# jopohl/urh

Hardware: NVIDIA H100
Metric: MSamples/s IQ demod+digitize (complex64) (higher is better)
Workload: dtype f32

## Files before the change

### urh_b200/csrc/center.cu

```cuda
#include "dense.cuh"
#include "scan.cuh"

#include <math.h>
#include <stdlib.h>

int urh_window_var_bitwise(urh_ctx* ctx, const float* d_x, int64_t n, const int64_t* d_prefix, int64_t t0, int64_t t1, int64_t r0,
                           int64_t r1, float* h_out2);

struct CenStats {
    double sum, sumsq;
    float mn, mx;
    long long cnt;
};

__global__ void __launch_bounds__(URH_WARPS_PER_BLOCK * 32)
k_tile_stats_f32(const float* __restrict__ x, int64_t n, int64_t ntiles, UrhTileStats* __restrict__ ts) {
    const int lane = threadIdx.x & 31;
    const int64_t tile = (int64_t)blockIdx.x * URH_WARPS_PER_BLOCK + (threadIdx.x >> 5);
    if (tile >= ntiles) return;
    const int64_t base = tile * URH_TILE;
    UrhStatAcc acc;
    acc.init();
    acc.all_noise = false;
    if (base + URH_TILE <= n && (((uintptr_t)x) & 15) == 0) {
// ... 344 lines not shown
    const int lane = threadIdx.x & 31;
    if (SMEM)
        for (int b = threadIdx.x; b < nbins; b += 256) s_hist[b] = 0u;
    if (edges_in_smem)
        for (int b = threadIdx.x; b < nbins + 3; b += 256) s_fe[b] = g_fe[b];
    __syncthreads();
    HistBins hb;
    if (FAST) hb.load(s_fe, scale, nbins);
    else hb.load(edges_in_smem ? s_fe : g_fe, scale, nbins);
    HistCache hc;
    hc.init();
    const int64_t gw = (int64_t)blk * 8 + (threadIdx.x >> 5), nw = (int64_t)nblk * 8;
    const bool vec = (((uintptr_t)x) & 15) == 0;
    const unsigned one = blockDim.x >> 8;
    {
        for (int64_t t = t_first + gw; t < t_end; t += nw) {
            if (prefix[t + 1] == prefix[t]) continue;
            const int64_t base = t * URH_TILE;
            if (vec) {
                const float4* p = (const float4*)(x + base) + lane;
                constexpr int ITERS = URH_TILE / 128, DEPTH = 4;
                float4 buf[DEPTH];
#pragma unroll
                for (int j = 0; j < DEPTH; j++) buf[j] = __ldg(p + j * 32);
#pragma unroll 1
                for (int it = 0; it < ITERS; it += DEPTH) {
                    const bool more = it + DEPTH < ITERS;
#pragma unroll
                    for (int j = 0; j < DEPTH; j++) {
                        const float4 v = buf[j];
                        if (more) buf[j] = __ldg(p + (it + DEPTH + j) * 32);
                        hist_put<SMEM, FAST>(hc, hb, s_hist, hist, v.x, one);
                        hist_put<SMEM, FAST>(hc, hb, s_hist, hist, v.y, one);
                        hist_put<SMEM, FAST>(hc, hb, s_hist, hist, v.z, one);
                        hist_put<SMEM, FAST>(hc, hb, s_hist, hist, v.w, one);
                    }
                }
            } else {
                for (int j = lane; j < URH_TILE; j += 32) hist_put<SMEM, FAST>(hc, hb, s_hist, hist, x[base + j], one);
            }
        }
    }
    hist_flush<SMEM>(hc, s_hist, hist);
    if (SMEM) {
        __syncthreads();
        for (int b = threadIdx.x; b < nbins; b += 256)
            if (s_hist[b]) atomicAdd(&hist[b], (unsigned long long)s_hist[b]);
    }
}

template <bool SMEM, bool FAST>
__global__ void __launch_bounds__(256, 4) k_hist_interior(const float* __restrict__ x, int64_t n, const int64_t* __restrict__ win,
                                                      const float* __restrict__ g_fe, float scale, int nbins,
                                                      unsigned long long* __restrict__ hist, int edges_in_smem,
                                                      const int64_t* __restrict__ prefix) {
    const int64_t w0 = win[0];
    hist_interior_body<SMEM, FAST>(x, n, w0 + 1, w0 >= 0 ? win[1] : 0, blockIdx.x, gridDim.x, g_fe, scale, nbins, hist, edges_in_smem, prefix);
}

__device__ __forceinline__ void hist_window_ends_body(const float* __restrict__ x, int64_t n, const int64_t* __restrict__ prefix,
                                                      const int64_t* __restrict__ win, int64_t r0, int64_t r1,
                                                      const float* __restrict__ g_fe, float scale, int nbins,
                                                      unsigned long long* __restrict__ hist, unsigned long long* __restrict__ hist2 = nullptr) {
    __shared__ int s_pre[256];
    const int64_t t = win[blockIdx.x];
    if (t < 0 || (blockIdx.x == 1 && t == win[0])) return;
    HistBins hb;
    hb.load(g_fe, scale, nbins);
    float v[CEN_PER];
    int64_t rank = cen_tile_ranks(x, n, t, prefix[t], v, s_pre);
#pragma unroll
    for (int j = 0; j < CEN_PER; j++) {
        const bool kept = v[j] > -4.0f;
        const int k = hb.bin_of<false>(v[j]);
        if (k >= 0 && rank >= r0 && rank < r1) {
            atomicAdd(&hist[k], 1ull);
            if (hist2) atomicAdd(&hist2[k], 1ull);
        }
        rank += kept ? 1 : 0;
    }
}

__global__ void __launch_bounds__(256) k_hist_window_ends(const float* __restrict__ x, int64_t n, const int64_t* __restrict__ prefix,
                                                         const int64_t* __restrict__ win, int64_t r0, int64_t r1,
                                                         const float* __restrict__ g_fe, float scale, int nbins,
                                                         unsigned long long* __restrict__ hist) {
    hist_window_ends_body(x, n, prefix, win, r0, r1, g_fe, scale, nbins, hist);
}

extern "C" int urh_center_histogram_tiles(urh_ctx* ctx, const float* d_qad, int64_t n, int64_t r0, int64_t r1, double hmin,
                                          double hstep, int64_t nbins, int64_t* h_hist) {
    if (nbins <= 0) return URH_OK;
    if (!tiles_match(ctx, d_qad, n)) URH_FAIL(ctx, URH_ERR_INVALID, "urh_afp_demod_tiles (same qad, same n) must precede urh_center_histogram_tiles");
    if (nbins > (int64_t)1 << 30) URH_FAIL(ctx, URH_ERR_INVALID, "too many histogram bins");
    const int64_t ntiles = urh_div_up(n, URH_TILE);
    const int64_t* prefix = (const int64_t*)ctx->center_prefix;
    unsigned long long* hist;
    float* fe;
    int64_t* d_win;
    URH_CHECK(urh_arena(ctx, (size_t)nbins, &hist));
    URH_CHECK(urh_arena(ctx, (size_t)nbins + 3, &fe));
    URH_CHECK(urh_arena(ctx, 4, &d_win));
    URH_CUDA(ctx, cudaMemsetAsync(hist, 0, (size_t)nbins * sizeof(unsigned long long), ctx->stream));
    URH_CUDA(ctx, cudaMemsetAsync(d_win, 0xff, 4 * sizeof(int64_t), ctx->stream));
    if (r1 > r0) {
        URH_LAUNCH(ctx, k_hist_edges, (unsigned)urh_div_up(nbins + 1, 256), 256, 0, hmin, hstep, nbins, fe);
        URH_LAUNCH(ctx, k_find_window_tiles, (unsigned)urh_div_up(ntiles, 256), 256, 0, prefix, ntiles, r0, r1, d_win);
        const bool in_smem = nbins <= 12000;
        const int edges_smem = (in_smem && nbins <= 6000) ? 1 : 0;
        const size_t dyn = (in_smem ? (size_t)nbins * 4 : 0) + (edges_smem ? (size_t)(nbins + 3) * 4 : 0);
        const float scale = (float)(1.0 / hstep);
        const double edge_abs = fmax(fabs(hmin), fabs(hmin + (double)nbins * hstep));
        const bool fast = edges_smem && hstep > 0.0 && edge_abs / hstep < 1048576.0;
        const unsigned gs = (unsigned)min(urh_div_up(ntiles, 8), (int64_t)ctx->sm_count * 8);
        const int64_t* cw = d_win;
        const float* cfe = fe;
        if (in_smem && fast) URH_LAUNCH(ctx, (k_hist_interior<true, true>), gs, 256, dyn, d_qad, n, cw, cfe, scale, (int)nbins, hist, edges_smem, prefix);
        else if (in_smem) URH_LAUNCH(ctx, (k_hist_interior<true, false>), gs, 256, dyn, d_qad, n, cw, cfe, scale, (int)nbins, hist, edges_smem, prefix);
        else URH_LAUNCH(ctx, (k_hist_interior<false, false>), gs, 256, dyn, d_qad, n, cw, cfe, scale, (int)nbins, hist, edges_smem, prefix);
        URH_LAUNCH(ctx, k_hist_window_ends, 2, 256, 0, d_qad, n, prefix, (const int64_t*)d_win, r0, r1, (const float*)fe, scale, (int)nbins, hist);
    }
    URH_CUDA(ctx, cudaMemcpyAsync(h_hist, hist, (size_t)nbins * sizeof(int64_t), cudaMemcpyDeviceToHost, ctx->stream));
    URH_CUDA(ctx, cudaStreamSynchronize(ctx->stream));
    return URH_OK;
}

extern "C" int urh_center_histogram(urh_ctx* ctx, const float* d_x, int64_t n, int64_t r0, int64_t r1, double hmin,
                                    double hstep, int64_t nbins, int64_t* h_hist) {
    if (nbins <= 0 || n <= 0) return URH_OK;
    if (!tiles_match(ctx, d_x, n)) {
        int64_t total = 0;
        URH_CHECK(tiles_from_array(ctx, d_x, n, &total));
    }
    return urh_center_histogram_tiles(ctx, d_x, n, r0, r1, hmin, hstep, nbins, h_hist);
}

#include "tilescan.cuh"

#define CEN_MAX_BINS 6000

struct __align__(16) CenterPlan {
    long long total, offset;
    long long r0, r1;
    long long lr0, lr1;
    long long win[4];
    CenStats local;
    double hmin, edge1, delta;
    long long nbins;
    double center;
    float centerf;
    float scale;
    int fast;
    int state;
    unsigned int ticket;
    int certified;
    long long straddle;
    long long pad;
};

struct ScanKept {
    const UrhTileStats* ts;
    int64_t* prefix;
    __device__ __forceinline__ int64_t load(int64_t t) const { return ts[t].cnt; }
    __device__ __forceinline__ void post(int64_t t, const int64_t& excl, const int64_t&) const { prefix[t] = excl; }
};
struct CenAddI64 {
    __device__ __forceinline__ int64_t operator()(int64_t a, int64_t b) const { return a + b; }
};

__global__ void k_center_ranks(const int64_t* __restrict__ counts, int rank, int world, int64_t max_size, CenterPlan* __restrict__ plan) {
    long long total = 0, offset = 0;
    for (int q = 0; q < world; q++) {
        if (q < rank) offset += counts[q];
        total += counts[q];
    }
    const long long kept = counts[rank];
    long long r0 = (long long)(0.05 * (double)total), r1 = (long long)(0.95 * (double)total);
    if (max_size >= 0 && r1 - r0 > max_size) r1 = r0 + max_size;
    plan->total = total; plan->offset = offset; plan->r0 = r0; plan->r1 = r1;
    long long a = r0 - offset, b = r1 - offset;
    a = a < 0 ? 0 : (a > kept ? kept : a);
    b = b < 0 ? 0 : (b > kept ? kept : b);
    plan->lr0 = a; plan->lr1 = b;
    plan->ticket = 0u;
    plan->state = 1;
    plan->certified = 0;
    plan->straddle = 0;
}

__device__ __forceinline__ int64_t cen_tile_of_rank(const int64_t* __restrict__ prefix, int64_t ntiles, int64_t r) {
    int64_t lo = 0, hi = ntiles;
    while (hi - lo > 1) {
        const int64_t mid = (lo + hi) >> 1;
        if (prefix[mid] <= r) lo = mid; else hi = mid;
    }
    return lo;
}

__global__ void __launch_bounds__(256) k_center_window(const float* __restrict__ x, int64_t n, const UrhTileStats* __restrict__ ts,
                                                      const int64_t* __restrict__ prefix, int64_t ntiles, CenterPlan* __restrict__ plan,
                                                      CenStats* __restrict__ partial) {
    __shared__ long long s_win[4];
    __shared__ int s_pre[256];
    __shared__ bool s_last;
    const long long r0 = plan->lr0, r1 = plan->lr1;
    if (threadIdx.x == 0) {
        long long w0 = -1, w1 = -1, w2 = -1, w3 = -1;
        if (r1 > r0) {
            w0 = cen_tile_of_rank(prefix, ntiles, r0);
            w1 = cen_tile_of_rank(prefix, ntiles, r1 - 1);
            const bool cov0 = prefix[w0] >= r0 && prefix[w0 + 1] <= r1;
            const bool cov1 = prefix[w1] >= r0 && prefix[w1 + 1] <= r1;
            w2 = cov0 ? -1 : w0;
            w3 = (cov1 || w1 == w0) ? -1 : w1;
        }
        s_win[0] = w0; s_win[1] = w1; s_win[2] = w2; s_win[3] = w3;
        if (blockIdx.x == 0) { plan->win[0] = w0; plan->win[1] = w1; plan->win[2] = w2; plan->win[3] = w3; }
    }
    __syncthreads();
    double sum = 0.0, sq = 0.0;
    float mn = INFINITY, mx = -INFINITY;
    long long cnt = 0;
    if (s_win[0] >= 0) {
        for (int64_t t = s_win[0] + (int64_t)blockIdx.x * 256 + threadIdx.x; t <= s_win[1]; t += (int64_t)gridDim.x * 256) {
            const int64_t a = prefix[t], b = prefix[t + 1];
            if (b > a && a >= r0 && b <= r1) {
                const UrhTileStats v = ts[t];
                sum += v.sum; sq += v.sumsq; mn = fminf(mn, v.mn); mx = fmaxf(mx, v.mx); cnt += v.cnt;
            }
        }
    }
    cen_block_fold(sum, sq, mn, mx, cnt, partial + blockIdx.x);
    if (blockIdx.x < 2) {
        const int64_t t = s_win[2 + blockIdx.x];
        sum = 0.0; sq = 0.0; mn = INFINITY; mx = -INFINITY; cnt = 0;
        if (t >= 0) {
            float v[CEN_PER];
            int64_t rank = cen_tile_ranks(x, n, t, prefix[t], v, s_pre);
#pragma unroll
            for (int j = 0; j < CEN_PER; j++) {
                if (v[j] > -4.0f) {
                    if (rank >= r0 && rank < r1) {
                        sum += (double)v[j];
                        sq += (double)v[j] * (double)v[j];
                        mn = fminf(mn, v[j]);
                        mx = fmaxf(mx, v[j]);
                        cnt++;
                    }
                    rank++;
                }
            }
        }
        cen_block_fold(sum, sq, mn, mx, cnt, partial + gridDim.x + blockIdx.x);
    }
    __threadfence();
    __syncthreads();
    if (threadIdx.x == 0) s_last = atomicAdd(&plan->ticket, 1u) == gridDim.x - 1;
    __syncthreads();
    if (!s_last) return;
    __threadfence();
    sum = 0.0; sq = 0.0; mn = INFINITY; mx = -INFINITY; cnt = 0;
    for (int64_t t = threadIdx.x; t < (int64_t)gridDim.x + 2; t += 256) {
        CenStats p;
        {
            const int4* src = (const int4*)(partial + t);
            int4 w0 = __ldcg(src), w1 = __ldcg(src + 1);
            memcpy(&p, &w0, 16);
            memcpy((char*)&p + 16, &w1, 16);
        }
        sum += p.sum; sq += p.sumsq; mn = fminf(mn, p.mn); mx = fmaxf(mx, p.mx); cnt += p.cnt;
    }
    cen_block_fold(sum, sq, mn, mx, cnt, &plan->local);
}

__global__ void __launch_bounds__(256) k_center_plan(const CenStats* __restrict__ parts, int world, CenterPlan* __restrict__ plan,
                                                    float* __restrict__ fe, unsigned long long* __restrict__ hist,
                                                    unsigned long long* __restrict__ xhist) {
    __shared__ int s_state;
    __shared__ long long s_nbins;
    __shared__ double s_hmin, s_edge1, s_delta;
    if (threadIdx.x == 0) {
        double cnt = 0.0, sum = 0.0, sq = 0.0;
        float mn = INFINITY, mx = -INFINITY;
        for (int q = 0; q < world; q++) {
            cnt += (double)parts[q].cnt;
            mn = fminf(mn, parts[q].mn);
            mx = fmaxf(mx, parts[q].mx);
            sum = __dadd_rn(sum, parts[q].sum);
            sq = __dadd_rn(sq, parts[q].sumsq);
        }
        int state = 0;
        long long nbins = 0;
        double hmin = 0.0, edge1 = 0.0, delta = 0.0;
        if (plan->r1 > plan->r0 && cnt > 0.0) {
            const double mean = __ddiv_rn(sum, cnt);
            double ss = __dsub_rn(sq, __dmul_rn(__dmul_rn(cnt, mean), mean));
            if (ss < 0.0) ss = 0.0;
            const double var = __ddiv_rn(ss, cnt);
            const double hstep = (double)__double2float_rn(var);
            hmin = (double)mn;
            const double stop = __dadd_rn((double)mx, hstep);
            if (hstep != 0.0) {
                const double val = __ddiv_rn(__dsub_rn(stop, hmin), hstep);
                if (val == val && fabs(val) < 9.0e18) {
                    const long long len = (long long)ceil(val);
                    if (len >= 2) {
                        nbins = len - 1;
                        edge1 = __dadd_rn(hmin, hstep);
                        delta = __dsub_rn(edge1, hmin);
                        state = (nbins <= CEN_MAX_BINS && delta > 0.0) ? 1 : 2;
                    }
                }
            }
        }
        plan->hmin = hmin; plan->edge1 = edge1; plan->delta = delta; plan->nbins = nbins;
        plan->state = state;
        plan->center = 0.0; plan->centerf = 0.0f;
        if (state == 1) {
            plan->scale = (float)(1.0 / delta);
            const double edge_abs = fmax(fabs(hmin), fabs(hmin + (double)nbins * delta));
            plan->fast = (edge_abs / delta < 1048576.0) ? 1 : 0;
        }
        s_state = state; s_nbins = nbins; s_hmin = hmin; s_edge1 = edge1; s_delta = delta;
    }
    __syncthreads();
    if (s_state != 1) return;
    const long long nbins = s_nbins;
    for (long long k = threadIdx.x; k <= nbins; k += 256) {
        const double e = (k == 0) ? s_hmin : (k == 1 ? s_edge1 : __dadd_rn(s_hmin, __dmul_rn((double)k, s_delta)));
        fe[k] = __double2float_ru(e);
        if (k == nbins) {
            fe[nbins + 1] = __double2float_rd(e);
            fe[nbins + 2] = fmaxf(__double2float_ru(s_hmin), nextafterf(-4.0f, 0.0f));
        }
        if (k < nbins) {
            hist[k] = 0ull;
            if (xhist) xhist[k] = 0ull;
        }
    }
}

template <bool FAST>
__global__ void __launch_bounds__(256, 3) k_hist_interior_dev(const float* __restrict__ x, int64_t n, const CenterPlan* __restrict__ plan,
                                                          const float* __restrict__ g_fe, unsigned long long* __restrict__ hist,
                                                          const int64_t* __restrict__ prefix) {
    if (plan->state != 1 || plan->certified || (plan->fast != 0) != FAST) return;
    hist_interior_body<true, FAST>(x, n, plan->win[0] + 1, plan->win[1], blockIdx.x, gridDim.x, g_fe, plan->scale, (int)plan->nbins, hist, 1,
                                   prefix);
}

__device__ __forceinline__ void cen_full_slabs(int64_t win0, int64_t win1, int64_t slab_tiles, int64_t* sf, int64_t* se) {
    *sf = (win0 + slab_tiles) / slab_tiles;
    *se = win1 / slab_tiles;
}

__global__ void __launch_bounds__(256) k_hist_window_ends_dev(const float* __restrict__ x, int64_t n, const int64_t* __restrict__ prefix,
                                                             const CenterPlan* __restrict__ plan, const float* __restrict__ g_fe,
                                                             unsigned long long* __restrict__ hist, unsigned long long* __restrict__ xhist,
                                                             int64_t slab_tiles) {
    if (plan->state != 1) return;
    if (blockIdx.x < 2) {
        hist_window_ends_body(x, n, prefix, (const int64_t*)plan->win, plan->lr0, plan->lr1, g_fe, plan->scale, (int)plan->nbins, hist, xhist);
        return;
    }
    const int64_t w0 = plan->win[0], w1 = plan->win[1];
    int64_t sf, se;
    cen_full_slabs(w0, w1, slab_tiles, &sf, &se);
    int64_t a_end = w1, b_begin = w1;
    if (sf < se) { a_end = sf * slab_tiles; b_begin = se * slab_tiles; }
    const int blk = blockIdx.x - 2, nblk = gridDim.x - 2, nbins = (int)plan->nbins;
    const float scale = plan->scale;
    if (plan->fast) {
        hist_interior_body<true, true>(x, n, w0 + 1, a_end, blk, nblk, g_fe, scale, nbins, xhist, 1, prefix);
        hist_interior_body<true, true>(x, n, b_begin, w1, blk, nblk, g_fe, scale, nbins, xhist, 1, prefix);
    } else {
        hist_interior_body<true, false>(x, n, w0 + 1, a_end, blk, nblk, g_fe, scale, nbins, xhist, 1, prefix);
        hist_interior_body<true, false>(x, n, b_begin, w1, blk, nblk, g_fe, scale, nbins, xhist, 1, prefix);
    }
}

__device__ __forceinline__ double cen_left_edge(const CenterPlan* plan, int k) {
    return (k == 0) ? plan->hmin : (k == 1 ? plan->edge1 : __dadd_rn(plan->hmin, __dmul_rn((double)k, plan->delta)));
}

#define CERT_THREADS 512
__global__ void __launch_bounds__(CERT_THREADS) k_center_certify(const UrhFine fine, CenterPlan* __restrict__ plan, const float* __restrict__ fe,
                                                                 const unsigned long long* __restrict__ xhist, unsigned long long* __restrict__ lo,
                                                                 unsigned long long* __restrict__ hi) {
    __shared__ unsigned long long s_ge[URH_FINE_NB + 1];
    __shared__ unsigned long long s_part[CERT_THREADS];
    __shared__ unsigned char s_flag[CEN_MAX_BINS];
    __shared__ unsigned long long s_key[3];
    __shared__ unsigned int s_certain;
    if (plan->state != 1) return;
    const int tid = threadIdx.x;
    constexpr int PER = URH_FINE_NB / CERT_THREADS;
    int64_t sf, se;
    cen_full_slabs(plan->win[0], plan->win[1], fine.slab_tiles, &sf, &se);
    unsigned long long b[PER], tot = 0;
#pragma unroll
    for (int j = 0; j < PER; j++) {
        unsigned long long v = 0;
        for (int64_t sl = sf; sl < se; sl++) v += fine.gh[sl * URH_FINE_NB + tid * PER + j];
        b[j] = v;
        tot += v;
    }
    s_part[tid] = tot;
    if (tid < 3) s_key[tid] = 0ull;
    if (tid == 0) s_certain = 0u;
    __syncthreads();
    for (int off = 1; off < CERT_THREADS; off <<= 1) {
        const unsigned long long add = (tid + off < CERT_THREADS) ? s_part[tid + off] : 0ull;
        __syncthreads();
        s_part[tid] += add;
        __syncthreads();
    }
    unsigned long long run = (tid + 1 < CERT_THREADS) ? s_part[tid + 1] : 0ull;
#pragma unroll
    for (int j = PER - 1; j >= 0; j--) {
        run += b[j];
        s_ge[tid * PER + j] = run;
    }
    if (tid == 0) s_ge[URH_FINE_NB] = 0ull;
    __syncthreads();
    const int nbins = (int)plan->nbins;
    const float f_hi = fe[nbins + 1], f_min = fe[nbins + 2], top = nextafterf(f_hi, INFINITY);
    auto ge = [&](float t, unsigned long long& glo, unsigned long long& ghi) {
        const int bt = urh_fine_bucket(t, fine.scale, fine.off);
        const bool straddles = urh_fine_bucket(nextafterf(t, -INFINITY), fine.scale, fine.off) == bt;
        ghi = s_ge[bt];
        glo = straddles ? s_ge[bt + 1] : s_ge[bt];
    };
    for (int k = tid; k < nbins; k += CERT_THREADS) {
        const float a = fmaxf(fe[k], f_min), e = (k == nbins - 1) ? top : fminf(fe[k + 1], top);
        unsigned long long l = 0, u = 0;
        if (a < e) {
            unsigned long long alo, ahi, elo, ehi;
            ge(a, alo, ahi);
            ge(e, elo, ehi);
            l = alo > ehi ? alo - ehi : 0ull;
            u = ahi - elo;
        }
        lo[k] = xhist[k] + l;
        hi[k] = xhist[k] + u;
    }
    __syncthreads();
    int window = (int)(0.05 * (double)nbins) + 1;
    if (window < 2) window = 2;
    for (int k = tid; k < nbins; k += CERT_THREADS) {
        const unsigned long long l = lo[k], u = hi[k];
        bool certain = l > 0ull, possible = u > 0ull;
        for (int d = -(window - 1); d < window && (certain || possible); d++) {
            const int j = k + d;
            if (d == 0 || j < 0 || j >= nbins) continue;
            certain = certain && l > hi[j];
            possible = possible && u > lo[j];
        }
        s_flag[k] = certain ? 1 : (possible ? 2 : 0);
        if (certain) atomicAdd(&s_certain, 1u);
    }
    __syncthreads();
    for (int pass = 0; pass < 3; pass++) {
        const long long p0 = pass > 0 ? (long long)(8191 - (s_key[0] & 8191)) : -1, p1 = pass > 1 ? (long long)(8191 - (s_key[1] & 8191)) : -1;
        for (int k = tid; k < nbins; k += CERT_THREADS) {
            if (k == p0 || k == p1) continue;
            if (pass < 2 && s_flag[k] == 1) atomicMax(&s_key[pass], (lo[k] << 13) | (unsigned long long)(8191 - k));
            if (pass == 2 && s_flag[k] != 0) atomicMax(&s_key[2], hi[k]);
        }
        __syncthreads();
    }
    if (tid != 0 || s_certain < 2u) return;
    const int k1 = 8191 - (int)(s_key[0] & 8191), k2 = 8191 - (int)(s_key[1] & 8191);
    plan->straddle = (long long)((hi[k1] - lo[k1]) + (hi[k2] - lo[k2]));
    if (!(lo[k2] > s_key[2])) return;
    const double c = __ddiv_rn(__dadd_rn(cen_left_edge(plan, k1), cen_left_edge(plan, k2)), 2.0);
    plan->center = c;
    plan->centerf = __double2float_rn(c);
    plan->certified = 1;
}

__global__ void __launch_bounds__(256) k_center_pick(const unsigned long long* __restrict__ y, CenterPlan* __restrict__ plan) {
    __shared__ unsigned long long s_best[256];
    __shared__ int s_idx[256];
    __shared__ int s_cnt[256];
    if (plan->state != 1 || plan->certified) return;
    const int nbins = (int)plan->nbins;
    int window = (int)(0.05 * (double)nbins) + 1;
    if (window < 2) window = 2;
    unsigned long long top_val[2] = {0ull, 0ull};
    int top_idx[2] = {-1, -1};
    int found = 0;
    bool undecided = false;
    for (int pass = 0; pass < 2 && !undecided; pass++) {
        unsigned long long best = 0ull;
        int bi = -1, ties = 0;
        for (int i = threadIdx.x; i < nbins; i += 256) {
            if (pass == 1 && i == top_idx[0]) continue;
            const unsigned long long v = y[i];
            if (v == 0ull || v < best) continue;
            bool peak = true;
            for (int d = 1; d < window && peak; d++) {
                const unsigned long long a = (i + d < nbins) ? y[i + d] : 0ull;
                const unsigned long long b = (i - d >= 0) ? y[i - d] : 0ull;
                peak = v > a && v > b;
            }
            if (!peak) continue;
            if (v > best) { best = v; bi = i; ties = 1; }
            else ties++;
        }
        s_best[threadIdx.x] = best; s_idx[threadIdx.x] = bi; s_cnt[threadIdx.x] = ties;
        __syncthreads();
        if (threadIdx.x == 0) {
            unsigned long long b = 0ull;
            int idx = -1, t = 0;
            for (int j = 0; j < 256; j++) {
                if (s_idx[j] < 0) continue;
                if (s_best[j] > b) { b = s_best[j]; idx = s_idx[j]; t = s_cnt[j]; }
                else if (s_best[j] == b) t += s_cnt[j];
            }
            s_best[0] = b; s_idx[0] = idx; s_cnt[0] = t;
        }
        __syncthreads();
        const unsigned long long b = s_best[0];
        const int idx = s_idx[0], t = s_cnt[0];
        __syncthreads();
        if (idx < 0) break;
        if (pass == 0) {
            top_val[0] = b; top_idx[0] = idx; found = 1;
            if (t == 2) {
                int other = -1;
                for (int i = threadIdx.x; i < nbins; i += 256) {
                    if (i == idx || y[i] != b) continue;
                    bool peak = true;
                    for (int d = 1; d < window && peak; d++) {
                        const unsigned long long a = (i + d < nbins) ? y[i + d] : 0ull;
                        const unsigned long long c = (i - d >= 0) ? y[i - d] : 0ull;
                        peak = b > a && b > c;
                    }
                    if (peak) other = i;
                }
                s_idx[threadIdx.x] = other;
                __syncthreads();
                if (threadIdx.x == 0) {
                    int o = -1;
                    for (int j = 0; j < 256; j++) if (s_idx[j] >= 0) o = s_idx[j];
                    s_idx[0] = o;
                }
                __syncthreads();
                top_idx[1] = s_idx[0]; top_val[1] = b; found = 2;
                __syncthreads();
                break;
            }
            if (t > 2) undecided = true;
        } else {
            if (t > 1) undecided = true;
            else { top_val[1] = b; top_idx[1] = idx; found = 2; }
        }
    }
    if (threadIdx.x != 0) return;
    if (undecided) { plan->state = 2; return; }
    if (found == 0) { plan->state = 0; return; }
    double c;
    if (found == 1) c = cen_left_edge(plan, top_idx[0]);
    else c = __ddiv_rn(__dadd_rn(cen_left_edge(plan, top_idx[0]), cen_left_edge(plan, top_idx[1])), 2.0);
    plan->center = c;
    plan->centerf = __double2float_rn(c);
    plan->state = 1;
    (void)top_val;
}

int urh_coll_allgather(urh_ctx* ctx, const void* d_send, void* d_recv, size_t bytes_per_rank);
bool urh_p2p_usable(urh_ctx* ctx, size_t bytes_per_rank);
extern "C" int urh_p2p_allreduce_u64_dev(urh_ctx* ctx, const void* d_in, void* d_out, const int64_t* d_count, int max_words);
extern "C" int urh_nccl_allreduce_i64(urh_ctx* ctx, int64_t* d_buf, int64_t count, int op);

int urh_center_chain(urh_ctx* ctx, const float* d_qad, int64_t n, const UrhTileStats* ts, int64_t max_size, int rank, int world,
                     const UrhFine* fine, CenterPlan** d_plan_out) {
    const int64_t ntiles = urh_div_up(n, URH_TILE);
    int64_t* prefix;
    CenterPlan* plan;
    CenStats* partial;
    float* fe;
    unsigned long long* hist;
    int64_t* d_counts;
    CenStats* d_parts;
    unsigned long long *xhist = nullptr, *cert_lo = nullptr, *cert_hi = nullptr;
    const int nb = ctx->sm_count * 2;
    URH_CHECK(urh_arena(ctx, (size_t)ntiles + 1, &prefix));
    URH_CHECK(urh_arena(ctx, 1, &plan));
    URH_CHECK(urh_arena(ctx, (size_t)nb + 2, &partial));
    URH_CHECK(urh_arena(ctx, (size_t)CEN_MAX_BINS + 3, &fe));
    URH_CHECK(urh_arena(ctx, (size_t)CEN_MAX_BINS, &hist));
    URH_CHECK(urh_arena(ctx, (size_t)world, &d_counts));
    URH_CHECK(urh_arena(ctx, (size_t)world, &d_parts));
    if (fine) {
        URH_CHECK(urh_arena(ctx, (size_t)CEN_MAX_BINS, &xhist));
        URH_CHECK(urh_arena(ctx, (size_t)CEN_MAX_BINS, &cert_lo));
        URH_CHECK(urh_arena(ctx, (size_t)CEN_MAX_BINS, &cert_hi));
    }
    ScanKept fk;
    fk.ts = ts; fk.prefix = prefix;
    URH_CHECK((urhts::scan<int64_t, CenAddI64, ScanKept>(ctx, ntiles, (int64_t)0, CenAddI64(), fk, prefix + ntiles)));
    const int64_t* counts = prefix + ntiles;
    if (world > 1) {
        URH_TL_MARK(ctx, "x1 kept counts: enter");
        URH_CHECK(urh_coll_allgather(ctx, prefix + ntiles, d_counts, sizeof(int64_t)));
        URH_TL_MARK(ctx, "x1 kept counts: done");
        counts = d_counts;
    }
    URH_LAUNCH(ctx, k_center_ranks, 1, 1, 0, counts, rank, world, max_size, plan);
    URH_LAUNCH(ctx, k_center_window, nb, 256, 0, d_qad, n, ts, (const int64_t*)prefix, ntiles, plan, partial);
    const CenStats* parts = &plan->local;
    if (world > 1) {
        URH_TL_MARK(ctx, "x2 window partials: enter");
        URH_CHECK(urh_coll_allgather(ctx, &plan->local, d_parts, sizeof(CenStats)));
        URH_TL_MARK(ctx, "x2 window partials: done");
        parts = d_parts;
    }
    URH_LAUNCH(ctx, k_center_plan, 1, 256, 0, parts, world, plan, fe, hist, xhist);
    const size_t dyn = (size_t)CEN_MAX_BINS * 4 + (size_t)(CEN_MAX_BINS + 3) * 4;
    const unsigned gs = (unsigned)min(urh_div_up(ntiles, 8), (int64_t)ctx->sm_count * 8);
    URH_LAUNCH(ctx, k_hist_window_ends_dev, fine ? 2 + ctx->sm_count * 4 : 2, 256, fine ? dyn : 0, d_qad, n, (const int64_t*)prefix,
               (const CenterPlan*)plan, (const float*)fe, hist, xhist, fine ? fine->slab_tiles : (int64_t)1);
    if (fine) URH_LAUNCH(ctx, k_center_certify, 1, CERT_THREADS, 0, *fine, plan, (const float*)fe, (const unsigned long long*)xhist, cert_lo, cert_hi);
    URH_LAUNCH(ctx, (k_hist_interior_dev<true>), gs, 256, dyn, d_qad, n, (const CenterPlan*)plan, (const float*)fe, hist, (const int64_t*)prefix);
    URH_LAUNCH(ctx, (k_hist_interior_dev<false>), gs, 256, dyn, d_qad, n, (const CenterPlan*)plan, (const float*)fe, hist, (const int64_t*)prefix);
    const unsigned long long* hist_all = hist;
    if (world > 1) URH_TL_MARK(ctx, "x3 histogram sum: enter");
    if (world > 1) {
        if (urh_p2p_usable(ctx, 8)) {
            unsigned long long* hist_sum;
            URH_CHECK(urh_arena(ctx, (size_t)CEN_MAX_BINS, &hist_sum));
            URH_CHECK(urh_p2p_allreduce_u64_dev(ctx, hist, hist_sum, (const int64_t*)&plan->nbins, CEN_MAX_BINS));
            hist_all = hist_sum;
        } else {
            URH_CHECK(urh_nccl_allreduce_i64(ctx, (int64_t*)hist, CEN_MAX_BINS, 0));
        }
    }
    if (world > 1) URH_TL_MARK(ctx, "x3 histogram sum: done");
    URH_LAUNCH(ctx, k_center_pick, 1, 256, 0, hist_all, plan);
    ctx->center_prefix = prefix;
    ctx->center_ts = ts;
    ctx->center_n = n;
    ctx->center_x = d_qad;
    *d_plan_out = plan;
    return URH_OK;
}

int urh_center_plan_certify_stats(urh_ctx* ctx, const CenterPlan* plan, int64_t* h_dst3) {
    h_dst3[0] = h_dst3[1] = h_dst3[2] = 0;
    URH_CUDA(ctx, cudaMemcpyAsync(h_dst3, &plan->certified, sizeof(int), cudaMemcpyDeviceToHost, ctx->stream));
    URH_CUDA(ctx, cudaMemcpyAsync(h_dst3 + 2, &plan->straddle, sizeof(long long), cudaMemcpyDeviceToHost, ctx->stream));
    return URH_OK;
}

extern "C" int urh_center_certify_stats(urh_ctx* ctx, int64_t* h_out3) {
    for (int i = 0; i < 3; i++) h_out3[i] = ctx->center_cert[i];
    return URH_OK;
}

int urh_center_plan_result(urh_ctx* ctx, const CenterPlan* plan, const float** d_centerf, const double** d_center, const int** d_state) {
    if (d_centerf) *d_centerf = &plan->centerf;
    if (d_center) *d_center = &plan->center;
    if (d_state) *d_state = &plan->state;
    return URH_OK;
}
```

### urh_b200/csrc/common.cuh

```cuda
#pragma once
#include <cuda_runtime.h>
#include <stdint.h>
#include <stdio.h>
#include <stdlib.h>
#include <string.h>
#include <vector>

#include "../../include/urh_b200.h"

#define URH_FULL_MASK 0xffffffffu

struct urh_block {
    void* ptr;
    size_t bytes;
};

struct urh_ctx {
    int device;
    int sm_count;
    cudaStream_t stream;
    cudaStream_t copy_stream[2];
    cudaEvent_t ev_start, ev_stop;
    cudaEvent_t ev_copy[2], ev_comp[2];
    cudaEvent_t ev_k0, ev_k1;
    int profiling;
    int dense_timed;
    cudaEvent_t tl_ev[32];
    const char* tl_name[32];
    int tl_count, tl_ready;
    char err[512];
    int64_t launches;
    std::vector<urh_block> arena;
    size_t arena_block;
    size_t arena_used;
    size_t arena_need;
    int64_t* pulses;
    size_t pulses_cap_rows;
    int64_t pulses_k;
    int64_t* h_mail;
    void* h_stage[2];
    size_t h_stage_bytes;
    int fft_plan;
    int fft_nfft;
    int64_t fft_batch;
    bool fft_valid;
    void* img_tw;
    int img_tw_n;
    void* shard_tiles;
    void* shard_staging;
    int shard_cap, shard_tol;
    int64_t shard_n;
    void* shard_state;
    int64_t costas_stats[3];
    int64_t costas_redone;
    int64_t costas_stitch[4];
    int mod_plan[2];
    int mod_plan_valid[2];
    int64_t mod_plan_n[2];
    int bits_valid;
    int64_t bits_nmsg, bits_total, bits_npos;
    void *bits_ptr, *bits_msg_off, *bits_pauses, *bits_pos;
    const void* center_ts;
    const void* center_x;
    int64_t center_n;
    void* center_prefix;
    int64_t center_cert[3];
    int64_t spec_stats[3];
    void* nccl_comm;
    void* nccl_stage;
    void* nccl_hstage;
    int nccl_rank, nccl_world;
    void* p2p_local;
    void* p2p_peer[8];
    void* p2p_hout;
    int p2p_rank, p2p_world;
    unsigned long long p2p_seq;
    void* ts_mem;
    int64_t ts_cap_blocks;
    unsigned long long ts_issued;
    uint32_t ts_epoch;
    void* step_dev;
    void* shard_fin;
    int64_t stream_free_low, stream_chunks;
    size_t arena_live;
    size_t arena_peak;
};

#define URH_CUDA(ctx, call)                                                                         \
    do {                                                                                            \
        cudaError_t e__ = (call);                                                                   \
        if (e__ != cudaSuccess) {                                                                   \
            snprintf((ctx)->err, sizeof((ctx)->err), "%s:%d: %s -> %s", __FILE__, __LINE__, #call,  \
                     cudaGetErrorString(e__));                                                      \
            return (e__ == cudaErrorMemoryAllocation) ? URH_ERR_NOMEM : URH_ERR_CUDA;               \
        }                                                                                           \
    } while (0)

#define URH_CHECK(call)                 \
    do {                                \
        int rc__ = (call);              \
        if (rc__ != URH_OK) return rc__; \
    } while (0)

#define URH_FAIL(ctx, code, ...)                                  \
    do {                                                          \
        snprintf((ctx)->err, sizeof((ctx)->err), __VA_ARGS__);    \
        return (code);                                            \
    } while (0)

#define URH_LAUNCH(ctx, kernel, grid, block, smem, ...)                                   \
    do {                                                                                  \
        kernel<<<(grid), (block), (smem), (ctx)->stream>>>(__VA_ARGS__);                  \
        (ctx)->launches++;                                                                \
        URH_CUDA(ctx, cudaGetLastError());                                                \
    } while (0)

#define URH_TL_MARK(ctx, label) do { if ((ctx)->profiling >= 2 && (ctx)->tl_ready && (ctx)->tl_count < 32) { \
        (ctx)->tl_name[(ctx)->tl_count] = (label); cudaEventRecord((ctx)->tl_ev[(ctx)->tl_count++], (ctx)->stream); } } while (0)
#define URH_TL_RESET(ctx) do { (ctx)->tl_count = 0; } while (0)
#define URH_PROF_BEGIN(ctx) do { if ((ctx)->profiling) cudaEventRecord((ctx)->ev_k0, (ctx)->stream); } while (0)
#define URH_PROF_END(ctx) do { if ((ctx)->profiling) { cudaEventRecord((ctx)->ev_k1, (ctx)->stream); (ctx)->dense_timed = 1; } } while (0)

void urh_arena_reset(urh_ctx* ctx);
int urh_arena_alloc(urh_ctx* ctx, size_t bytes, void** out);
template <typename T>
static inline int urh_arena(urh_ctx* ctx, size_t count, T** out) {
    void* p = nullptr;
    int rc = urh_arena_alloc(ctx, count * sizeof(T), &p);
    *out = (T*)p;
    return rc;
}
struct UrhArenaMark {
    size_t block, used, live;
};
static inline UrhArenaMark urh_arena_mark(const urh_ctx* ctx) { return UrhArenaMark{ctx->arena_block, ctx->arena_used, ctx->arena_live}; }
static inline void urh_arena_release(urh_ctx* ctx, const UrhArenaMark& m) {
    ctx->arena_block = m.block;
    ctx->arena_used = m.used;
    ctx->arena_live = m.live;
}
int urh_ensure_pulses(urh_ctx* ctx, size_t rows);
int urh_ensure_pulses_keep(urh_ctx* ctx, size_t rows, size_t keep);
void urh_stream_sample_free(urh_ctx* ctx);
void urh_release_mod_plans(urh_ctx* ctx);
int urh_ensure_stage(urh_ctx* ctx, size_t bytes);

struct UrhCostasStream {
    float* state;
    int64_t* acc;
    int segs;
};
int urh_costas_stream_begin(urh_ctx* ctx, UrhCostasStream* S);
int urh_costas_stream_chunk(urh_ctx* ctx, UrhCostasStream* S, int64_t c, const void* d_iq, int dtype, int64_t n, float noise_sqrd,
                            int loop_order, float bandwidth, float* d_out);
int urh_costas_stream_end(urh_ctx* ctx, const UrhCostasStream* S);
int64_t urh_costas_arena_bytes(int64_t n, int loop_order);

int urh_read_i64(urh_ctx* ctx, const int64_t* d_src, int count, int64_t* h_out);

__host__ __device__ static inline int64_t urh_div_up(int64_t a, int64_t b) { return (a + b - 1) / b; }

static inline int urh_iq_bytes(int dtype) {
    switch (dtype) {
        case URH_DT_I8:
        case URH_DT_U8: return 2;
        case URH_DT_I16:
        case URH_DT_U16: return 4;
        case URH_DT_F32: return 8;
        default: return 0;
    }
}

static inline float urh_noise_value(int mod_type) {
    switch (mod_type) {
        case URH_MOD_ASK: return 0.0f;
        case URH_MOD_FSK:
        case URH_MOD_PSK:
        case URH_MOD_OQPSK: return -4.0f;
        case URH_MOD_QAM: return 0.0f * -4.0f;
        default: return 0.0f;
    }
}
```

### urh_b200/csrc/context.cu

```cuda
#include "common.cuh"
#include "tilescan.cuh"

extern "C" int urh_device_count(void) {
    int n = 0;
    if (cudaGetDeviceCount(&n) != cudaSuccess) return 0;
    return n;
}

extern "C" int urh_ctx_create(int device, urh_ctx** out) {
    if (!out) return URH_ERR_INVALID;
    *out = nullptr;
    int n = 0;
    if (cudaGetDeviceCount(&n) != cudaSuccess || n <= 0) return URH_ERR_NO_DEVICE;
    if (device < 0 || device >= n) return URH_ERR_INVALID;
    urh_ctx* ctx = new urh_ctx();
    ctx->device = device;
    ctx->err[0] = 0;
    ctx->launches = 0;
    ctx->arena_block = 0;
    ctx->arena_used = 0;
    ctx->arena_need = 0;
    ctx->pulses = nullptr;
    ctx->pulses_cap_rows = 0;
    ctx->pulses_k = 0;
    ctx->h_mail = nullptr;
    ctx->h_stage[0] = ctx->h_stage[1] = nullptr;
    ctx->h_stage_bytes = 0;
    ctx->fft_valid = false;
    ctx->shard_tiles = nullptr;
    ctx->shard_staging = nullptr;
    ctx->shard_state = nullptr;
    ctx->bits_valid = 0;
    ctx->mod_plan_valid[0] = ctx->mod_plan_valid[1] = 0;
    ctx->center_prefix = nullptr;
    ctx->center_ts = nullptr;
    ctx->center_x = nullptr;
    ctx->center_n = 0;
    ctx->nccl_comm = nullptr;
    ctx->nccl_stage = nullptr;
    ctx->nccl_hstage = nullptr;
    ctx->p2p_local = nullptr;
    ctx->p2p_hout = nullptr;
    ctx->p2p_world = 0;
    ctx->p2p_rank = 0;
    ctx->p2p_seq = 0;
    for (int i = 0; i < 8; i++) ctx->p2p_peer[i] = nullptr;
    ctx->nccl_rank = 0;
    ctx->nccl_world = 1;
    ctx->stream_free_low = -1;
    ctx->stream_chunks = 0;
    if (cudaSetDevice(device) != cudaSuccess) {
        delete ctx;
        return URH_ERR_CUDA;
    }
    cudaDeviceProp prop;
    if (cudaGetDeviceProperties(&prop, device) != cudaSuccess) {
        delete ctx;
        return URH_ERR_CUDA;
    }
    ctx->sm_count = prop.multiProcessorCount;
    {
        cudaMemPool_t pool;
        if (cudaDeviceGetDefaultMemPool(&pool, device) == cudaSuccess) {
            unsigned long long keep = ~0ull;
            cudaMemPoolSetAttribute(pool, cudaMemPoolAttrReleaseThreshold, &keep);
        }
    }
    bool ok = cudaStreamCreateWithFlags(&ctx->stream, cudaStreamNonBlocking) == cudaSuccess;
    ok = ok && cudaStreamCreateWithFlags(&ctx->copy_stream[0], cudaStreamNonBlocking) == cudaSuccess;
    ok = ok && cudaStreamCreateWithFlags(&ctx->copy_stream[1], cudaStreamNonBlocking) == cudaSuccess;
    ok = ok && cudaEventCreate(&ctx->ev_start) == cudaSuccess && cudaEventCreate(&ctx->ev_stop) == cudaSuccess;
    for (int i = 0; i < 2 && ok; i++) {
        ok = ok && cudaEventCreateWithFlags(&ctx->ev_copy[i], cudaEventDisableTiming) == cudaSuccess;
        ok = ok && cudaEventCreateWithFlags(&ctx->ev_comp[i], cudaEventDisableTiming) == cudaSuccess;
    }
    ok = ok && cudaEventCreate(&ctx->ev_k0) == cudaSuccess && cudaEventCreate(&ctx->ev_k1) == cudaSuccess;
    ctx->profiling = 0;
    ctx->dense_timed = 0;
    ctx->tl_count = 0;
    ctx->tl_ready = 0;
    ok = ok && cudaHostAlloc((void**)&ctx->h_mail, 64 * sizeof(int64_t), cudaHostAllocDefault) == cudaSuccess;
    if (!ok) {
        delete ctx;
        return URH_ERR_CUDA;
    }
    *out = ctx;
    return URH_OK;
}

extern "C" void urh_ctx_destroy(urh_ctx* ctx) {
    if (!ctx) return;
    cudaSetDevice(ctx->device);
    cudaStreamSynchronize(ctx->stream);
    urh_release_mod_plans(ctx);
    for (auto& b : ctx->arena) cudaFree(b.ptr);
    if (ctx->pulses) cudaFree(ctx->pulses);
    if (ctx->shard_state) free(ctx->shard_state);
    if (ctx->h_mail) cudaFreeHost(ctx->h_mail);
    if (ctx->ts_mem) cudaFree(ctx->ts_mem);
    if (ctx->step_dev) cudaFree(ctx->step_dev);
    if (ctx->img_tw) cudaFree(ctx->img_tw);
    if (ctx->shard_fin) free(ctx->shard_fin);
    for (int i = 0; i < 2; i++)
        if (ctx->h_stage[i]) cudaFreeHost(ctx->h_stage[i]);
    cudaEventDestroy(ctx->ev_start);
    cudaEventDestroy(ctx->ev_stop);
    for (int i = 0; i < 2; i++) {
        cudaEventDestroy(ctx->ev_copy[i]);
        cudaEventDestroy(ctx->ev_comp[i]);
        cudaStreamDestroy(ctx->copy_stream[i]);
    }
    cudaStreamDestroy(ctx->stream);
    delete ctx;
}

extern "C" const char* urh_last_error(urh_ctx* ctx) { return ctx ? ctx->err : "null context"; }

extern "C" int urh_sync(urh_ctx* ctx) {
    URH_CUDA(ctx, cudaStreamSynchronize(ctx->stream));
    return URH_OK;
}

extern "C" int urh_device_info(urh_ctx* ctx, int* sm_count, int* cc_major, int* cc_minor, size_t* total_mem,
                               char* name, int name_cap) {
    cudaDeviceProp prop;
    URH_CUDA(ctx, cudaGetDeviceProperties(&prop, ctx->device));
    if (sm_count) *sm_count = prop.multiProcessorCount;
    if (cc_major) *cc_major = prop.major;
    if (cc_minor) *cc_minor = prop.minor;
    if (total_mem) *total_mem = prop.totalGlobalMem;
    if (name && name_cap > 0) {
        strncpy(name, prop.name, name_cap - 1);
        name[name_cap - 1] = 0;
    }
    return URH_OK;
}

extern "C" int urh_malloc(urh_ctx* ctx, size_t bytes, void** d_ptr) {
    URH_CUDA(ctx, cudaSetDevice(ctx->device));
    if (bytes == 0) bytes = 16;
    URH_CUDA(ctx, cudaMallocAsync(d_ptr, bytes, ctx->stream));
    return URH_OK;
}

extern "C" int urh_free(urh_ctx* ctx, void* d_ptr) {
    if (!d_ptr) return URH_OK;
    URH_CUDA(ctx, cudaFreeAsync(d_ptr, ctx->stream));
    return URH_OK;
}

extern "C" int urh_memset(urh_ctx* ctx, void* d_ptr, int value, size_t bytes) {
    URH_CUDA(ctx, cudaMemsetAsync(d_ptr, value, bytes, ctx->stream));
    return URH_OK;
}

extern "C" int urh_memcpy_h2d(urh_ctx* ctx, void* d_dst, const void* h_src, size_t bytes) {
    if (bytes == 0) return URH_OK;
    URH_CUDA(ctx, cudaMemcpyAsync(d_dst, h_src, bytes, cudaMemcpyHostToDevice, ctx->stream));
    return URH_OK;
}

extern "C" int urh_memcpy_d2h(urh_ctx* ctx, void* h_dst, const void* d_src, size_t bytes) {
    if (bytes) URH_CUDA(ctx, cudaMemcpyAsync(h_dst, d_src, bytes, cudaMemcpyDeviceToHost, ctx->stream));
    URH_CUDA(ctx, cudaStreamSynchronize(ctx->stream));
    return URH_OK;
}

extern "C" int urh_memcpy_d2d(urh_ctx* ctx, void* d_dst, const void* d_src, size_t bytes) {
    if (bytes == 0) return URH_OK;
    URH_CUDA(ctx, cudaMemcpyAsync(d_dst, d_src, bytes, cudaMemcpyDeviceToDevice, ctx->stream));
    return URH_OK;
}

extern "C" int urh_host_alloc(urh_ctx* ctx, size_t bytes, void** h_ptr) {
    if (bytes == 0) bytes = 16;
    URH_CUDA(ctx, cudaHostAlloc(h_ptr, bytes, cudaHostAllocDefault));
    return URH_OK;
}

extern "C" int urh_host_free(urh_ctx* ctx, void* h_ptr) {
    if (h_ptr) URH_CUDA(ctx, cudaFreeHost(h_ptr));
    return URH_OK;
}

extern "C" int urh_timer_start(urh_ctx* ctx) {
    URH_CUDA(ctx, cudaEventRecord(ctx->ev_start, ctx->stream));
    return URH_OK;
}

extern "C" int urh_timer_stop(urh_ctx* ctx, float* ms) {
    URH_CUDA(ctx, cudaEventRecord(ctx->ev_stop, ctx->stream));
    URH_CUDA(ctx, cudaEventSynchronize(ctx->ev_stop));
    float t = 0.f;
    URH_CUDA(ctx, cudaEventElapsedTime(&t, ctx->ev_start, ctx->ev_stop));
    if (ms) *ms = t;
    return URH_OK;
}

extern "C" int urh_set_profiling(urh_ctx* ctx, int enabled) {
    ctx->profiling = enabled < 0 ? 0 : (enabled > 2 ? 2 : enabled);
    ctx->dense_timed = 0;
    if (ctx->profiling >= 2 && !ctx->tl_ready) {
        for (int i = 0; i < 32; i++) URH_CUDA(ctx, cudaEventCreate(&ctx->tl_ev[i]));
        ctx->tl_ready = 1;
    }
    ctx->tl_count = 0;
    return URH_OK;
}

extern "C" int urh_timeline_fetch(urh_ctx* ctx, float* h_ms, char* h_names, int names_cap, int* count) {
    if (!count) return URH_ERR_INVALID;
    *count = 0;
    if (ctx->profiling < 2 || ctx->tl_count == 0) return URH_OK;
    URH_CUDA(ctx, cudaEventSynchronize(ctx->tl_ev[ctx->tl_count - 1]));
    int pos = 0;
    for (int i = 0; i < ctx->tl_count; i++) {
        float t = 0.f;
        URH_CUDA(ctx, cudaEventElapsedTime(&t, ctx->tl_ev[0], ctx->tl_ev[i]));
        if (h_ms) h_ms[i] = t;
        if (h_names) pos += snprintf(h_names + pos, pos < names_cap ? (size_t)(names_cap - pos) : 0, "%s\n", ctx->tl_name[i]);
    }
    *count = ctx->tl_count;
    return URH_OK;
}

extern "C" int urh_last_dense_ms(urh_ctx* ctx, float* ms) {
    if (!ctx->dense_timed) URH_FAIL(ctx, URH_ERR_INVALID, "no dense kernel timed (enable urh_set_profiling first)");
    URH_CUDA(ctx, cudaEventSynchronize(ctx->ev_k1));
    URH_CUDA(ctx, cudaEventElapsedTime(ms, ctx->ev_k0, ctx->ev_k1));
    return URH_OK;
}

extern "C" int64_t urh_launch_count(urh_ctx* ctx) { return ctx ? ctx->launches : 0; }

void urh_arena_reset(urh_ctx* ctx) {
    if (ctx->arena.size() > 1) {
        cudaStreamSynchronize(ctx->stream);
        size_t total = 0;
        for (auto& b : ctx->arena) {
            total += b.bytes;
            cudaFree(b.ptr);
        }
        ctx->arena.clear();
        void* p = nullptr;
        if (cudaMalloc(&p, total) == cudaSuccess) ctx->arena.push_back({p, total});
        else cudaGetLastError();
    }
    ctx->arena_block = 0;
    ctx->arena_used = 0;
    ctx->arena_need = 0;
    ctx->arena_live = 0;
    ctx->arena_peak = 0;
    ctx->center_prefix = nullptr;
    ctx->bits_valid = 0;
}

static void arena_note_peak(urh_ctx* ctx) {
    if (ctx->arena_live > ctx->arena_peak) ctx->arena_peak = ctx->arena_live;
}

int urh_arena_alloc(urh_ctx* ctx, size_t bytes, void** out) {
    bytes = (bytes + 255) & ~(size_t)255;
    if (bytes == 0) bytes = 256;
    ctx->arena_need += bytes;
// ... 126 lines not shown
```

### urh_b200/csrc/digitize.cu

```cuda
#include "dense.cuh"
#include "scan.cuh"
#include "sparse.cuh"
#ifndef URH_FAST_MIN_BLOCKS
#define URH_FAST_MIN_BLOCKS 4
#endif
#include "fsk_fast.cuh"
#include "dense_f32.cuh"
#include "stream_ring.cuh"

#include <math.h>
#include <stdlib.h>


template <int DT, int MOD, bool DIGITIZE>
__device__ __forceinline__ void dense_iq_tile(const void* __restrict__ iq, int64_t n, const UrhDemodParams& dp, float* __restrict__ qad_out,
                                              int vec_in, int vec_out, const UrhClassify& cls, int tol, UrhTileSummary* __restrict__ tiles,
                                              uint32_t* __restrict__ staging, int stage_cap, int16_t* __restrict__ init_cls, int cls_of_zero,
                                              int64_t tile, int has_halo, UrhTileStats* __restrict__ tile_stats, const UrhFine& fine,
                                              unsigned int* s_fine, unsigned int* g_fine) {
    const int lane = threadIdx.x & 31;
    const int64_t tile_start = tile * URH_TILE;
    const int tile_len = (int)((n - tile_start) < URH_TILE ? (n - tile_start) : URH_TILE);
    const int iters = (tile_len + 63) >> 6;

    UrhRunTracker rt;
    if (DIGITIZE) rt.init(tol, staging + tile * (int64_t)stage_cap);
    UrhStatAcc acc;
    acc.init();

    float cA = 0.0f, cB = 0.0f;
    if (MOD == URH_MOD_FSK && (tile_start > 0 || has_halo) && lane == 0) {
        typedef typename UrhElem<DT>::type E;
        const E* pp = (const E*)iq + 2 * (tile_start - 1);
        const UrhFskTerms t = urh_fsk_terms((float)pp[0], (float)pp[1]);
        cA = t.A; cB = t.B;
    }

    UrhPair cur = urh_load_pair<DT>(iq, tile_start + 2 * lane, n, vec_in != 0);
    for (int it = 0; it < iters; it++) {
        const int64_t pos0 = tile_start + (int64_t)it * 64 + 2 * lane;
        UrhPair nxt;
        if (it + 1 < iters) nxt = urh_load_pair<DT>(iq, pos0 + 64, n, vec_in != 0);

        const float m0 = __fadd_rn(__fmul_rn(cur.r0, cur.r0), __fmul_rn(cur.i0, cur.i0));
        const float m1 = __fadd_rn(__fmul_rn(cur.r1, cur.r1), __fmul_rn(cur.i1, cur.i1));
        float s0 = dp.noise_value, s1 = dp.noise_value;
        if (MOD == URH_MOD_FSK) {
            const UrhFskTerms t0 = urh_fsk_terms(cur.r0, cur.i0);
            const UrhFskTerms t1 = urh_fsk_terms(cur.r1, cur.i1);
            float pA = __shfl_up_sync(URH_FULL_MASK, t1.A, 1);
            float pB = __shfl_up_sync(URH_FULL_MASK, t1.B, 1);
            if (lane == 0) { pA = cA; pB = cB; }
            cA = __shfl_sync(URH_FULL_MASK, t1.A, 31);
            cB = __shfl_sync(URH_FULL_MASK, t1.B, 31);
            if (!(m0 <= dp.noise_sqrd)) s0 = urh_fsk_angle(pA, pB, t0.C, t0.D);
            if (!(m1 <= dp.noise_sqrd)) s1 = urh_fsk_angle(t0.A, t0.B, t1.C, t1.D);
        } else if (MOD == URH_MOD_ASK) {
            if (!(m0 <= dp.noise_sqrd)) s0 = __fdiv_rn(__fsqrt_rn(m0), dp.max_mag);
            if (!(m1 <= dp.noise_sqrd)) s1 = __fdiv_rn(__fsqrt_rn(m1), dp.max_mag);
        }
        if (pos0 == 0 && !has_halo) s0 = dp.noise_value;

        const bool v0 = pos0 < n, v1 = pos0 + 1 < n;
        if (tile_stats) {
            if (v0) { acc.add(s0); acc.all_noise = acc.all_noise && (s0 == dp.noise_value); }
            if (v1) { acc.add(s1); acc.all_noise = acc.all_noise && (s1 == dp.noise_value); }
            if (s_fine) {
                if (v0) urh_fine_add(s0, fine, s_fine, g_fine);
                if (v1) urh_fine_add(s1, fine, s_fine, g_fine);
            }
        }
        if (qad_out) {
            if (v1 && vec_out) urh_stg_f2(qad_out + pos0, s0, s1);
            else {
                if (v0) qad_out[pos0] = s0;
                if (v1) qad_out[pos0 + 1] = s1;
            }
        }
        if (DIGITIZE) {
            const int c0 = urh_classify(s0, cls), c1 = urh_classify(s1, cls);
            if (pos0 == 0) *init_cls = (int16_t)((s0 == cls.noise_value) ? -1 : cls_of_zero);
            rt.feed(it, c0, c1, v0, v1, lane);
        }
        cur = nxt;
    }
    if (tile_stats) acc.store(tile_stats + tile, lane);
    if (DIGITIZE) rt.finish(tile_len, tiles + tile, lane);
}

template <int DT, int MOD, bool DIGITIZE>
__global__ void __launch_bounds__(URH_WARPS_PER_BLOCK * 32)
k_dense_iq(const void* __restrict__ iq, int64_t n, UrhDemodParams dp, float* __restrict__ qad_out, int vec_in,
           int vec_out, const __grid_constant__ UrhClassify cls, int tol, UrhTileSummary* __restrict__ tiles,
           uint32_t* __restrict__ staging, int stage_cap, int16_t* __restrict__ init_cls, int cls_of_zero,
           int64_t tile_begin, int64_t tile_count, int has_halo, UrhTileStats* __restrict__ tile_stats, const UrhFine fine) {
    extern __shared__ unsigned int s_fine[];
    const int64_t tile_rel = (int64_t)blockIdx.x * URH_WARPS_PER_BLOCK + (threadIdx.x >> 5);
    const int64_t block_tile0 = tile_begin + (int64_t)blockIdx.x * URH_WARPS_PER_BLOCK;
    if (fine.gh) urh_fine_zero(s_fine);
    if (tile_rel < tile_count && (tile_begin + tile_rel) * URH_TILE < n)
        dense_iq_tile<DT, MOD, DIGITIZE>(iq, n, dp, qad_out, vec_in, vec_out, cls, tol, tiles, staging, stage_cap, init_cls, cls_of_zero,
                                    tile_begin + tile_rel, has_halo, tile_stats, fine,
                                    fine.gh ? s_fine : nullptr, fine.gh ? urh_fine_row(fine, tile_begin + tile_rel, block_tile0) : nullptr);
    if (fine.gh) urh_fine_flush(fine, s_fine, block_tile0);
}

template <int DT, bool DIGITIZE, bool WRITE, bool STATS>
__global__ void __launch_bounds__(URH_WARPS_PER_BLOCK * 32, URH_FAST_MIN_BLOCKS)
k_fsk_fast(const void* __restrict__ iq, int64_t n, UrhDemodParams dp, float* __restrict__ qad_out, float thr0,
           float cls_noise, int tol, UrhTileSummary* __restrict__ tiles, uint32_t* __restrict__ staging, int stage_cap,
           int64_t tile_begin, int64_t tile_count, UrhTileStats* __restrict__ tile_stats, const UrhFine fine) {
    extern __shared__ unsigned int s_fine[];
    const bool fine_on = STATS && fine.gh;
    const int lane = threadIdx.x & 31;
    const int64_t tile_rel = (int64_t)blockIdx.x * URH_WARPS_PER_BLOCK + (threadIdx.x >> 5);
    const int64_t block_tile0 = tile_begin + (int64_t)blockIdx.x * URH_WARPS_PER_BLOCK;
    if (fine_on) urh_fine_zero(s_fine);
    if (tile_rel < tile_count) {
        const int64_t tile = tile_begin + tile_rel;
        UrhRunTracker rt;
        if (DIGITIZE) rt.init(tol, staging + tile * (int64_t)stage_cap);
        UrhOne one;
        one.p = dp.one;
        one.m = dp.mone;
        urh_fsk_full_tile<DT, DIGITIZE, WRITE, STATS>(iq, n, tile * URH_TILE, dp, qad_out, thr0, cls_noise, rt, lane, one,
                                                      STATS ? tile_stats + tile : nullptr, 0u, DIGITIZE ? tiles + tile : nullptr, fine,
                                                      fine_on ? s_fine : nullptr, fine_on ? urh_fine_row(fine, tile, block_tile0) : nullptr);
    }
    if (fine_on) urh_fine_flush(fine, s_fine, block_tile0);
}

#define URH_FSK_FIFO 3
template <int DT, bool DIGITIZE, bool WRITE, bool STATS>
__global__ void __launch_bounds__(URH_WARPS_PER_BLOCK * 32, (DT == URH_DT_F32) ? 5 : 4)
k_fsk_fifo(const void* __restrict__ iq, int64_t n, UrhDemodParams dp, float* __restrict__ qad_out, float thr0,
           float cls_noise, int tol, UrhTileSummary* __restrict__ tiles, uint32_t* __restrict__ staging, int stage_cap,
           int64_t tile_begin, int64_t tile_count, UrhTileStats* __restrict__ tile_stats, const UrhFine fine,
           const float* __restrict__ d_thr0 = nullptr, float* __restrict__ margin = nullptr) {
    __shared__ __align__(16) unsigned char s_fifo[URH_WARPS_PER_BLOCK][URH_FSK_FIFO + 1][64 * 2 * sizeof(typename UrhElem<DT>::type)];
    extern __shared__ unsigned int s_fine[];
    const bool fine_on = STATS && fine.gh;
    if (DIGITIZE && STATS) thr0 = *d_thr0;
    const int lane = threadIdx.x & 31;
    const int64_t tile_rel = (int64_t)blockIdx.x * URH_WARPS_PER_BLOCK + (threadIdx.x >> 5);
    const int64_t block_tile0 = tile_begin + (int64_t)blockIdx.x * URH_WARPS_PER_BLOCK;
    if (fine_on) urh_fine_zero(s_fine);
    if (tile_rel < tile_count) {
        const int64_t tile = tile_begin + tile_rel;
        UrhRunTracker rt;
        if (DIGITIZE) rt.init(tol, staging + tile * (int64_t)stage_cap);
        UrhOne one;
        one.p = dp.one;
        one.m = dp.mone;
        const uint32_t fifo = (uint32_t)__cvta_generic_to_shared(&s_fifo[threadIdx.x >> 5][0][0]);
        urh_fsk_full_tile<DT, DIGITIZE, WRITE, STATS, URH_FSK_FIFO>(iq, n, tile * URH_TILE, dp, qad_out, thr0, cls_noise, rt, lane, one,
                                                                    STATS ? tile_stats + tile : nullptr, fifo,
                                                                    DIGITIZE ? tiles + tile : nullptr, fine, fine_on ? s_fine : nullptr,
                                                                    fine_on ? urh_fine_row(fine, tile, block_tile0) : nullptr,
                                                                    (DIGITIZE && STATS) ? margin + tile : nullptr);
    }
    if (fine_on) urh_fine_flush(fine, s_fine, block_tile0);
}

#define URH_GUESS_SAMPLES 16384
#define URH_GUESS_BINS 128
#define URH_GUESS_THREADS 1024
__global__ void __launch_bounds__(URH_GUESS_THREADS) k_speculate_guess(const float2* __restrict__ iq, int64_t n, float noise_sqrd, int forced,
                                                                      float forced_tg, float* __restrict__ d_tg, unsigned int* __restrict__ redone) {
    constexpr int PER = URH_GUESS_SAMPLES / URH_GUESS_THREADS;
    __shared__ unsigned int s_hist[URH_GUESS_BINS];
    __shared__ float s_mn[32], s_mx[32];
    if (forced) {
        if (threadIdx.x == 0) { *d_tg = forced_tg; *redone = 0u; }
        return;
    }
    for (int b = threadIdx.x; b < URH_GUESS_BINS; b += blockDim.x) s_hist[b] = 0u;
    float v[PER];
    float mn = INFINITY, mx = -INFINITY;
#pragma unroll
    for (int k = 0; k < PER; k++) {
        const int64_t i = 1 + (int64_t)(k * URH_GUESS_THREADS + threadIdx.x) * (n - 1) / URH_GUESS_SAMPLES;
        const float2 p = iq[i - 1], c = iq[i];
        v[k] = NAN;
        if (!(c.x * c.x + c.y * c.y <= noise_sqrd)) {
            v[k] = atan2f(p.x * c.y - p.y * c.x, p.x * c.x + p.y * c.y);
            mn = fminf(mn, v[k]);
            mx = fmaxf(mx, v[k]);
        }
    }
    for (int off = 16; off > 0; off >>= 1) {
        mn = fminf(mn, __shfl_xor_sync(URH_FULL_MASK, mn, off));
        mx = fmaxf(mx, __shfl_xor_sync(URH_FULL_MASK, mx, off));
    }
    if ((threadIdx.x & 31) == 0) { s_mn[threadIdx.x >> 5] = mn; s_mx[threadIdx.x >> 5] = mx; }
    __syncthreads();
    mn = INFINITY; mx = -INFINITY;
    for (int w = 0; w < URH_GUESS_THREADS / 32; w++) { mn = fminf(mn, s_mn[w]); mx = fmaxf(mx, s_mx[w]); }
    const float width = (mx - mn) / URH_GUESS_BINS;
    if (width > 0.0f) {
#pragma unroll
        for (int k = 0; k < PER; k++)
            if (!isnan(v[k])) atomicAdd(&s_hist[min((int)((v[k] - mn) / width), URH_GUESS_BINS - 1)], 1u);
    }
    __syncthreads();
    if (threadIdx.x != 0) return;
    *redone = 0u;
    if (!(mn <= mx)) { *d_tg = 0.0f; return; }
    if (!(width > 0.0f)) { *d_tg = mn; return; }
    constexpr int WINDOW = (int)(0.05 * URH_GUESS_BINS) + 1;
    int top[2] = {-1, -1};
    for (int b = 0; b < URH_GUESS_BINS; b++) {
        const unsigned int y = s_hist[b];
        bool peak = y > 0u;
        for (int d = 1; d < WINDOW && peak; d++)
            peak = y > (b + d < URH_GUESS_BINS ? s_hist[b + d] : 0u) && y > (b - d >= 0 ? s_hist[b - d] : 0u);
        if (!peak) continue;
        if (top[0] < 0 || y > s_hist[top[0]]) { top[1] = top[0]; top[0] = b; }
        else if (top[1] < 0 || y > s_hist[top[1]]) top[1] = b;
    }
    if (top[0] < 0) *d_tg = 0.5f * (mn + mx);
    else if (top[1] < 0) *d_tg = mn + ((float)top[0] + 0.5f) * width;
    else *d_tg = mn + (0.5f * (float)(top[0] + top[1]) + 0.5f) * width;
}


extern "C" int urh_get_center_thresholds(float center, float spacing, int modulation_order, float* h_out) {
    const int n = modulation_order / 2;
    for (int i = 0; i < n; i++) {
        volatile float t = (float)(n - (i + 1)) * spacing;
        h_out[i] = center - t;
    }
    for (int i = n; i < modulation_order - 1; i++) {
        volatile float t = (float)(i + 1 - n) * spacing;
        h_out[i] = center + t;
    }
    return URH_OK;
}

static int fill_classify(urh_ctx* ctx, UrhClassify* C, int mod_type, float center, uint8_t bits_per_symbol,
                         float spacing) {
    if (bits_per_symbol > 8) URH_FAIL(ctx, URH_ERR_INVALID, "bits_per_symbol %d > 8 not supported", (int)bits_per_symbol);
    memset(C, 0, sizeof(*C));
    C->noise_value = urh_noise_value(mod_type);
    C->order = 1 << bits_per_symbol;
    if (C->order > 1) urh_get_center_thresholds(center, spacing, C->order, C->thr);
    return URH_OK;
}

static int host_classify(float s, const UrhClassify& C) {
    int c = C.order - 1;
    for (int k = 0; k < C.order - 1; k++)
        if (s <= C.thr[k]) { c = k; break; }
    return c;
}

static float max_magnitude_for(int dtype) {
    switch (dtype) {
        case URH_DT_I8: return (float)sqrt(127.0 * 127.0 + 128.0 * 128.0);
        case URH_DT_U8: return (float)sqrt(255.0 * 255.0);
        case URH_DT_I16: return (float)sqrt(32768.0 * 32768.0 + 32767.0 * 32767.0);
        case URH_DT_U16: return (float)sqrt(65535.0 * 65535.0);
        default: return (float)sqrt(2.0);
    }
}

static bool iq_vec_aligned(const void* p, int dtype) { return ((uintptr_t)p % (2 * (size_t)urh_iq_bytes(dtype))) == 0; }

template <int DT, int MOD, bool DIG>
static int launch_dense_iq_t(urh_ctx* ctx, const void* d_iq, int64_t n, const UrhDemodParams& dp, float* d_qad,
                             const UrhClassify& cls, int tol, UrhTileSummary* tiles, uint32_t* staging,
                             int stage_cap, int16_t* init_cls, int cls_of_zero, int has_halo = 0,
                             UrhTileStats* tile_stats = nullptr, int64_t tile_lo = 0, int64_t tile_hi = -1,
                             const UrhFine& fine = UrhFine{}, UrhSpec* spec = nullptr) {
    const int64_t ntiles = urh_div_up(n, URH_TILE);
    const size_t fine_smem = fine.gh ? (size_t)URH_FINE_NB * sizeof(unsigned int) : 0;
    if (tile_hi < 0 || tile_hi > ntiles) tile_hi = ntiles;
    const int vec_in = iq_vec_aligned(d_iq, DT) ? 1 : 0;
    const int vec_out = (d_qad && ((uintptr_t)d_qad % 8) == 0) ? 1 : 0;
    const int threads = URH_WARPS_PER_BLOCK * 32;
    auto generic = [&](int64_t begin, int64_t end) -> int {
        begin = begin < tile_lo ? tile_lo : begin;
        end = end > tile_hi ? tile_hi : end;
        const int64_t count = end - begin;
        if (count <= 0) return URH_OK;
        URH_LAUNCH(ctx, (k_dense_iq<DT, MOD, DIG>), (unsigned)urh_div_up(count, URH_WARPS_PER_BLOCK), threads, fine_smem, d_iq, n, dp,
                   d_qad, vec_in, vec_out, cls, tol, tiles, staging, stage_cap, init_cls, cls_of_zero, begin, count, has_halo,
                   tile_stats, fine);
        return URH_OK;
    };
    const int64_t nfull = n / URH_TILE;
    const bool fast = MOD == URH_MOD_FSK && vec_in && (!d_qad || vec_out) && (!DIG || cls.order == 2) && nfull > 1;
    URH_PROF_BEGIN(ctx);
    if (fast) {
        const int64_t fb = tile_lo > 1 ? tile_lo : 1, fe = tile_hi < nfull ? tile_hi : nfull;
        if (fe > fb) {
            const unsigned grid = (unsigned)urh_div_up(fe - fb, URH_WARPS_PER_BLOCK);
            static const bool fifo = getenv("URH_B200_FSK_NO_FIFO") == nullptr;
            const bool ff = fifo;
            bool speculated = false;
            if constexpr (DT == URH_DT_F32 && MOD == URH_MOD_FSK && !DIG) {
                if (spec && ff && tile_stats && d_qad) {
                    URH_LAUNCH(ctx, (k_fsk_fifo<DT, true, true, true>), grid, threads, fine_smem, d_iq, n, dp, d_qad, 0.0f, dp.noise_value,
                               tol, tiles, staging, stage_cap, fb, fe - fb, tile_stats, fine, (const float*)spec->tg, spec->margin);
                    spec->lo = fb;
                    spec->hi = fe;
                    speculated = true;
                }
            }
            if (speculated) {
            } else if (tile_stats && d_qad && !DIG) {
                if (ff) URH_LAUNCH(ctx, (k_fsk_fifo<DT, false, true, true>), grid, threads, fine_smem, d_iq, n, dp, d_qad, cls.thr[0], cls.noise_value,
                                   tol, tiles, staging, stage_cap, fb, fe - fb, tile_stats, fine);
                else URH_LAUNCH(ctx, (k_fsk_fast<DT, false, true, true>), grid, threads, fine_smem, d_iq, n, dp, d_qad, cls.thr[0], cls.noise_value,
                                tol, tiles, staging, stage_cap, fb, fe - fb, tile_stats, fine);
            } else if (d_qad) {
                if (ff) URH_LAUNCH(ctx, (k_fsk_fifo<DT, DIG, true, false>), grid, threads, 0, d_iq, n, dp, d_qad, cls.thr[0], cls.noise_value, tol,
                                   tiles, staging, stage_cap, fb, fe - fb, nullptr, UrhFine{});
                else URH_LAUNCH(ctx, (k_fsk_fast<DT, DIG, true, false>), grid, threads, 0, d_iq, n, dp, d_qad, cls.thr[0], cls.noise_value, tol,
                                tiles, staging, stage_cap, fb, fe - fb, nullptr, UrhFine{});
            } else {
                if (ff) URH_LAUNCH(ctx, (k_fsk_fifo<DT, DIG, false, false>), grid, threads, 0, d_iq, n, dp, d_qad, cls.thr[0], cls.noise_value, tol,
                                   tiles, staging, stage_cap, fb, fe - fb, nullptr, UrhFine{});
                else URH_LAUNCH(ctx, (k_fsk_fast<DT, DIG, false, false>), grid, threads, 0, d_iq, n, dp, d_qad, cls.thr[0], cls.noise_value, tol,
                                tiles, staging, stage_cap, fb, fe - fb, nullptr, UrhFine{});
            }
        }
        URH_CHECK(generic(0, 1));
        URH_CHECK(generic(nfull, ntiles));
    } else {
        URH_CHECK(generic(0, ntiles));
    }
    URH_PROF_END(ctx);
    return URH_OK;
}

template <int MOD, bool DIG>
static int launch_dense_iq_m(urh_ctx* ctx, int dtype, const void* d_iq, int64_t n, const UrhDemodParams& dp,
                             float* d_qad, const UrhClassify& cls, int tol, UrhTileSummary* tiles,
                             uint32_t* staging, int stage_cap, int16_t* init_cls, int cls_of_zero, int has_halo = 0,
                             UrhTileStats* tile_stats = nullptr, int64_t tile_lo = 0, int64_t tile_hi = -1,
                             const UrhFine& fine = UrhFine{}, UrhSpec* spec = nullptr) {
    switch (dtype) {
        case URH_DT_I8: return launch_dense_iq_t<URH_DT_I8, MOD, DIG>(ctx, d_iq, n, dp, d_qad, cls, tol, tiles, staging, stage_cap, init_cls, cls_of_zero, has_halo, tile_stats, tile_lo, tile_hi, fine);
        case URH_DT_U8: return launch_dense_iq_t<URH_DT_U8, MOD, DIG>(ctx, d_iq, n, dp, d_qad, cls, tol, tiles, staging, stage_cap, init_cls, cls_of_zero, has_halo, tile_stats, tile_lo, tile_hi, fine);
        case URH_DT_I16: return launch_dense_iq_t<URH_DT_I16, MOD, DIG>(ctx, d_iq, n, dp, d_qad, cls, tol, tiles, staging, stage_cap, init_cls, cls_of_zero, has_halo, tile_stats, tile_lo, tile_hi, fine);
        case URH_DT_U16: return launch_dense_iq_t<URH_DT_U16, MOD, DIG>(ctx, d_iq, n, dp, d_qad, cls, tol, tiles, staging, stage_cap, init_cls, cls_of_zero, has_halo, tile_stats, tile_lo, tile_hi, fine);
        case URH_DT_F32: return launch_dense_iq_t<URH_DT_F32, MOD, DIG>(ctx, d_iq, n, dp, d_qad, cls, tol, tiles, staging, stage_cap, init_cls, cls_of_zero, has_halo, tile_stats, tile_lo, tile_hi, fine, spec);
        default: URH_FAIL(ctx, URH_ERR_DTYPE, "Unsupported dtype");
    }
}

int urh_costas_demod(urh_ctx* ctx, const void* d_iq, int dtype, int64_t n, float noise_sqrd, int loop_order,
                     float bandwidth, float* d_out);

static UrhDemodParams make_demod_params(float noise_mag, int mod_type, int dtype) {
    UrhDemodParams dp;
    volatile float nm = noise_mag;
    volatile float sq = nm * nm;
    dp.noise_sqrd = sq;
    dp.noise_value = urh_noise_value(mod_type);
    dp.max_mag = max_magnitude_for(dtype);
    dp.one = 1.0f;
    dp.mone = -1.0f;
    return dp;
}

extern "C" int urh_afp_demod(urh_ctx* ctx, const void* d_iq, int dtype, int64_t n, float noise_mag, int mod_type,
                             int mod_order, float costas_loop_bandwidth, float* d_out) {
    if (n < 0) URH_FAIL(ctx, URH_ERR_INVALID, "negative length");
    if (urh_iq_bytes(dtype) == 0) URH_FAIL(ctx, URH_ERR_DTYPE, "Unsupported dtype");
    if (n == 0) return URH_OK;
    if (n <= 2 || (mod_type != URH_MOD_ASK && mod_type != URH_MOD_FSK && mod_type != URH_MOD_PSK)) {
        URH_CUDA(ctx, cudaMemsetAsync(d_out, 0, (size_t)n * sizeof(float), ctx->stream));
        if (n > 2) {
            const float nv = urh_noise_value(mod_type);
            URH_CUDA(ctx, cudaMemcpyAsync(d_out, &nv, sizeof(float), cudaMemcpyHostToDevice, ctx->stream));
            URH_CUDA(ctx, cudaStreamSynchronize(ctx->stream));
        }
        return URH_OK;
    }
    const UrhDemodParams dp = make_demod_params(noise_mag, mod_type, dtype);
    if (mod_type == URH_MOD_PSK) return urh_costas_demod(ctx, d_iq, dtype, n, dp.noise_sqrd, mod_order, costas_loop_bandwidth, d_out);
    UrhClassify cls;
    memset(&cls, 0, sizeof(cls));
    if (mod_type == URH_MOD_ASK)
        return launch_dense_iq_m<URH_MOD_ASK, false>(ctx, dtype, d_iq, n, dp, d_out, cls, 0, nullptr, nullptr, 0, nullptr, 0);
    return launch_dense_iq_m<URH_MOD_FSK, false>(ctx, dtype, d_iq, n, dp, d_out, cls, 0, nullptr, nullptr, 0, nullptr, 0);
}

int urh_center_tiles_begin(urh_ctx* ctx, const float* d_x, const UrhTileStats* ts, int64_t n, int64_t* h_total);

extern "C" int urh_afp_demod_tiles(urh_ctx* ctx, const void* d_iq, int dtype, int64_t n, float noise_mag, int mod_type,
                                   float* d_qad_out, int halo, int64_t* h_kept) {
    if (n <= 2 || (mod_type != URH_MOD_ASK && mod_type != URH_MOD_FSK) || !d_qad_out)
        URH_FAIL(ctx, URH_ERR_INVALID, "urh_afp_demod_tiles: ASK/FSK, n > 2 and a qad buffer are required");
    if (urh_iq_bytes(dtype) == 0) URH_FAIL(ctx, URH_ERR_DTYPE, "Unsupported dtype");
    urh_arena_reset(ctx);
    const UrhDemodParams dp = make_demod_params(noise_mag, mod_type, dtype);
    UrhClassify cls;
    memset(&cls, 0, sizeof(cls));
    const int64_t ntiles = urh_div_up(n, URH_TILE);
    UrhTileStats* ts;
    URH_CHECK(urh_arena(ctx, (size_t)ntiles, &ts));
    if (mod_type == URH_MOD_ASK)
        URH_CHECK((launch_dense_iq_m<URH_MOD_ASK, false>(ctx, dtype, d_iq, n, dp, d_qad_out, cls, 0, nullptr, nullptr, 0, nullptr, 0, halo, ts)));
    else
        URH_CHECK((launch_dense_iq_m<URH_MOD_FSK, false>(ctx, dtype, d_iq, n, dp, d_qad_out, cls, 0, nullptr, nullptr, 0, nullptr, 0, halo, ts)));
    return urh_center_tiles_begin(ctx, d_qad_out, ts, n, h_kept);
}

int urh_finish_local(urh_ctx* ctx, int64_t n, int tol, bool is_ask, uint32_t sps, const UrhTileSummary* tiles, const uint32_t* staging,
                     int stage_cap, const int16_t* d_init, int64_t* k);
int urh_finish_shard(urh_ctx* ctx, int64_t n, int tol, bool is_ask, uint32_t sps, const UrhTileSummary* tiles, const uint32_t* staging,
                     int stage_cap, const int16_t* d_init, int64_t global_offset, int64_t n_total, int64_t* k);

static int digitize_finish(urh_ctx* ctx, int64_t n, int tol, bool is_ask, uint32_t sps, UrhTileSummary* tiles,
                           uint32_t* staging, int stage_cap, int16_t* d_init, int64_t* k) {
    if (getenv("URH_B200_OLD_FINISH")) {
        UrhCandidates cand;
        URH_CHECK(urh_collect_candidates(ctx, n, tol, tiles, staging, stage_cap, &cand));
        return urh_pulses_from_candidates(ctx, n, tol, is_ask, sps, cand, d_init, k);
    }
    return urh_finish_local(ctx, n, tol, is_ask, sps, tiles, staging, stage_cap, d_init, k);
}

static int stage_cap_for(int tol) { return URH_TILE / (tol + 1) + 2; }

extern "C" int urh_grab_pulse_lens(urh_ctx* ctx, const float* d_qad, int64_t n, float center, uint16_t tolerance,
                                   int mod_type, uint32_t samples_per_symbol, uint8_t bits_per_symbol,
                                   float center_spacing, int64_t* k) {
    if (!k) return URH_ERR_INVALID;
    *k = 0;
    ctx->pulses_k = 0;
    if (n < 0) URH_FAIL(ctx, URH_ERR_INVALID, "negative length");
    if (n == 0) return URH_OK;
    urh_arena_reset(ctx);
    UrhClassify cls;
    URH_CHECK(fill_classify(ctx, &cls, mod_type, center, bits_per_symbol, center_spacing));
    const int tol = tolerance;
    const int64_t ntiles = urh_div_up(n, URH_TILE);
    const int cap = stage_cap_for(tol);
    UrhTileSummary* tiles;
    uint32_t* staging;
    int16_t* d_init;
    URH_CHECK(urh_arena(ctx, (size_t)ntiles, &tiles));
    URH_CHECK(urh_arena(ctx, (size_t)ntiles * cap, &staging));
    URH_CHECK(urh_arena(ctx, 8, &d_init));
    const unsigned grid = (unsigned)urh_div_up(ntiles, URH_WARPS_PER_BLOCK);
    const int vec_in = (((uintptr_t)d_qad % 8) == 0) ? 1 : 0;
    URH_PROF_BEGIN(ctx);
    if (cls.order == 2)
        URH_LAUNCH(ctx, (k_dense_f32<SrcQad2, float>), grid, URH_WARPS_PER_BLOCK * 32, 0, d_qad, n, vec_in, cls, tol, tiles,
                   staging, cap, d_init, host_classify(0.0f, cls));
    else
        URH_LAUNCH(ctx, (k_dense_f32<SrcQad, float>), grid, URH_WARPS_PER_BLOCK * 32, 0, d_qad, n, vec_in, cls, tol, tiles,
                   staging, cap, d_init, host_classify(0.0f, cls));
    URH_PROF_END(ctx);
    return digitize_finish(ctx, n, tol, mod_type == URH_MOD_ASK, samples_per_symbol, tiles, staging, cap, d_init, k);
}

extern "C" int urh_demod_digitize(urh_ctx* ctx, const void* d_iq, int dtype, int64_t n, float noise_mag,
                                  int mod_type, float center, uint16_t tolerance, uint32_t samples_per_symbol,
                                  uint8_t bits_per_symbol, float center_spacing, float* d_qad_out, int64_t* k) {
    if (!k) return URH_ERR_INVALID;
    *k = 0;
    ctx->pulses_k = 0;
    if (n < 0) URH_FAIL(ctx, URH_ERR_INVALID, "negative length");
    if (urh_iq_bytes(dtype) == 0) URH_FAIL(ctx, URH_ERR_DTYPE, "Unsupported dtype");
    if (n == 0) return URH_OK;
    if (n <= 2 || (mod_type != URH_MOD_ASK && mod_type != URH_MOD_FSK)) {
        float* q = d_qad_out;
        if (!q) URH_CUDA(ctx, cudaMalloc((void**)&q, (size_t)n * sizeof(float)));
        int rc = urh_afp_demod(ctx, d_iq, dtype, n, noise_mag, mod_type, 1 << bits_per_symbol, 0.1f, q);
        if (rc == URH_OK)
            rc = urh_grab_pulse_lens(ctx, q, n, center, tolerance, mod_type, samples_per_symbol, bits_per_symbol,
                                     center_spacing, k);
        if (!d_qad_out) {
            cudaStreamSynchronize(ctx->stream);
            cudaFree(q);
        }
        return rc;
    }
    urh_arena_reset(ctx);
    UrhClassify cls;
    URH_CHECK(fill_classify(ctx, &cls, mod_type, center, bits_per_symbol, center_spacing));
    const UrhDemodParams dp = make_demod_params(noise_mag, mod_type, dtype);
    const int tol = tolerance;
    const int64_t ntiles = urh_div_up(n, URH_TILE);
    const int cap = stage_cap_for(tol);
    UrhTileSummary* tiles;
    uint32_t* staging;
    int16_t* d_init;
    URH_CHECK(urh_arena(ctx, (size_t)ntiles, &tiles));
    URH_CHECK(urh_arena(ctx, (size_t)ntiles * cap, &staging));
    URH_CHECK(urh_arena(ctx, 8, &d_init));
    const int c0 = host_classify(0.0f, cls);
    if (mod_type == URH_MOD_ASK)
        URH_CHECK((launch_dense_iq_m<URH_MOD_ASK, true>(ctx, dtype, d_iq, n, dp, d_qad_out, cls, tol, tiles, staging, cap, d_init, c0)));
    else
        URH_CHECK((launch_dense_iq_m<URH_MOD_FSK, true>(ctx, dtype, d_iq, n, dp, d_qad_out, cls, tol, tiles, staging, cap, d_init, c0)));
    return digitize_finish(ctx, n, tol, mod_type == URH_MOD_ASK, samples_per_symbol, tiles, staging, cap, d_init, k);
}

extern "C" int urh_shard_dense(urh_ctx* ctx, const void* d_iq, int dtype, int64_t n, int has_halo, float noise_mag, int mod_type,
                               float center, uint16_t tolerance, uint8_t bits_per_symbol, float center_spacing,
                               float* d_qad_out, int64_t* h_summary) {
    if (n <= 0) URH_FAIL(ctx, URH_ERR_INVALID, "empty shard");
    if (mod_type != URH_MOD_ASK && mod_type != URH_MOD_FSK) URH_FAIL(ctx, URH_ERR_INVALID, "sharded path: ASK / FSK only (PSK is a serial recurrence)");
    if (urh_iq_bytes(dtype) == 0) URH_FAIL(ctx, URH_ERR_DTYPE, "Unsupported dtype");
    urh_arena_reset(ctx);
    UrhClassify cls;
    URH_CHECK(fill_classify(ctx, &cls, mod_type, center, bits_per_symbol, center_spacing));
    const UrhDemodParams dp = make_demod_params(noise_mag, mod_type, dtype);
    const int tol = tolerance;
    const int64_t ntiles = urh_div_up(n, URH_TILE);
    const int cap = stage_cap_for(tol);
    UrhTileSummary* tiles;
    uint32_t* staging;
    int16_t* d_init;
    URH_CHECK(urh_arena(ctx, (size_t)ntiles, &tiles));
    URH_CHECK(urh_arena(ctx, (size_t)ntiles * cap, &staging));
    URH_CHECK(urh_arena(ctx, 8, &d_init));
    URH_CUDA(ctx, cudaMemsetAsync(d_init, 0, 16, ctx->stream));
    const int c0 = host_classify(0.0f, cls);
    if (mod_type == URH_MOD_ASK)
        URH_CHECK((launch_dense_iq_m<URH_MOD_ASK, true>(ctx, dtype, d_iq, n, dp, d_qad_out, cls, tol, tiles, staging, cap, d_init, c0, has_halo)));
    else
        URH_CHECK((launch_dense_iq_m<URH_MOD_FSK, true>(ctx, dtype, d_iq, n, dp, d_qad_out, cls, tol, tiles, staging, cap, d_init, c0, has_halo)));
    ctx->shard_tiles = tiles;
    ctx->shard_staging = staging;
    ctx->shard_cap = cap;
    ctx->shard_n = n;
    ctx->shard_tol = tol;
    URH_CHECK(urh_shard_run_total(ctx, n, tiles, h_summary));
    int16_t init16 = 0;
    URH_CUDA(ctx, cudaMemcpyAsync(&init16, d_init, sizeof(int16_t), cudaMemcpyDeviceToHost, ctx->stream));
    URH_CUDA(ctx, cudaStreamSynchronize(ctx->stream));
    h_summary[3] = init16;
    return URH_OK;
}

extern "C" int urh_shard_dense_qad(urh_ctx* ctx, const float* d_qad, int64_t n, int mod_type, float center, uint16_t tolerance,
                                   uint8_t bits_per_symbol, float center_spacing, int64_t* h_summary) {
    if (n <= 0) URH_FAIL(ctx, URH_ERR_INVALID, "empty shard");
    urh_arena_reset(ctx);
    UrhClassify cls;
    URH_CHECK(fill_classify(ctx, &cls, mod_type, center, bits_per_symbol, center_spacing));
    const int tol = tolerance;
    const int64_t ntiles = urh_div_up(n, URH_TILE);
    const int cap = stage_cap_for(tol);
    UrhTileSummary* tiles;
    uint32_t* staging;
    int16_t* d_init;
    URH_CHECK(urh_arena(ctx, (size_t)ntiles, &tiles));
    URH_CHECK(urh_arena(ctx, (size_t)ntiles * cap, &staging));
    URH_CHECK(urh_arena(ctx, 8, &d_init));
    URH_CUDA(ctx, cudaMemsetAsync(d_init, 0, 16, ctx->stream));
    const int vec_in = (((uintptr_t)d_qad % 8) == 0) ? 1 : 0;
    URH_PROF_BEGIN(ctx);
    const unsigned grid = (unsigned)urh_div_up(ntiles, URH_WARPS_PER_BLOCK);
    if (cls.order == 2)
        URH_LAUNCH(ctx, (k_dense_f32<SrcQad2, float>), grid, URH_WARPS_PER_BLOCK * 32, 0, d_qad, n, vec_in, cls, tol, tiles, staging, cap,
                   d_init, host_classify(0.0f, cls));
    else
        URH_LAUNCH(ctx, (k_dense_f32<SrcQad, float>), grid, URH_WARPS_PER_BLOCK * 32, 0, d_qad, n, vec_in, cls, tol, tiles, staging, cap,
                   d_init, host_classify(0.0f, cls));
    URH_PROF_END(ctx);
// ... 83 lines not shown
    } else {
        z.src_slot = (kind == URH_STREAM_ENTRY_GRAB_PULSE_LENS && (entry & URH_STREAM_QAD_ON_DEVICE)) ? 0
                     : URH_STREAM_PAD + z.cs * (iq ? urh_iq_bytes(dtype) : 4);
        const bool qad_ring = kind == URH_STREAM_ENTRY_AFP_DEMOD ||
                              (kind == URH_STREAM_ENTRY_DEMOD_DIGITIZE && ((entry & URH_STREAM_QAD_OUT) || psk));
        z.qad_slot = qad_ring ? z.cs * 4 : 0;
        z.ring_bytes = ring * (r256(z.src_slot) + r256(z.qad_slot));
        if (kind == URH_STREAM_ENTRY_DEMOD_CENTER_DIGITIZE) z.ring_bytes += r256(n * 4);
    }
    z.arena = 0;
    z.scan_items = ct > z.rows_chunk ? ct : z.rows_chunk;
    if (digitize) z.arena += r256(ct * (int64_t)sizeof(UrhTileSummary)) + r256(ct * cap * 4) + r256(16) + r256(sizeof(UrhChain)) +
                             finish_arena_bytes(ct, z.rows_chunk, true);
    if (psk && !resident) z.arena += urh_costas_arena_bytes(z.cs, psk) + r256(16) + r256(6 * 8);
    if (kind == URH_STREAM_ENTRY_DEMOD_CENTER_DIGITIZE) {
        z.arena += r256(ntiles * (int64_t)sizeof(UrhTileStats)) + r256((int64_t)URH_FINE_SLABS * URH_FINE_NB * 4) + r256((ntiles + 1) * 8) +
                   ((int64_t)2 << 20);
        if (ntiles > z.scan_items) z.scan_items = ntiles;
    }
    return z;
}

extern "C" int urh_stream_footprint(int64_t n, int dtype, int tolerance, int64_t chunk_samples, int ring, int entry, int64_t rows,
                                    int64_t* bytes) {
    if (!bytes || n < 0 || tolerance < 0 || tolerance > 0xffff || (entry & 0xf) > URH_STREAM_ENTRY_DEMOD_CENTER_DIGITIZE) return URH_ERR_INVALID;
    if (!(entry & URH_STREAM_RESIDENT) && (ring < 2 || ring > URH_STREAM_MAX_RING)) return URH_ERR_INVALID;
    if ((entry & 0xf) != URH_STREAM_ENTRY_GRAB_PULSE_LENS && urh_iq_bytes(dtype) == 0) return URH_ERR_DTYPE;
    if ((entry & URH_STREAM_PSK) && (entry & 0xf) != URH_STREAM_ENTRY_AFP_DEMOD && (entry & 0xf) != URH_STREAM_ENTRY_DEMOD_DIGITIZE)
        return URH_ERR_INVALID;
    const StreamSizes z = stream_sizes(n, dtype, tolerance, chunk_samples, ring, entry);
    const bool digitize = (entry & 0xf) != URH_STREAM_ENTRY_AFP_DEMOD;
    const int64_t r = rows == -2 ? n / 64 + 1024 : (rows < 0 ? rows_bound(n, tolerance) : rows);
    if (entry & URH_STREAM_RESIDENT) {
        const int64_t ntiles = urh_div_up(n, URH_TILE);
        int64_t b = z.ring_bytes + ((int64_t)64 << 20);
        if (digitize)
            b += r256(ntiles * (int64_t)sizeof(UrhTileSummary)) + r256(ntiles * (int64_t)stage_cap_for(tolerance) * 4) +
                 finish_arena_bytes(ntiles, r + r / 4, true) + 16 * (r + r / 4);
        if ((entry & 0xf) == URH_STREAM_ENTRY_DEMOD_CENTER_DIGITIZE)
            b += r256(ntiles * (int64_t)sizeof(UrhTileStats)) + r256((int64_t)URH_FINE_SLABS * URH_FINE_NB * 4) + r256((ntiles + 1) * 8);
        if (psk_order_of(entry)) b += urh_costas_arena_bytes(n, psk_order_of(entry));
        *bytes = b;
        return URH_OK;
    }
    int64_t b = z.ring_bytes;
    b += 2 * z.arena + ((int64_t)64 << 20);
    const int64_t nb = 2 * (z.scan_items / 256 + 1);
    b += 256 + (nb > 8192 ? nb : 8192) * (4 + 2 * 32);
    if (digitize) b += 3 * 16 * (r + z.rows_chunk);
    *bytes = b;
    return URH_OK;
}

extern "C" int urh_stream_stats(urh_ctx* ctx, int64_t* h_out3) {
    h_out3[0] = ctx->stream_free_low;
    h_out3[1] = ctx->stream_chunks;
    h_out3[2] = (int64_t)ctx->arena_peak;
    return URH_OK;
}

struct StreamDigitizer {
    UrhTileSummary* tiles;
    uint32_t* staging;
    int16_t* d_init;
    UrhChain* chain;
    int cap, tol;
    bool is_ask;
    uint32_t sps;
    int64_t n, rows, rows_all;
    UrhArenaMark mark;
    int init(urh_ctx* ctx, int64_t n_total, int64_t cs, int tolerance, bool ask, uint32_t samples_per_symbol) {
        n = n_total; tol = tolerance; is_ask = ask; sps = samples_per_symbol; rows = 0;
        cap = stage_cap_for(tol);
        rows_all = rows_bound(n, tol);
        const int64_t ct = cs / URH_TILE;
        URH_CHECK(urh_arena(ctx, (size_t)ct, &tiles));
        URH_CHECK(urh_arena(ctx, (size_t)ct * cap, &staging));
        URH_CHECK(urh_arena(ctx, 8, &d_init));
        URH_CHECK(urh_arena(ctx, 1, &chain));
        URH_CUDA(ctx, cudaMemsetAsync(d_init, 0, 16, ctx->stream));
        mark = urh_arena_mark(ctx);
        return URH_OK;
    }
    int finish(urh_ctx* ctx, int64_t s0, int64_t s1) {
        const int64_t rc = rows_bound(s1 - s0, tol);
        const int64_t need = rows + rc;
        if (need > (int64_t)ctx->pulses_cap_rows) {
            int64_t grow = 2 * (int64_t)ctx->pulses_cap_rows;
            if (grow > rows_all + rc) grow = rows_all + rc;
            URH_CHECK(urh_ensure_pulses_keep(ctx, (size_t)(grow > need ? grow : need), (size_t)rows));
        }
        urh_arena_release(ctx, mark);
        int64_t kc = 0;
        URH_CHECK(urh_finish_chunk(ctx, s1 - s0, tol, is_ask, sps, tiles, staging, cap, d_init, chain, s0, n, rows, rc, &kc));
        urh_stream_sample_free(ctx);
        rows += kc;
        return URH_OK;
    }
};

static int stream_check(urh_ctx* ctx, int64_t n, int ring, int mod_type, int dtype, bool iq);
static int psk_stream_check(urh_ctx* ctx, int64_t n, int ring, int dtype) {
    URH_CHECK(stream_check(ctx, n, ring, URH_MOD_PSK, dtype, false));
    if (n <= 2) URH_FAIL(ctx, URH_ERR_INVALID, "streamed PSK demodulation: n > 2");
    if (urh_iq_bytes(dtype) == 0) URH_FAIL(ctx, URH_ERR_DTYPE, "Unsupported dtype");
    return URH_OK;
}

static int stream_check(urh_ctx* ctx, int64_t n, int ring, int mod_type, int dtype, bool iq) {
    if (n <= 0) URH_FAIL(ctx, URH_ERR_INVALID, "streamed call: empty capture");
    if (ring < 2 || ring > URH_STREAM_MAX_RING) URH_FAIL(ctx, URH_ERR_INVALID, "streamed call: ring of %d slots (2..%d)", ring, URH_STREAM_MAX_RING);
    if (iq && (n <= 2 || (mod_type != URH_MOD_ASK && mod_type != URH_MOD_FSK)))
        URH_FAIL(ctx, URH_ERR_INVALID, "streamed demodulation: ASK/FSK and n > 2 (PSK is a serial recurrence)");
    if (iq && urh_iq_bytes(dtype) == 0) URH_FAIL(ctx, URH_ERR_DTYPE, "Unsupported dtype");
    return URH_OK;
}

template <bool DIG>
static int stream_dense_iq(urh_ctx* ctx, int dtype, int mod_type, const char* d_src, int64_t src_slot, int64_t n, const UrhDemodParams& dp,
                           float* qad_global, const UrhClassify& cls, int tol, StreamDigitizer* dz, int64_t s0, int64_t s1, int s,
                           UrhTileStats* ts = nullptr, const UrhFine& fine = UrhFine{}) {
    const int b = urh_iq_bytes(dtype);
    const void* iq = d_src + s * src_slot + URH_STREAM_PAD - s0 * b;
    const int64_t t0 = s0 / URH_TILE, t1 = urh_div_up(s1, URH_TILE);
    UrhTileSummary* tiles = dz ? dz->tiles - t0 : nullptr;
    uint32_t* staging = dz ? dz->staging - t0 * dz->cap : nullptr;
    const int cap = dz ? dz->cap : 0;
    int16_t* init = dz ? dz->d_init : nullptr;
    const int c0 = DIG ? host_classify(0.0f, cls) : 0;
    if (mod_type == URH_MOD_ASK)
        return launch_dense_iq_m<URH_MOD_ASK, DIG>(ctx, dtype, iq, n, dp, qad_global, cls, tol, tiles, staging, cap, init, c0, 0, ts, t0, t1, fine);
    return launch_dense_iq_m<URH_MOD_FSK, DIG>(ctx, dtype, iq, n, dp, qad_global, cls, tol, tiles, staging, cap, init, c0, 0, ts, t0, t1, fine);
}

static int stream_dense_qad(urh_ctx* ctx, const float* x, int64_t s0, int64_t s1, const UrhClassify& cls, StreamDigitizer& dz,
                            const float* d_thr0 = nullptr, const UrhTileStats* ts = nullptr) {
    const int64_t nc = s1 - s0;
    const unsigned grid = (unsigned)urh_div_up(urh_div_up(nc, URH_TILE), URH_WARPS_PER_BLOCK);
    const int vec_in = (((uintptr_t)x % 8) == 0) ? 1 : 0;
    int16_t* init = s0 == 0 ? dz.d_init : nullptr;
    const int c0 = d_thr0 ? 0 : host_classify(0.0f, cls);
    const UrhTileStats* tsc = ts ? ts + s0 / URH_TILE : nullptr;
    if (cls.order == 2)
        URH_LAUNCH(ctx, (k_dense_f32<SrcQad2, float>), grid, URH_WARPS_PER_BLOCK * 32, 0, x, nc, vec_in, cls, dz.tol, dz.tiles, dz.staging,
                   dz.cap, init, c0, d_thr0, tsc);
    else
        URH_LAUNCH(ctx, (k_dense_f32<SrcQad, float>), grid, URH_WARPS_PER_BLOCK * 32, 0, x, nc, vec_in, cls, dz.tol, dz.tiles, dz.staging,
                   dz.cap, init, c0, d_thr0, tsc);
    return URH_OK;
}

struct CenterPlan;
int urh_center_chain(urh_ctx* ctx, const float* d_qad, int64_t n, const UrhTileStats* ts, int64_t max_size, int rank, int world,
                     const UrhFine* fine, CenterPlan** d_plan_out);
int urh_center_plan_result(urh_ctx* ctx, const CenterPlan* plan, const float** d_centerf, const double** d_center, const int** d_state);
int urh_center_plan_certify_stats(urh_ctx* ctx, const CenterPlan* plan, int64_t* h_dst3);

extern "C" int urh_shard_digitize(urh_ctx* ctx, const void* d_iq, int dtype, const float* d_qad_in, int64_t n, int has_halo,
                                  float noise_mag, int mod_type, float center, uint16_t tolerance, uint32_t samples_per_symbol,
                                  uint8_t bits_per_symbol, float center_spacing, float* d_qad_out, int64_t global_offset,
                                  int64_t n_total, int64_t* k) {
    if (!k) return URH_ERR_INVALID;
    *k = 0;
    ctx->pulses_k = 0;
    if (n <= 0) URH_FAIL(ctx, URH_ERR_INVALID, "empty shard");
    if (mod_type != URH_MOD_ASK && mod_type != URH_MOD_FSK) URH_FAIL(ctx, URH_ERR_INVALID, "sharded path: ASK / FSK only");
    if (!d_qad_in && urh_iq_bytes(dtype) == 0) URH_FAIL(ctx, URH_ERR_DTYPE, "Unsupported dtype");
    if (!ctx->nccl_comm) URH_FAIL(ctx, URH_ERR_INVALID, "NCCL communicator not initialised (urh_nccl_init)");
    urh_arena_reset(ctx);
    UrhClassify cls;
    URH_CHECK(fill_classify(ctx, &cls, mod_type, center, bits_per_symbol, center_spacing));
    const int tol = tolerance;
    const int64_t ntiles = urh_div_up(n, URH_TILE);
    const int cap = stage_cap_for(tol);
    UrhTileSummary* tiles;
    uint32_t* staging;
    int16_t* d_init;
    URH_CHECK(urh_arena(ctx, (size_t)ntiles, &tiles));
    URH_CHECK(urh_arena(ctx, (size_t)ntiles * cap, &staging));
    URH_CHECK(urh_arena(ctx, 8, &d_init));
    URH_CUDA(ctx, cudaMemsetAsync(d_init, 0, 16, ctx->stream));
    const int c0 = host_classify(0.0f, cls);
    if (d_qad_in) {
        const int vec_in = (((uintptr_t)d_qad_in % 8) == 0) ? 1 : 0;
        const unsigned grid = (unsigned)urh_div_up(ntiles, URH_WARPS_PER_BLOCK);
        URH_PROF_BEGIN(ctx);
        if (cls.order == 2)
            URH_LAUNCH(ctx, (k_dense_f32<SrcQad2, float>), grid, URH_WARPS_PER_BLOCK * 32, 0, d_qad_in, n, vec_in, cls, tol, tiles, staging, cap,
                       d_init, c0, (const float*)nullptr);
        else
            URH_LAUNCH(ctx, (k_dense_f32<SrcQad, float>), grid, URH_WARPS_PER_BLOCK * 32, 0, d_qad_in, n, vec_in, cls, tol, tiles, staging, cap,
                       d_init, c0, (const float*)nullptr);
        URH_PROF_END(ctx);
    } else {
        const UrhDemodParams dp = make_demod_params(noise_mag, mod_type, dtype);
        if (mod_type == URH_MOD_ASK)
            URH_CHECK((launch_dense_iq_m<URH_MOD_ASK, true>(ctx, dtype, d_iq, n, dp, d_qad_out, cls, tol, tiles, staging, cap, d_init, c0, has_halo)));
        else
            URH_CHECK((launch_dense_iq_m<URH_MOD_FSK, true>(ctx, dtype, d_iq, n, dp, d_qad_out, cls, tol, tiles, staging, cap, d_init, c0, has_halo)));
    }
    return urh_finish_shard(ctx, n, tol, mod_type == URH_MOD_ASK, samples_per_symbol, tiles, staging, cap, d_init, global_offset, n_total, k);
}

struct StreamCenter {
    int ring;
    int64_t chunk_samples;
    const void* h_iq;
    float* h_qad;
    int64_t* kept;
};
static int demod_center_digitize_impl(urh_ctx* ctx, const void* d_iq, int dtype, int64_t n, int has_halo, float noise_mag, int mod_type,
                                      uint16_t tolerance, uint32_t samples_per_symbol, int64_t max_size, float* d_qad_out, bool sharded,
                                      int64_t global_offset, int64_t n_total, double* center, int* center_state, int64_t* k,
                                      const void* h_iq = nullptr, int64_t chunk_samples = 0, const StreamCenter* sc = nullptr) {
    if (!k || !center || !center_state) return URH_ERR_INVALID;
    *k = 0;
    *center = 0.0;
    *center_state = 0;
    ctx->pulses_k = 0;
    if (n <= 2 || (mod_type != URH_MOD_ASK && mod_type != URH_MOD_FSK) || !d_qad_out)
        URH_FAIL(ctx, URH_ERR_INVALID, "demod_center_digitize: ASK/FSK, n > 2 and a qad buffer are required");
    if (urh_iq_bytes(dtype) == 0) URH_FAIL(ctx, URH_ERR_DTYPE, "Unsupported dtype");
    if (sharded && !ctx->nccl_comm) URH_FAIL(ctx, URH_ERR_INVALID, "NCCL communicator not initialised (urh_nccl_init)");
    urh_arena_reset(ctx);
    URH_TL_RESET(ctx);
    URH_TL_MARK(ctx, "step start");
    const UrhDemodParams dp = make_demod_params(noise_mag, mod_type, dtype);
    UrhClassify cls;
    memset(&cls, 0, sizeof(cls));
    const int64_t ntiles = urh_div_up(n, URH_TILE);
    UrhTileStats* ts;
    URH_CHECK(urh_arena(ctx, (size_t)ntiles, &ts));
    const bool no_certify = getenv("URH_B200_CENTER_NO_CERTIFY") != nullptr;
    UrhFine fine = {};
    if (!sharded && !no_certify) {
        fine.slab_tiles = urh_div_up(ntiles, URH_FINE_SLABS);
        if (fine.slab_tiles < URH_WARPS_PER_BLOCK) fine.slab_tiles = URH_WARPS_PER_BLOCK;
        const int64_t nslabs = urh_div_up(ntiles, fine.slab_tiles);
        URH_CHECK(urh_arena(ctx, (size_t)(nslabs * URH_FINE_NB), &fine.gh));
        URH_CUDA(ctx, cudaMemsetAsync(fine.gh, 0, (size_t)(nslabs * URH_FINE_NB) * sizeof(unsigned int), ctx->stream));
        fine.scale = (mod_type == URH_MOD_FSK) ? 512.0f : 4096.0f;
        fine.off = (mod_type == URH_MOD_FSK) ? 2048.0f : 0.0f;
    }
    const int64_t chunk_tiles = (h_iq && chunk_samples > 0) ? (chunk_samples >= URH_TILE ? chunk_samples / URH_TILE : 1) : ntiles;
    const size_t sample_bytes = (size_t)urh_iq_bytes(dtype);
    StreamRing ring;
    int64_t scs = 0;
    if (sc) {
        const StreamSizes z = stream_sizes(n, dtype, tolerance, sc->chunk_samples, sc->ring, URH_STREAM_ENTRY_DEMOD_CENTER_DIGITIZE);
        scs = z.cs;
        URH_CHECK(ring.init(ctx, sc->ring, sc->ring * r256(z.src_slot)));
        const int64_t slot = r256(z.src_slot);
        URH_CHECK(stream_run(ctx, n, scs, ring, (const char*)sc->h_iq, urh_iq_bytes(dtype), true, ring.mem, slot, sc->h_qad, d_qad_out,
                             [&](int64_t, int64_t s0, int64_t s1, int s) {
                                 return stream_dense_iq<false>(ctx, dtype, mod_type, ring.mem, slot, n, dp, d_qad_out, cls, 0, nullptr, s0, s1, s,
                                                               ts, fine);
                             }, true));
    }
    cls.noise_value = urh_noise_value(mod_type);
    cls.order = 2;
    const int tol = tolerance;
    const int cap = stage_cap_for(tol);
    UrhTileSummary* tiles = nullptr;
    uint32_t* staging = nullptr;
    int16_t* d_init = nullptr;
    if (!sc) {
        URH_CHECK(urh_arena(ctx, (size_t)ntiles, &tiles));
        URH_CHECK(urh_arena(ctx, (size_t)ntiles * cap, &staging));
        URH_CHECK(urh_arena(ctx, 8, &d_init));
    }
    const bool speculate = !sharded && !h_iq && !sc && mod_type == URH_MOD_FSK && dtype == URH_DT_F32 &&
                           getenv("URH_B200_NO_SPECULATE") == nullptr;
    UrhSpec spec = {};
    if (speculate) {
        float* tg;
        URH_CHECK(urh_arena(ctx, 1, &tg));
        URH_CHECK(urh_arena(ctx, 1, &spec.redone));
        URH_CHECK(urh_arena(ctx, (size_t)ntiles, &spec.margin));
        spec.tg = tg;
        const char* forced = getenv("URH_B200_SPECULATE_GUESS");
        URH_LAUNCH(ctx, k_speculate_guess, 1, URH_GUESS_THREADS, 0, (const float2*)d_iq, n, dp.noise_sqrd, forced ? 1 : 0,
                   forced ? strtof(forced, nullptr) : 0.0f, tg, spec.redone);
    }
    int chunk_no = 0;
    for (int64_t t0 = 0; t0 < (sc ? 0 : ntiles); t0 += chunk_tiles, chunk_no++) {
        const int64_t t1 = (t0 + chunk_tiles < ntiles) ? t0 + chunk_tiles : ntiles;
        if (h_iq) {
            const int64_t s0 = t0 * URH_TILE, s1 = (t1 * URH_TILE < n) ? t1 * URH_TILE : n;
            cudaEvent_t ev = ctx->ev_copy[chunk_no & 1];
            URH_CUDA(ctx, cudaMemcpyAsync((char*)d_iq + (size_t)s0 * sample_bytes, (const char*)h_iq + (size_t)s0 * sample_bytes,
                                          (size_t)(s1 - s0) * sample_bytes, cudaMemcpyHostToDevice, ctx->copy_stream[0]));
            URH_CUDA(ctx, cudaEventRecord(ev, ctx->copy_stream[0]));
            URH_CUDA(ctx, cudaStreamWaitEvent(ctx->stream, ev, 0));
        }
        if (mod_type == URH_MOD_ASK)
            URH_CHECK((launch_dense_iq_m<URH_MOD_ASK, false>(ctx, dtype, d_iq, n, dp, d_qad_out, cls, 0, nullptr, nullptr, 0, nullptr, 0, has_halo, ts, t0, t1, fine)));
        else
            URH_CHECK((launch_dense_iq_m<URH_MOD_FSK, false>(ctx, dtype, d_iq, n, dp, d_qad_out, cls, tol, tiles, staging, cap, nullptr, 0, has_halo,
                                                             ts, t0, t1, fine, speculate ? &spec : nullptr)));
    }
    CenterPlan* plan = nullptr;
    URH_CHECK(urh_center_chain(ctx, d_qad_out, n, ts, max_size, sharded ? ctx->nccl_rank : 0, sharded ? ctx->nccl_world : 1,
                               fine.gh ? &fine : nullptr, &plan));
    const float* d_centerf;
    const double* d_center;
    const int* d_state;
    urh_center_plan_result(ctx, plan, &d_centerf, &d_center, &d_state);
    int64_t rows = 0;
    if (sc) {
        URH_CUDA(ctx, cudaMemcpyAsync(ctx->h_mail + 40, d_center, sizeof(double), cudaMemcpyDeviceToHost, ctx->stream));
        URH_CUDA(ctx, cudaMemcpyAsync(ctx->h_mail + 41, d_state, sizeof(int), cudaMemcpyDeviceToHost, ctx->stream));
        URH_CHECK(urh_center_plan_certify_stats(ctx, plan, ctx->h_mail + 42));
        URH_CUDA(ctx, cudaMemcpyAsync(ctx->h_mail + 45, (const int64_t*)ctx->center_prefix + ntiles, sizeof(int64_t), cudaMemcpyDeviceToHost,
                                      ctx->stream));
        URH_CUDA(ctx, cudaStreamSynchronize(ctx->stream));
        int st0 = 0;
        memcpy(&st0, ctx->h_mail + 41, sizeof(int));
        if (st0 == 1) {
            StreamDigitizer dz;
            URH_CHECK(dz.init(ctx, n, scs, tol, mod_type == URH_MOD_ASK, samples_per_symbol));
            for (int64_t s0 = 0; s0 < n; s0 += scs) {
                const int64_t s1 = s0 + scs < n ? s0 + scs : n;
                URH_CHECK(stream_dense_qad(ctx, d_qad_out + s0, s0, s1, cls, dz, d_centerf, ts));
                URH_CHECK(dz.finish(ctx, s0, s1));
            }
            rows = dz.rows;
        }
        *sc->kept = ctx->h_mail[45];
    } else {
        URH_CUDA(ctx, cudaMemsetAsync(d_init, 0, 16, ctx->stream));
        const int vec_in = (((uintptr_t)d_qad_out % 8) == 0) ? 1 : 0;
        int64_t grid = urh_div_up(ntiles, URH_WARPS_PER_BLOCK);
        if (speculate) {
            int per_sm = 0;
            URH_CUDA(ctx, cudaOccupancyMaxActiveBlocksPerMultiprocessor(&per_sm, k_dense_f32<SrcQad2, float>, URH_WARPS_PER_BLOCK * 32, 0));
            const int64_t resident = (int64_t)ctx->sm_count * (per_sm > 0 ? per_sm : 1);
            if (grid > resident) grid = resident;
        }
        URH_LAUNCH(ctx, (k_dense_f32<SrcQad2, float>), (unsigned)grid, URH_WARPS_PER_BLOCK * 32, 0,
                   (const float*)d_qad_out, n, vec_in, cls, tol, tiles, staging, cap, d_init, 0, d_centerf, (const UrhTileStats*)ts, spec);
        URH_CUDA(ctx, cudaMemcpyAsync(ctx->h_mail + 40, d_center, sizeof(double), cudaMemcpyDeviceToHost, ctx->stream));
        URH_CUDA(ctx, cudaMemcpyAsync(ctx->h_mail + 41, d_state, sizeof(int), cudaMemcpyDeviceToHost, ctx->stream));
        URH_CHECK(urh_center_plan_certify_stats(ctx, plan, ctx->h_mail + 42));
        ctx->h_mail[46] = 0;
        if (speculate) URH_CUDA(ctx, cudaMemcpyAsync(ctx->h_mail + 46, spec.redone, sizeof(unsigned int), cudaMemcpyDeviceToHost, ctx->stream));
        if (sharded)
            URH_CHECK(urh_finish_shard(ctx, n, tol, mod_type == URH_MOD_ASK, samples_per_symbol, tiles, staging, cap, d_init, global_offset, n_total, &rows));
        else
            URH_CHECK(urh_finish_local(ctx, n, tol, mod_type == URH_MOD_ASK, samples_per_symbol, tiles, staging, cap, d_init, &rows));
    }
    memcpy(center, ctx->h_mail + 40, sizeof(double));
    int st = 0;
    memcpy(&st, ctx->h_mail + 41, sizeof(int));
    *center_state = st;
    ctx->center_cert[0] = ctx->h_mail[42];
    ctx->center_cert[1] = fine.gh ? URH_FINE_NB : 0;
    ctx->center_cert[2] = ctx->h_mail[44];
    const int64_t redone = (spec.hi > spec.lo) ? ctx->h_mail[46] : 0;
    ctx->spec_stats[0] = spec.hi - spec.lo;
    ctx->spec_stats[1] = spec.hi - spec.lo - redone;
    ctx->spec_stats[2] = redone;
    if (st != 1) {
        ctx->pulses_k = 0;
        rows = 0;
    }
    *k = rows;
    return URH_OK;
}

extern "C" int urh_speculate_stats(urh_ctx* ctx, int64_t* h_out3) {
    for (int i = 0; i < 3; i++) h_out3[i] = ctx->spec_stats[i];
    return URH_OK;
}

extern "C" int urh_demod_center_digitize(urh_ctx* ctx, const void* d_iq, int dtype, int64_t n, float noise_mag, int mod_type,
                                         uint16_t tolerance, uint32_t samples_per_symbol, int64_t max_size, float* d_qad_out,
                                         double* center, int* center_state, int64_t* k) {
    return demod_center_digitize_impl(ctx, d_iq, dtype, n, 0, noise_mag, mod_type, tolerance, samples_per_symbol, max_size, d_qad_out, false,
                                      0, n, center, center_state, k);
}

extern "C" int urh_demod_center_digitize_host(urh_ctx* ctx, const void* h_iq, int dtype, int64_t n, float noise_mag, int mod_type,
                                              uint16_t tolerance, uint32_t samples_per_symbol, int64_t max_size, int64_t chunk_samples,
                                              void* d_iq_scratch, float* d_qad_out, double* center, int* center_state, int64_t* k) {
    if (!h_iq || !d_iq_scratch) return URH_ERR_INVALID;
    URH_CUDA(ctx, cudaEventRecord(ctx->ev_comp[0], ctx->stream));
    URH_CUDA(ctx, cudaStreamWaitEvent(ctx->copy_stream[0], ctx->ev_comp[0], 0));
    return demod_center_digitize_impl(ctx, d_iq_scratch, dtype, n, 0, noise_mag, mod_type, tolerance, samples_per_symbol, max_size, d_qad_out,
                                      false, 0, n, center, center_state, k, h_iq, chunk_samples > 0 ? chunk_samples : ((int64_t)1 << 24));
}

extern "C" int urh_shard_demod_center_digitize_host(urh_ctx* ctx, const void* h_iq, int dtype, int64_t n, int has_halo, float noise_mag,
                                                    int mod_type, uint16_t tolerance, uint32_t samples_per_symbol, int64_t max_size,
                                                    int64_t chunk_samples, void* d_iq_scratch, float* d_qad_out, int64_t global_offset,
                                                    int64_t n_total, double* center, int* center_state, int64_t* k) {
    if (!h_iq || !d_iq_scratch) return URH_ERR_INVALID;
    URH_CUDA(ctx, cudaEventRecord(ctx->ev_comp[0], ctx->stream));
    URH_CUDA(ctx, cudaStreamWaitEvent(ctx->copy_stream[0], ctx->ev_comp[0], 0));
    return demod_center_digitize_impl(ctx, d_iq_scratch, dtype, n, has_halo, noise_mag, mod_type, tolerance, samples_per_symbol, max_size,
                                      d_qad_out, true, global_offset, n_total, center, center_state, k, h_iq,
                                      chunk_samples > 0 ? chunk_samples : ((int64_t)1 << 24));
}

extern "C" int urh_shard_demod_center_digitize(urh_ctx* ctx, const void* d_iq, int dtype, int64_t n, int has_halo, float noise_mag,
                                               int mod_type, uint16_t tolerance, uint32_t samples_per_symbol, int64_t max_size,
                                               float* d_qad_out, int64_t global_offset, int64_t n_total, double* center,
                                               int* center_state, int64_t* k) {
    return demod_center_digitize_impl(ctx, d_iq, dtype, n, has_halo, noise_mag, mod_type, tolerance, samples_per_symbol, max_size, d_qad_out,
                                      true, global_offset, n_total, center, center_state, k);
}

extern "C" int urh_afp_demod_stream(urh_ctx* ctx, const void* h_iq, int dtype, int64_t n, float noise_mag, int mod_type, int64_t chunk_samples,
                                    int ring, float* h_qad) {
    if (!h_iq || !h_qad) return URH_ERR_INVALID;
    URH_CHECK(stream_check(ctx, n, ring, mod_type, dtype, true));
    urh_arena_reset(ctx);
    const StreamSizes z = stream_sizes(n, dtype, 0, chunk_samples, ring, URH_STREAM_ENTRY_AFP_DEMOD);
    StreamRing R;
    URH_CHECK(R.init(ctx, ring, z.ring_bytes));
    char* d_src = R.mem;
    float* d_qad = (float*)(R.mem + ring * r256(z.src_slot));
    const UrhDemodParams dp = make_demod_params(noise_mag, mod_type, dtype);
    UrhClassify cls;
    memset(&cls, 0, sizeof(cls));
    return stream_run(ctx, n, z.cs, R, (const char*)h_iq, urh_iq_bytes(dtype), true, d_src, r256(z.src_slot), h_qad, d_qad,
                      [&](int64_t, int64_t s0, int64_t s1, int s) {
                          return stream_dense_iq<false>(ctx, dtype, mod_type, d_src, r256(z.src_slot), n, dp, d_qad + s * z.cs - s0, cls, 0,
                                                        nullptr, s0, s1, s);
                      });
}

extern "C" int urh_grab_pulse_lens_stream(urh_ctx* ctx, const float* qad, int qad_on_device, int64_t n, float center, uint16_t tolerance,
                                          int mod_type, uint32_t samples_per_symbol, uint8_t bits_per_symbol, float center_spacing,
                                          int64_t chunk_samples, int ring, int64_t* k) {
    if (!k || !qad) return URH_ERR_INVALID;
    *k = 0;
    ctx->pulses_k = 0;
    URH_CHECK(stream_check(ctx, n, ring, mod_type, 0, false));
    urh_arena_reset(ctx);
    UrhClassify cls;
    URH_CHECK(fill_classify(ctx, &cls, mod_type, center, bits_per_symbol, center_spacing));
    const StreamSizes z = stream_sizes(n, 0, tolerance, chunk_samples, ring,
                                       URH_STREAM_ENTRY_GRAB_PULSE_LENS | (qad_on_device ? URH_STREAM_QAD_ON_DEVICE : 0));
    StreamRing R;
    URH_CHECK(R.init(ctx, ring, z.ring_bytes));
    StreamDigitizer dz;
    URH_CHECK(dz.init(ctx, n, z.cs, tolerance, mod_type == URH_MOD_ASK, samples_per_symbol));
    char* d_src = R.mem;
    URH_CHECK(stream_run(ctx, n, z.cs, R, qad_on_device ? nullptr : (const char*)qad, 4, false, d_src, r256(z.src_slot), nullptr, nullptr,
                         [&](int64_t, int64_t s0, int64_t s1, int s) {
                             const float* x = qad_on_device ? qad + s0 : (const float*)(d_src + s * r256(z.src_slot) + URH_STREAM_PAD);
                             URH_CHECK(stream_dense_qad(ctx, x, s0, s1, cls, dz));
                             return dz.finish(ctx, s0, s1);
                         }));
    *k = dz.rows;
    return URH_OK;
}

extern "C" int urh_demod_digitize_stream(urh_ctx* ctx, const void* h_iq, int dtype, int64_t n, float noise_mag, int mod_type, float center,
                                         uint16_t tolerance, uint32_t samples_per_symbol, uint8_t bits_per_symbol, float center_spacing,
                                         int64_t chunk_samples, int ring, float* h_qad_out, int64_t* k) {
    if (!k || !h_iq) return URH_ERR_INVALID;
    *k = 0;
    ctx->pulses_k = 0;
    URH_CHECK(stream_check(ctx, n, ring, mod_type, dtype, true));
    urh_arena_reset(ctx);
    UrhClassify cls;
    URH_CHECK(fill_classify(ctx, &cls, mod_type, center, bits_per_symbol, center_spacing));
    const UrhDemodParams dp = make_demod_params(noise_mag, mod_type, dtype);
    const StreamSizes z = stream_sizes(n, dtype, tolerance, chunk_samples, ring,
                                       URH_STREAM_ENTRY_DEMOD_DIGITIZE | (h_qad_out ? URH_STREAM_QAD_OUT : 0));
    StreamRing R;
    URH_CHECK(R.init(ctx, ring, z.ring_bytes));
    StreamDigitizer dz;
    URH_CHECK(dz.init(ctx, n, z.cs, tolerance, mod_type == URH_MOD_ASK, samples_per_symbol));
    char* d_src = R.mem;
    float* d_qad = h_qad_out ? (float*)(R.mem + ring * r256(z.src_slot)) : nullptr;
    URH_CHECK(stream_run(ctx, n, z.cs, R, (const char*)h_iq, urh_iq_bytes(dtype), true, d_src, r256(z.src_slot), h_qad_out, d_qad,
                         [&](int64_t, int64_t s0, int64_t s1, int s) {
                             URH_CHECK(stream_dense_iq<true>(ctx, dtype, mod_type, d_src, r256(z.src_slot), n, dp,
                                                             d_qad ? d_qad + s * z.cs - s0 : nullptr, cls, tolerance, &dz, s0, s1, s));
                             return dz.finish(ctx, s0, s1);
                         }));
    *k = dz.rows;
    return URH_OK;
}

extern "C" int urh_demod_center_digitize_stream(urh_ctx* ctx, const void* h_iq, int dtype, int64_t n, float noise_mag, int mod_type,
                                                uint16_t tolerance, uint32_t samples_per_symbol, int64_t max_size, int64_t chunk_samples,
                                                int ring, float* d_qad_out, float* h_qad_out, double* center, int* center_state,
                                                int64_t* kept, int64_t* k) {
    if (!h_iq || !d_qad_out || !kept) return URH_ERR_INVALID;
    URH_CHECK(stream_check(ctx, n, ring, mod_type, dtype, true));
    StreamCenter sc;
    sc.ring = ring; sc.chunk_samples = chunk_samples; sc.h_iq = h_iq; sc.h_qad = h_qad_out; sc.kept = kept;
    return demod_center_digitize_impl(ctx, nullptr, dtype, n, 0, noise_mag, mod_type, tolerance, samples_per_symbol, max_size, d_qad_out,
                                      false, 0, n, center, center_state, k, nullptr, 0, &sc);
}

extern "C" int urh_afp_demod_psk_stream(urh_ctx* ctx, const void* h_iq, int dtype, int64_t n, float noise_mag, int mod_order,
                                        float costas_loop_bandwidth, int64_t chunk_samples, int ring, float* h_qad) {
    if (!h_iq || !h_qad) return URH_ERR_INVALID;
    URH_CHECK(psk_stream_check(ctx, n, ring, dtype));
    urh_arena_reset(ctx);
    const StreamSizes z = stream_sizes(n, dtype, 0, chunk_samples, ring, URH_STREAM_ENTRY_AFP_DEMOD | psk_entry_flags(mod_order));
    StreamRing R;
    URH_CHECK(R.init(ctx, ring, z.ring_bytes));
    const int64_t slot = r256(z.src_slot);
    char* d_src = R.mem;
    float* d_qad = (float*)(R.mem + ring * slot);
    const UrhDemodParams dp = make_demod_params(noise_mag, URH_MOD_PSK, dtype);
// ... 187 lines not shown
```

### urh_b200/csrc/finish.cu

```cuda
#include "sparse.cuh"
#include "tilescan.cuh"

#include <limits.h>

#define CLS_NONE INT_MIN

struct __align__(16) CandAgg {
    int64_t cnt;
    int32_t last_cls;
    int32_t pad;
};
struct CandOp {
    __device__ __forceinline__ CandAgg operator()(const CandAgg& a, const CandAgg& b) const {
        CandAgg r;
        r.cnt = a.cnt + b.cnt;
        r.last_cls = (b.last_cls != CLS_NONE) ? b.last_cls : a.last_cls;
        r.pad = 0;
        return r;
    }
};
struct __align__(16) FireAgg {
    int64_t fired;
    int64_t last_pos;
};
// ... 27 lines not shown
    int32_t first_cls;
    int32_t first_rel;
    int32_t fired;
    int32_t last_rel;
};
struct ScanCandidates {
    const UrhTileSummary* tiles;
    const uint32_t* staging;
    int stage_cap;
    const RunCarry* carry;
    const RunCarry* xcarry;
    int tol;
    int32_t* head_rel;
    int32_t* prev_cls;
    TileFire* fire;
    __device__ __forceinline__ CandAgg load(int64_t t) const {
        const UrhTileSummary s = tiles[t];
        RunCarry c = carry[t];
        if (xcarry) c = RunCarryOp()(*xcarry, c);
        int64_t start_len = 0;
        if (!(c.flags & 2) && c.cls == s.first_cls) start_len = c.len;
        int32_t rel = -1;
        if (start_len <= tol && (int64_t)tol < start_len + s.head_len) rel = (int32_t)(tol - start_len);
        head_rel[t] = rel;
        TileFire f;
        f.first_cls = CLS_NONE; f.first_rel = -1; f.fired = 0; f.last_rel = -1;
        int prev = CLS_NONE;
        if (rel >= 0) {
            prev = s.first_cls;
            f.first_cls = prev;
            f.first_rel = rel;
        }
        const uint32_t* st = staging + t * (int64_t)stage_cap;
        for (int j = 0; j < s.ncand; j += 4) {
            uint32_t w[4];
#pragma unroll
            for (int u = 0; u < 4; u++) w[u] = (j + u < s.ncand) ? st[j + u] : 0u;
#pragma unroll
            for (int u = 0; u < 4; u++) {
                if (j + u < s.ncand) {
                    const int cl = (int)(w[u] & 0xffffu) - 1;
                    const int p = (int)(w[u] >> 16);
                    if (prev == CLS_NONE) {
                        f.first_cls = cl;
                        f.first_rel = p;
                    } else if (cl != prev) {
                        f.fired++;
                        f.last_rel = p;
                    }
                    prev = cl;
                }
            }
        }
        fire[t] = f;
        CandAgg r;
        r.cnt = (int64_t)s.ncand + (rel >= 0 ? 1 : 0);
        r.last_cls = prev;
        r.pad = 0;
        return r;
    }
    __device__ __forceinline__ void post(int64_t t, const CandAgg& excl, const CandAgg&) const { prev_cls[t] = excl.last_cls; }
};

struct ScanFirings {
    const TileFire* fire;
    const int32_t* prev_cls;
    const int16_t* d_prev0;
    int64_t global_offset;
    int64_t* row_off;
    int64_t* prev_fired;
    __device__ __forceinline__ FireAgg load(int64_t t) const {
        const TileFire f = fire[t];
        int prev = prev_cls[t];
        if (prev == CLS_NONE) prev = *d_prev0;
        FireAgg r;
        r.fired = f.fired;
        int32_t last = f.last_rel;
        if (f.first_cls != CLS_NONE && f.first_cls != prev) {
            r.fired++;
            if (last < 0) last = f.first_rel;
        }
        r.last_pos = (last >= 0) ? t * URH_TILE + global_offset + last : -1;
        return r;
    }
    __device__ __forceinline__ void post(int64_t t, const FireAgg& excl, const FireAgg&) const {
        row_off[t] = excl.fired;
        prev_fired[t] = excl.last_pos;
    }
};

constexpr int FIN_TILES = 32;
constexpr int FIN_BATCH = 8;

struct FinRows {
    int64_t* out;
    int64_t cap_rows;
    int tol;
    int is_ask;
    int64_t sps;
};

struct FinWalk {
    int prev;
    int64_t pp;
    int64_t idx;
};

__device__ __forceinline__ void fin_row(const FinRows& R, int64_t idx, int64_t p, int64_t pp, int prev) {
    const int64_t rec = (pp >= 0) ? (p - pp) : (p + 1 - R.tol);
    int64_t st = prev;
    if (R.is_ask && st == -1 && rec < R.sps) st = 0;
    if (idx < R.cap_rows) *((longlong2*)R.out + idx) = make_longlong2(st, rec);
}

__device__ __forceinline__ void fin_chunk(FinWalk& W, uint32_t w, int cnt, int lane, int64_t base, const FinRows& R) {
    const int c = (int)(w & 0xffffu) - 1;
    const int rel = (int)(w >> 16);
    int pc = __shfl_up_sync(URH_FULL_MASK, c, 1);
    if (lane == 0) pc = W.prev;
    const bool fire = lane < cnt && c != pc;
    const unsigned fm = __ballot_sync(URH_FULL_MASK, fire);
    const unsigned lower = fm & ((1u << lane) - 1u);
    const int before = __shfl_sync(URH_FULL_MASK, rel, lower ? 31 - __clz(lower) : 0);
    if (fire) fin_row(R, W.idx + __popc(lower), base + rel, lower ? base + before : W.pp, pc);
    if (fm) W.pp = base + __shfl_sync(URH_FULL_MASK, rel, 31 - __clz(fm));
    W.idx += __popc(fm);
    if (cnt > 0) W.prev = __shfl_sync(URH_FULL_MASK, c, cnt - 1);
}

__global__ void __launch_bounds__(256) k_finish_rows(const UrhTileSummary* __restrict__ tiles, const uint32_t* __restrict__ staging,
                                                    int stage_cap, const int32_t* __restrict__ head_rel, const int32_t* __restrict__ prev_cls,
                                                    const int16_t* __restrict__ d_prev0, const int64_t* __restrict__ row_off,
                                                    const int64_t* __restrict__ prev_fired, const int64_t* __restrict__ d_xprev_fired,
                                                    int64_t ntiles, int64_t global_offset, int64_t n_total, int tol, int is_ask, int64_t sps,
                                                    int emit_tail, int64_t row_base, int64_t* __restrict__ out, int64_t cap_rows,
                                                    int64_t* __restrict__ d_out) {
    const int64_t t0 = ((int64_t)blockIdx.x * blockDim.x + threadIdx.x) / 32 * FIN_TILES;
    if (t0 >= ntiles) return;
    const int lane = threadIdx.x & 31;
    FinRows R;
    R.out = out; R.cap_rows = cap_rows; R.tol = tol; R.is_ask = is_ask; R.sps = sps;
    const int64_t tl = t0 + lane;
    int l_first = 0, l_ncand = 0, l_rel = -1, l_prev = 0;
    int64_t l_idx = 0, l_pp = -1;
    if (tl < ntiles) {
        const UrhTileSummary s = tiles[tl];
        l_first = s.first_cls;
        l_ncand = s.ncand;
        l_rel = head_rel[tl];
        l_prev = prev_cls[tl];
        if (l_prev == CLS_NONE) l_prev = *d_prev0;
        l_idx = row_off[tl];
        l_pp = prev_fired[tl];
        if (l_pp < 0) l_pp = *d_xprev_fired;
    }
    for (int j0 = 0; j0 < FIN_TILES && t0 + j0 < ntiles; j0 += FIN_BATCH) {
        uint32_t w0[FIN_BATCH];
#pragma unroll
        for (int u = 0; u < FIN_BATCH; u++) {
            const int nc = __shfl_sync(URH_FULL_MASK, l_ncand, j0 + u);
            w0[u] = (lane < nc) ? __ldg(staging + (t0 + j0 + u) * (int64_t)stage_cap + lane) : 0u;
        }
#pragma unroll
        for (int u = 0; u < FIN_BATCH; u++) {
            const int j = j0 + u;
            const int64_t t = t0 + j;
            if (t >= ntiles) break;
            const int64_t base = t * URH_TILE + global_offset;
            const int ncand = __shfl_sync(URH_FULL_MASK, l_ncand, j);
            const int rel = __shfl_sync(URH_FULL_MASK, l_rel, j);
            FinWalk W;
            W.prev = __shfl_sync(URH_FULL_MASK, l_prev, j);
            W.pp = __shfl_sync(URH_FULL_MASK, l_pp, j);
            W.idx = __shfl_sync(URH_FULL_MASK, l_idx, j);
            if (rel >= 0) {
                const int c = __shfl_sync(URH_FULL_MASK, l_first, j);
                if (c != W.prev) {
                    if (lane == 0) fin_row(R, W.idx, base + rel, W.pp, W.prev);
                    W.idx++;
                    W.pp = base + rel;
                }
                W.prev = c;
            }
            const uint32_t* st = staging + t * (int64_t)stage_cap;
            for (int k = 0; k < ncand; k += 32) {
                const uint32_t w = (k == 0) ? w0[u] : ((k + lane < ncand) ? __ldg(st + k + lane) : 0u);
                fin_chunk(W, w, min(32, ncand - k), lane, base, R);
            }
            if (t == ntiles - 1 && lane == 0) {
                int64_t idx = W.idx;
                const int64_t fired = idx;
                if (emit_tail && (is_ask || row_base + fired < n_total)) {
                    if (idx < cap_rows) *((longlong2*)out + idx) = make_longlong2(W.prev, (W.pp >= 0) ? (n_total - 1 - W.pp) : (n_total - tol));
                    idx++;
                }
                d_out[0] = idx;
                d_out[1] = fired;
            }
        }
    }
}

struct ScanMergeRows {
    const int64_t* raw;
    int64_t rows;
    int64_t n_total;
    int has_tail;
    int64_t* out;
    int64_t* d_k;
    const int64_t* prev_last;
    int64_t row_base;
    __device__ __forceinline__ int64_t load(int64_t r) const {
        if (r == 0) return (prev_last && raw[0] == *prev_last) ? 0 : 1;
        return raw[2 * r] != raw[2 * r - 2] ? 1 : 0;
    }
    __device__ __forceinline__ void post(int64_t r, const int64_t& excl, const int64_t& head) const {
        const bool is_tail = has_tail && r == rows - 1;
        if (is_tail && row_base + excl >= n_total) {
            *d_k = excl;
            return;
        }
        const int64_t o = excl + head - 1;
        if (head) out[2 * o] = raw[2 * r];
        atomicAdd((unsigned long long*)&out[2 * o + 1], (unsigned long long)raw[2 * r + 1]);
        if (r == rows - 1) *d_k = o + 1;
    }
};
struct AddI64 {
    __device__ __forceinline__ int64_t operator()(int64_t a, int64_t b) const { return a + b; }
};

__global__ void k_pack_stage1(const int16_t* __restrict__ d_init, const RunCarry* __restrict__ total, int64_t* __restrict__ msg) {
    memcpy(msg, total, sizeof(RunCarry));
    msg[2] = *d_init;
    msg[3] = 0;
}
__global__ void k_fold_carry(const int64_t* __restrict__ all, int rank, RunCarry* __restrict__ xcarry) {
    RunCarry acc;
    acc.len = 0; acc.cls = 0; acc.flags = 2 | 1;
    for (int q = 0; q < rank; q++) {
        RunCarry c;
        memcpy(&c, all + 4 * q, sizeof(c));
        acc = RunCarryOp()(acc, c);
    }
    if (rank == 0) acc.flags = 2;
    else acc.flags &= ~1;
    *xcarry = acc;
}
__global__ void k_fold_prev_cls(const int64_t* __restrict__ all, int rank, const int64_t* __restrict__ stage1, int16_t* __restrict__ prev0) {
    int v = (int)stage1[2];
    for (int q = 0; q < rank; q++) {
        CandAgg c;
        memcpy(&c, all + 2 * q, sizeof(c));
        if (c.last_cls != CLS_NONE) v = c.last_cls;
    }
    *prev0 = (int16_t)v;
}
__global__ void k_fold_prev_fired(const int64_t* __restrict__ all, int rank, int64_t* __restrict__ xprev) {
    int64_t v = -1;
    for (int q = 0; q < rank; q++) {
        FireAgg c;
        memcpy(&c, all + 2 * q, sizeof(c));
        if (c.last_pos >= 0) v = c.last_pos;
    }
    *xprev = v;
}

__global__ void k_chain_start(const int16_t* __restrict__ d_init, UrhChain* __restrict__ chain) {
    chain->run.len = 0; chain->run.cls = 0; chain->run.flags = 2 | 1;
    chain->prev_fired = -1;
    chain->last_state = INT64_MIN;
    chain->prev_cls = *d_init;
}
__global__ void k_chain_advance(UrhChain* __restrict__ chain, const RunCarry* __restrict__ tot_run, const CandAgg* __restrict__ tot_cand,
                                const FireAgg* __restrict__ tot_fire) {
    chain->run = RunCarryOp()(chain->run, *tot_run);
    if (tot_cand->last_cls != CLS_NONE) chain->prev_cls = (int16_t)tot_cand->last_cls;
    if (tot_fire->last_pos >= 0) chain->prev_fired = tot_fire->last_pos;
}
__global__ void k_chain_last_row(UrhChain* __restrict__ chain, const int64_t* __restrict__ table, int64_t rows) {
    if (rows > 0) chain->last_state = table[2 * (rows - 1)];
}

int urh_coll_allgather(urh_ctx* ctx, const void* d_send, void* d_recv, size_t bytes_per_rank);
extern "C" int urh_p2p_check(urh_ctx* ctx);

struct FinishShard {
    int rank, world;
    int64_t global_offset;
    int64_t n_total;
    int emit_tail;
    UrhChain* chain;
    int64_t row_base, rows_cap;
};

static int finish_tiles(urh_ctx* ctx, int64_t n, int tol, bool is_ask, uint32_t sps, const UrhTileSummary* tiles, const uint32_t* staging,
                        int stage_cap, const int16_t* d_init, const FinishShard& sh, int64_t* k) {
    const int64_t ntiles = urh_div_up(n, URH_TILE);
    const bool sharded = sh.world > 1;
    UrhChain* chain = sh.chain;
    RunCarry* carry;
    int32_t *head_rel, *prev_cls;
    int64_t *row_off, *prev_fired, *d_small;
    URH_CHECK(urh_arena(ctx, (size_t)ntiles, &carry));
    URH_CHECK(urh_arena(ctx, (size_t)ntiles, &head_rel));
    URH_CHECK(urh_arena(ctx, (size_t)ntiles, &prev_cls));
    URH_CHECK(urh_arena(ctx, (size_t)ntiles, &row_off));
    URH_CHECK(urh_arena(ctx, (size_t)ntiles, &prev_fired));
    TileFire* fire;
    URH_CHECK(urh_arena(ctx, (size_t)ntiles, &fire));
    URH_CHECK(urh_arena(ctx, (size_t)(32 + 8 * (sharded ? sh.world : 0)), &d_small));
    URH_CUDA(ctx, cudaMemsetAsync(d_small, 0xff, 4 * sizeof(int64_t), ctx->stream));
    RunCarry* d_tot_run = (RunCarry*)(d_small + 4);
    CandAgg* d_tot_cand = (CandAgg*)(d_small + 6);
    FireAgg* d_tot_fire = (FireAgg*)(d_small + 8);
    RunCarry* d_xcarry = (RunCarry*)(d_small + 10);
    int16_t* d_prev0 = (int16_t*)(d_small + 12);
    int64_t* d_xprev = d_small + 13;
    int64_t* d_msg1 = d_small + 16;
    int64_t* d_all1 = d_small + 32;
    int64_t* d_all2 = d_all1 + 4 * (sharded ? sh.world : 0);
    int64_t* d_all3 = d_all2 + 2 * (sharded ? sh.world : 0);

    if (chain && sh.global_offset == 0) URH_LAUNCH(ctx, k_chain_start, 1, 1, 0, d_init, chain);
    RunCarry rc_ident;
    rc_ident.len = 0; rc_ident.cls = 0; rc_ident.flags = 2 | 1;
    ScanRunCarry fa;
    fa.tiles = tiles; fa.n = n; fa.carry = carry;
    URH_CHECK((urhts::scan<RunCarry, RunCarryOp, ScanRunCarry>(ctx, ntiles, rc_ident, RunCarryOp(), fa, d_tot_run)));
    if (sharded) {
        URH_LAUNCH(ctx, k_pack_stage1, 1, 1, 0, d_init, (const RunCarry*)d_tot_run, d_msg1);
        URH_TL_MARK(ctx, "x4 run carry: enter");
        URH_CHECK(urh_coll_allgather(ctx, d_msg1, d_all1, 4 * sizeof(int64_t)));
        URH_TL_MARK(ctx, "x4 run carry: done");
        URH_LAUNCH(ctx, k_fold_carry, 1, 1, 0, (const int64_t*)d_all1, sh.rank, d_xcarry);
    }
    ScanCandidates fb;
    fb.tiles = tiles; fb.staging = staging; fb.stage_cap = stage_cap; fb.carry = carry;
    fb.xcarry = sharded ? d_xcarry : (chain ? &chain->run : nullptr);
    fb.tol = tol; fb.head_rel = head_rel; fb.prev_cls = prev_cls; fb.fire = fire;
    CandAgg ca_ident;
    ca_ident.cnt = 0; ca_ident.last_cls = CLS_NONE; ca_ident.pad = 0;
    URH_CHECK((urhts::scan<CandAgg, CandOp, ScanCandidates, 4>(ctx, ntiles, ca_ident, CandOp(), fb, d_tot_cand)));
    const int16_t* prev0 = chain ? &chain->prev_cls : d_init;
    if (sharded) {
        URH_TL_MARK(ctx, "x5 candidates: enter");
        URH_CHECK(urh_coll_allgather(ctx, d_tot_cand, d_all2, sizeof(CandAgg)));
        URH_TL_MARK(ctx, "x5 candidates: done");
        URH_LAUNCH(ctx, k_fold_prev_cls, 1, 1, 0, (const int64_t*)d_all2, sh.rank, (const int64_t*)d_all1, d_prev0);
        prev0 = d_prev0;
    }
    ScanFirings fc;
    fc.fire = fire; fc.prev_cls = prev_cls; fc.d_prev0 = prev0; fc.global_offset = sh.global_offset; fc.row_off = row_off;
    fc.prev_fired = prev_fired;
    FireAgg fi_ident;
    fi_ident.fired = 0; fi_ident.last_pos = -1;
    URH_CHECK((urhts::scan<FireAgg, FireOp, ScanFirings>(ctx, ntiles, fi_ident, FireOp(), fc, d_tot_fire)));
    const int64_t* xprev = chain ? &chain->prev_fired : d_small + 2;
    if (sharded) {
        URH_TL_MARK(ctx, "x6 firings: enter");
        URH_CHECK(urh_coll_allgather(ctx, d_tot_fire, d_all3, sizeof(FireAgg)));
        URH_TL_MARK(ctx, "x6 firings: done");
        URH_LAUNCH(ctx, k_fold_prev_fired, 1, 1, 0, (const int64_t*)d_all3, sh.rank, d_xprev);
        xprev = d_xprev;
    }

    int64_t cap_rows = (int64_t)ctx->pulses_cap_rows;
    const int64_t guess = n / 64 + 1024;
    if (!chain && cap_rows < guess) {
        URH_CHECK(urh_ensure_pulses(ctx, (size_t)guess));
        cap_rows = (int64_t)ctx->pulses_cap_rows;
    }
    const int64_t row_base = chain ? sh.row_base : 0;
    int64_t* raw = ctx->pulses + 2 * row_base;
    int64_t raw_cap = chain ? sh.rows_cap : cap_rows;
    if (is_ask) URH_CHECK(urh_arena(ctx, (size_t)raw_cap * 2, &raw));
    int64_t got[2] = {0, 0};
    for (int attempt = 0; attempt < 2; attempt++) {
        URH_LAUNCH(ctx, k_finish_rows, (unsigned)urh_div_up(ntiles, 8 * FIN_TILES), 256, 0, tiles, staging, stage_cap, (const int32_t*)head_rel,
                   (const int32_t*)prev_cls, prev0, (const int64_t*)row_off, (const int64_t*)prev_fired, xprev, ntiles, sh.global_offset,
                   sh.n_total, tol, is_ask ? 1 : 0, (int64_t)sps, sh.emit_tail, row_base, raw, raw_cap, d_small);
        if (sharded && attempt == 0) URH_TL_MARK(ctx, "rows written");
        URH_CHECK(urh_read_i64(ctx, d_small, 2, got));
        if (sharded) URH_CHECK(urh_p2p_check(ctx));
        if (got[0] <= raw_cap) break;
        if (attempt == 1 || chain) URH_FAIL(ctx, URH_ERR_CUDA, "finish_tiles: row buffer overflow after regrowth");
        if (is_ask) {
            URH_CHECK(urh_arena(ctx, (size_t)got[0] * 2, &raw));
            raw_cap = got[0];
        } else {
            URH_CHECK(urh_ensure_pulses(ctx, (size_t)got[0]));
            raw = ctx->pulses;
            raw_cap = (int64_t)ctx->pulses_cap_rows;
        }
    }
    if (chain) URH_LAUNCH(ctx, k_chain_advance, 1, 1, 0, chain, (const RunCarry*)d_tot_run, (const CandAgg*)d_tot_cand, (const FireAgg*)d_tot_fire);
    int64_t K = got[0];
    if (is_ask && K > 0) {
        if (!chain) URH_CHECK(urh_ensure_pulses(ctx, (size_t)K));
        int64_t* out = ctx->pulses + 2 * row_base;
        URH_CUDA(ctx, cudaMemsetAsync(out, 0, (size_t)K * 2 * sizeof(int64_t), ctx->stream));
        ScanMergeRows fm;
        fm.raw = raw; fm.rows = K; fm.n_total = sh.n_total; fm.has_tail = (sh.emit_tail && K > got[1]) ? 1 : 0; fm.out = out;
        fm.d_k = d_small;
        fm.prev_last = (chain && row_base > 0) ? &chain->last_state : nullptr;
        fm.row_base = row_base;
        URH_CHECK((urhts::scan<int64_t, AddI64, ScanMergeRows>(ctx, K, (int64_t)0, AddI64(), fm, (int64_t*)nullptr)));
        URH_CHECK(urh_read_i64(ctx, d_small, 1, &K));
        if (chain) URH_LAUNCH(ctx, k_chain_last_row, 1, 1, 0, chain, (const int64_t*)ctx->pulses, row_base + K);
    }
    ctx->pulses_k = row_base + K;
    *k = K;
    return URH_OK;
}

int urh_finish_chunk(urh_ctx* ctx, int64_t n, int tol, bool is_ask, uint32_t sps, const UrhTileSummary* tiles, const uint32_t* staging,
                     int stage_cap, const int16_t* d_init, UrhChain* chain, int64_t global_offset, int64_t n_total, int64_t row_base,
                     int64_t rows_cap, int64_t* k) {
    FinishShard sh;
    sh.rank = 0; sh.world = 1; sh.global_offset = global_offset; sh.n_total = n_total;
    sh.emit_tail = (global_offset + n == n_total) ? 1 : 0;
    sh.chain = chain; sh.row_base = row_base; sh.rows_cap = rows_cap;
    return finish_tiles(ctx, n, tol, is_ask, sps, tiles, staging, stage_cap, d_init, sh, k);
}

int urh_finish_local(urh_ctx* ctx, int64_t n, int tol, bool is_ask, uint32_t sps, const UrhTileSummary* tiles, const uint32_t* staging,
                     int stage_cap, const int16_t* d_init, int64_t* k) {
    FinishShard sh;
    sh.rank = 0; sh.world = 1; sh.global_offset = 0; sh.n_total = n; sh.emit_tail = 1;
    sh.chain = nullptr; sh.row_base = 0; sh.rows_cap = 0;
    return finish_tiles(ctx, n, tol, is_ask, sps, tiles, staging, stage_cap, d_init, sh, k);
}

int urh_finish_shard(urh_ctx* ctx, int64_t n, int tol, bool is_ask, uint32_t sps, const UrhTileSummary* tiles, const uint32_t* staging,
                     int stage_cap, const int16_t* d_init, int64_t global_offset, int64_t n_total, int64_t* k) {
    FinishShard sh;
    sh.rank = ctx->nccl_rank; sh.world = ctx->nccl_world; sh.global_offset = global_offset; sh.n_total = n_total;
    sh.emit_tail = (ctx->nccl_rank == ctx->nccl_world - 1) ? 1 : 0;
    sh.chain = nullptr; sh.row_base = 0; sh.rows_cap = 0;
    return finish_tiles(ctx, n, tol, is_ask, sps, tiles, staging, stage_cap, d_init, sh, k);
}
```

Measured before the change: 213,500.

## Fold center-ranks into window kernel, parallelize fine histogram totals, batch result readback

Merges the single-thread rank kernel into the window kernel. The rank-to-tile binary search now runs as a block-parallel 256-way search. The per-slab fine-histogram totals move out of the single-block certify kernel into the window-ends kernel, which accumulates them with striped atomics. The two templated interior-histogram launches become one kernel that branches at runtime, and scattered small device-to-host copies are replaced by a single device record array read once. A side stream and events are added. The intent is fewer launches, fewer syncs and less serial work, at the cost of extra atomics and more complicated plumbing.

```diff
diff --git a/urh_b200/csrc/center.cu b/urh_b200/csrc/center.cu
--- a/urh_b200/csrc/center.cu
+++ b/urh_b200/csrc/center.cu
@@ -520,7 +520,6 @@
     float scale;
     int fast;
     int state;
-    unsigned int ticket;
     int certified;
     long long straddle;
     long long pad;
@@ -536,54 +535,58 @@
     __device__ __forceinline__ int64_t operator()(int64_t a, int64_t b) const { return a + b; }
 };
 
-__global__ void k_center_ranks(const int64_t* __restrict__ counts, int rank, int world, int64_t max_size, CenterPlan* __restrict__ plan) {
+__device__ __forceinline__ int64_t cen_tile_of_rank(const int64_t* __restrict__ prefix, int64_t ntiles, int64_t r) {
+    int64_t lo = 0, hi = ntiles;
+    while (hi - lo > 1) {
+        const int64_t step = urh_div_up(hi - lo, 256), p = lo + (int64_t)threadIdx.x * step;
+        const int below = __syncthreads_count(p < hi && prefix[p] <= r);
+        lo += (int64_t)(below - 1) * step;
+        hi = min(lo + step, hi);
+    }
+    return lo;
+}
+
+__global__ void __launch_bounds__(256) k_center_window(const float* __restrict__ x, int64_t n, const UrhTileStats* __restrict__ ts,
+                                                      const int64_t* __restrict__ prefix, int64_t ntiles, const int64_t* __restrict__ counts,
+                                                      int rank, int world, int64_t max_size, CenterPlan* __restrict__ plan,
+                                                      CenStats* __restrict__ partial, unsigned long long* __restrict__ ticket,
+                                                      unsigned long long ticket_base) {
+    __shared__ long long s_win[4];
+    __shared__ int s_pre[256];
+    __shared__ bool s_last;
     long long total = 0, offset = 0;
     for (int q = 0; q < world; q++) {
         if (q < rank) offset += counts[q];
         total += counts[q];
     }
     const long long kept = counts[rank];
-    long long r0 = (long long)(0.05 * (double)total), r1 = (long long)(0.95 * (double)total);
-    if (max_size >= 0 && r1 - r0 > max_size) r1 = r0 + max_size;
-    plan->total = total; plan->offset = offset; plan->r0 = r0; plan->r1 = r1;
-    long long a = r0 - offset, b = r1 - offset;
-    a = a < 0 ? 0 : (a > kept ? kept : a);
-    b = b < 0 ? 0 : (b > kept ? kept : b);
-    plan->lr0 = a; plan->lr1 = b;
-    plan->ticket = 0u;
-    plan->state = 1;
-    plan->certified = 0;
-    plan->straddle = 0;
-}
-
-__device__ __forceinline__ int64_t cen_tile_of_rank(const int64_t* __restrict__ prefix, int64_t ntiles, int64_t r) {
-    int64_t lo = 0, hi = ntiles;
-    while (hi - lo > 1) {
-        const int64_t mid = (lo + hi) >> 1;
-        if (prefix[mid] <= r) lo = mid; else hi = mid;
-    }
-    return lo;
-}
-
-__global__ void __launch_bounds__(256) k_center_window(const float* __restrict__ x, int64_t n, const UrhTileStats* __restrict__ ts,
-                                                      const int64_t* __restrict__ prefix, int64_t ntiles, CenterPlan* __restrict__ plan,
-                                                      CenStats* __restrict__ partial) {
-    __shared__ long long s_win[4];
-    __shared__ int s_pre[256];
-    __shared__ bool s_last;
-    const long long r0 = plan->lr0, r1 = plan->lr1;
+    long long g0 = (long long)(0.05 * (double)total), g1 = (long long)(0.95 * (double)total);
+    if (max_size >= 0 && g1 - g0 > max_size) g1 = g0 + max_size;
+    long long r0 = g0 - offset, r1 = g1 - offset;
+    r0 = r0 < 0 ? 0 : (r0 > kept ? kept : r0);
+    r1 = r1 < 0 ? 0 : (r1 > kept ? kept : r1);
+    int64_t w0 = -1, w1 = -1;
+    if (r1 > r0) {
+        w0 = cen_tile_of_rank(prefix, ntiles, r0);
+        w1 = cen_tile_of_rank(prefix, ntiles, r1 - 1);
+    }
     if (threadIdx.x == 0) {
-        long long w0 = -1, w1 = -1, w2 = -1, w3 = -1;
+        long long w2 = -1, w3 = -1;
         if (r1 > r0) {
-            w0 = cen_tile_of_rank(prefix, ntiles, r0);
-            w1 = cen_tile_of_rank(prefix, ntiles, r1 - 1);
             const bool cov0 = prefix[w0] >= r0 && prefix[w0 + 1] <= r1;
             const bool cov1 = prefix[w1] >= r0 && prefix[w1 + 1] <= r1;
             w2 = cov0 ? -1 : w0;
             w3 = (cov1 || w1 == w0) ? -1 : w1;
         }
         s_win[0] = w0; s_win[1] = w1; s_win[2] = w2; s_win[3] = w3;
-        if (blockIdx.x == 0) { plan->win[0] = w0; plan->win[1] = w1; plan->win[2] = w2; plan->win[3] = w3; }
+        if (blockIdx.x == 0) {
+            plan->win[0] = w0; plan->win[1] = w1; plan->win[2] = w2; plan->win[3] = w3;
+            plan->total = total; plan->offset = offset; plan->r0 = g0; plan->r1 = g1;
+            plan->lr0 = r0; plan->lr1 = r1;
+            plan->state = 1;
+            plan->certified = 0;
+            plan->straddle = 0;
+        }
     }
     __syncthreads();
     double sum = 0.0, sq = 0.0;
@@ -623,7 +626,7 @@
     }
     __threadfence();
     __syncthreads();
-    if (threadIdx.x == 0) s_last = atomicAdd(&plan->ticket, 1u) == gridDim.x - 1;
+    if (threadIdx.x == 0) s_last = atomicAdd(ticket, 1ull) - ticket_base == gridDim.x - 1;
     __syncthreads();
     if (!s_last) return;
     __threadfence();
@@ -643,7 +646,7 @@
 
 __global__ void __launch_bounds__(256) k_center_plan(const CenStats* __restrict__ parts, int world, CenterPlan* __restrict__ plan,
                                                     float* __restrict__ fe, unsigned long long* __restrict__ hist,
-                                                    unsigned long long* __restrict__ xhist) {
+                                                    unsigned long long* __restrict__ xhist, unsigned long long* __restrict__ ftot) {
     __shared__ int s_state;
     __shared__ long long s_nbins;
     __shared__ double s_hmin, s_edge1, s_delta;
@@ -693,6 +696,8 @@
     }
     __syncthreads();
     if (s_state != 1) return;
+    if (ftot)
+        for (int k = threadIdx.x; k < URH_FINE_NB; k += 256) ftot[k] = 0ull;
     const long long nbins = s_nbins;
     for (long long k = threadIdx.x; k <= nbins; k += 256) {
         const double e = (k == 0) ? s_hmin : (k == 1 ? s_edge1 : __dadd_rn(s_hmin, __dmul_rn((double)k, s_delta)));
@@ -708,13 +713,16 @@
     }
 }
 
-template <bool FAST>
 __global__ void __launch_bounds__(256, 3) k_hist_interior_dev(const float* __restrict__ x, int64_t n, const CenterPlan* __restrict__ plan,
                                                           const float* __restrict__ g_fe, unsigned long long* __restrict__ hist,
                                                           const int64_t* __restrict__ prefix) {
-    if (plan->state != 1 || plan->certified || (plan->fast != 0) != FAST) return;
-    hist_interior_body<true, FAST>(x, n, plan->win[0] + 1, plan->win[1], blockIdx.x, gridDim.x, g_fe, plan->scale, (int)plan->nbins, hist, 1,
-                                   prefix);
+    if (plan->state != 1 || plan->certified) return;
+    if (plan->fast)
+        hist_interior_body<true, true>(x, n, plan->win[0] + 1, plan->win[1], blockIdx.x, gridDim.x, g_fe, plan->scale, (int)plan->nbins, hist, 1,
+                                       prefix);
+    else
+        hist_interior_body<true, false>(x, n, plan->win[0] + 1, plan->win[1], blockIdx.x, gridDim.x, g_fe, plan->scale, (int)plan->nbins, hist,
+                                        1, prefix);
 }
 
 __device__ __forceinline__ void cen_full_slabs(int64_t win0, int64_t win1, int64_t slab_tiles, int64_t* sf, int64_t* se) {
@@ -722,10 +730,12 @@
     *se = win1 / slab_tiles;
 }
 
+#define CEN_FTOT_STRIPES 8
 __global__ void __launch_bounds__(256) k_hist_window_ends_dev(const float* __restrict__ x, int64_t n, const int64_t* __restrict__ prefix,
                                                              const CenterPlan* __restrict__ plan, const float* __restrict__ g_fe,
                                                              unsigned long long* __restrict__ hist, unsigned long long* __restrict__ xhist,
-                                                             int64_t slab_tiles) {
+                                                             int64_t slab_tiles, const unsigned int* __restrict__ gh,
+                                                             unsigned long long* __restrict__ ftot) {
     if (plan->state != 1) return;
     if (blockIdx.x < 2) {
         hist_window_ends_body(x, n, prefix, (const int64_t*)plan->win, plan->lr0, plan->lr1, g_fe, plan->scale, (int)plan->nbins, hist, xhist);
@@ -737,6 +747,12 @@
     int64_t a_end = w1, b_begin = w1;
     if (sf < se) { a_end = sf * slab_tiles; b_begin = se * slab_tiles; }
     const int blk = blockIdx.x - 2, nblk = gridDim.x - 2, nbins = (int)plan->nbins;
+    for (int64_t g = (int64_t)blk * 256 + threadIdx.x; g < (int64_t)URH_FINE_NB * CEN_FTOT_STRIPES; g += (int64_t)nblk * 256) {
+        const int bucket = (int)(g % URH_FINE_NB);
+        unsigned long long v = 0;
+        for (int64_t sl = sf + g / URH_FINE_NB; sl < se; sl += CEN_FTOT_STRIPES) v += gh[sl * URH_FINE_NB + bucket];
+        if (v) atomicAdd(ftot + bucket, v);
+    }
     const float scale = plan->scale;
     if (plan->fast) {
         hist_interior_body<true, true>(x, n, w0 + 1, a_end, blk, nblk, g_fe, scale, nbins, xhist, 1, prefix);
@@ -753,8 +769,8 @@
 
 #define CERT_THREADS 512
 __global__ void __launch_bounds__(CERT_THREADS) k_center_certify(const UrhFine fine, CenterPlan* __restrict__ plan, const float* __restrict__ fe,
-                                                                 const unsigned long long* __restrict__ xhist, unsigned long long* __restrict__ lo,
-                                                                 unsigned long long* __restrict__ hi) {
+                                                                 const unsigned long long* __restrict__ xhist, const unsigned long long* __restrict__ ftot,
+                                                                 unsigned long long* __restrict__ lo, unsigned long long* __restrict__ hi) {
     __shared__ unsigned long long s_ge[URH_FINE_NB + 1];
     __shared__ unsigned long long s_part[CERT_THREADS];
     __shared__ unsigned char s_flag[CEN_MAX_BINS];
@@ -763,15 +779,11 @@
     if (plan->state != 1) return;
     const int tid = threadIdx.x;
     constexpr int PER = URH_FINE_NB / CERT_THREADS;
-    int64_t sf, se;
-    cen_full_slabs(plan->win[0], plan->win[1], fine.slab_tiles, &sf, &se);
     unsigned long long b[PER], tot = 0;
 #pragma unroll
     for (int j = 0; j < PER; j++) {
-        unsigned long long v = 0;
-        for (int64_t sl = sf; sl < se; sl++) v += fine.gh[sl * URH_FINE_NB + tid * PER + j];
-        b[j] = v;
-        tot += v;
+        b[j] = ftot[tid * PER + j];
+        tot += b[j];
     }
     s_part[tid] = tot;
     if (tid < 3) s_key[tid] = 0ull;
@@ -847,7 +859,7 @@
     plan->certified = 1;
 }
 
-__global__ void __launch_bounds__(256) k_center_pick(const unsigned long long* __restrict__ y, CenterPlan* __restrict__ plan) {
+__device__ __forceinline__ void cen_pick(const unsigned long long* __restrict__ y, CenterPlan* __restrict__ plan) {
     __shared__ unsigned long long s_best[256];
     __shared__ int s_idx[256];
     __shared__ int s_cnt[256];
@@ -936,6 +948,18 @@
     plan->state = 1;
     (void)top_val;
 }
+__global__ void __launch_bounds__(256) k_center_pick(const unsigned long long* __restrict__ y, CenterPlan* __restrict__ plan,
+                                                     int64_t* __restrict__ record) {
+    cen_pick(y, plan);
+    if (threadIdx.x != 0 || !record) return;
+    long long c;
+    memcpy(&c, &plan->center, sizeof(c));
+    record[URH_REC_CENTER] = c;
+    record[URH_REC_STATE] = plan->state;
+    record[URH_REC_CERTIFIED] = plan->certified;
+    record[URH_REC_STRADDLE] = plan->straddle;
+    record[URH_REC_KEPT] = plan->total;
+}
 
 int urh_coll_allgather(urh_ctx* ctx, const void* d_send, void* d_recv, size_t bytes_per_rank);
 bool urh_p2p_usable(urh_ctx* ctx, size_t bytes_per_rank);
@@ -943,7 +967,7 @@
 extern "C" int urh_nccl_allreduce_i64(urh_ctx* ctx, int64_t* d_buf, int64_t count, int op);
 
 int urh_center_chain(urh_ctx* ctx, const float* d_qad, int64_t n, const UrhTileStats* ts, int64_t max_size, int rank, int world,
-                     const UrhFine* fine, CenterPlan** d_plan_out) {
+                     const UrhFine* fine, int64_t* record, CenterPlan** d_plan_out) {
     const int64_t ntiles = urh_div_up(n, URH_TILE);
     int64_t* prefix;
     CenterPlan* plan;
@@ -952,7 +976,7 @@
     unsigned long long* hist;
     int64_t* d_counts;
     CenStats* d_parts;
-    unsigned long long *xhist = nullptr, *cert_lo = nullptr, *cert_hi = nullptr;
+    unsigned long long *xhist = nullptr, *ftot = nullptr, *cert_lo = nullptr, *cert_hi = nullptr;
     const int nb = ctx->sm_count * 2;
     URH_CHECK(urh_arena(ctx, (size_t)ntiles + 1, &prefix));
     URH_CHECK(urh_arena(ctx, 1, &plan));
@@ -963,6 +987,7 @@
     URH_CHECK(urh_arena(ctx, (size_t)world, &d_parts));
     if (fine) {
         URH_CHECK(urh_arena(ctx, (size_t)CEN_MAX_BINS, &xhist));
+        URH_CHECK(urh_arena(ctx, (size_t)URH_FINE_NB, &ftot));
         URH_CHECK(urh_arena(ctx, (size_t)CEN_MAX_BINS, &cert_lo));
         URH_CHECK(urh_arena(ctx, (size_t)CEN_MAX_BINS, &cert_hi));
     }
@@ -976,8 +1001,10 @@
         URH_TL_MARK(ctx, "x1 kept counts: done");
         counts = d_counts;
     }
-    URH_LAUNCH(ctx, k_center_ranks, 1, 1, 0, counts, rank, world, max_size, plan);
-    URH_LAUNCH(ctx, k_center_window, nb, 256, 0, d_qad, n, ts, (const int64_t*)prefix, ntiles, plan, partial);
+    urhts::Ws ws;
+    URH_CHECK(urhts::prepare(ctx, nb, &ws));
+    URH_LAUNCH(ctx, k_center_window, nb, 256, 0, d_qad, n, ts, (const int64_t*)prefix, ntiles, counts, rank, world, max_size, plan, partial,
+               ws.counter, ws.base);
     const CenStats* parts = &plan->local;
     if (world > 1) {
         URH_TL_MARK(ctx, "x2 window partials: enter");
@@ -985,14 +1012,16 @@
         URH_TL_MARK(ctx, "x2 window partials: done");
         parts = d_parts;
     }
-    URH_LAUNCH(ctx, k_center_plan, 1, 256, 0, parts, world, plan, fe, hist, xhist);
+    URH_LAUNCH(ctx, k_center_plan, 1, 256, 0, parts, world, plan, fe, hist, xhist, ftot);
     const size_t dyn = (size_t)CEN_MAX_BINS * 4 + (size_t)(CEN_MAX_BINS + 3) * 4;
     const unsigned gs = (unsigned)min(urh_div_up(ntiles, 8), (int64_t)ctx->sm_count * 8);
     URH_LAUNCH(ctx, k_hist_window_ends_dev, fine ? 2 + ctx->sm_count * 4 : 2, 256, fine ? dyn : 0, d_qad, n, (const int64_t*)prefix,
-               (const CenterPlan*)plan, (const float*)fe, hist, xhist, fine ? fine->slab_tiles : (int64_t)1);
-    if (fine) URH_LAUNCH(ctx, k_center_certify, 1, CERT_THREADS, 0, *fine, plan, (const float*)fe, (const unsigned long long*)xhist, cert_lo, cert_hi);
-    URH_LAUNCH(ctx, (k_hist_interior_dev<true>), gs, 256, dyn, d_qad, n, (const CenterPlan*)plan, (const float*)fe, hist, (const int64_t*)prefix);
-    URH_LAUNCH(ctx, (k_hist_interior_dev<false>), gs, 256, dyn, d_qad, n, (const CenterPlan*)plan, (const float*)fe, hist, (const int64_t*)prefix);
+               (const CenterPlan*)plan, (const float*)fe, hist, xhist, fine ? fine->slab_tiles : (int64_t)1,
+               fine ? (const unsigned int*)fine->gh : nullptr, ftot);
+    if (fine)
+        URH_LAUNCH(ctx, k_center_certify, 1, CERT_THREADS, 0, *fine, plan, (const float*)fe, (const unsigned long long*)xhist,
+                   (const unsigned long long*)ftot, cert_lo, cert_hi);
+    URH_LAUNCH(ctx, k_hist_interior_dev, gs, 256, dyn, d_qad, n, (const CenterPlan*)plan, (const float*)fe, hist, (const int64_t*)prefix);
     const unsigned long long* hist_all = hist;
     if (world > 1) URH_TL_MARK(ctx, "x3 histogram sum: enter");
     if (world > 1) {
@@ -1006,7 +1035,7 @@
         }
     }
     if (world > 1) URH_TL_MARK(ctx, "x3 histogram sum: done");
-    URH_LAUNCH(ctx, k_center_pick, 1, 256, 0, hist_all, plan);
+    URH_LAUNCH(ctx, k_center_pick, 1, 256, 0, hist_all, plan, record);
     ctx->center_prefix = prefix;
     ctx->center_ts = ts;
     ctx->center_n = n;
@@ -1015,13 +1044,6 @@
     return URH_OK;
 }
 
-int urh_center_plan_certify_stats(urh_ctx* ctx, const CenterPlan* plan, int64_t* h_dst3) {
-    h_dst3[0] = h_dst3[1] = h_dst3[2] = 0;
-    URH_CUDA(ctx, cudaMemcpyAsync(h_dst3, &plan->certified, sizeof(int), cudaMemcpyDeviceToHost, ctx->stream));
-    URH_CUDA(ctx, cudaMemcpyAsync(h_dst3 + 2, &plan->straddle, sizeof(long long), cudaMemcpyDeviceToHost, ctx->stream));
-    return URH_OK;
-}
-
 extern "C" int urh_center_certify_stats(urh_ctx* ctx, int64_t* h_out3) {
     for (int i = 0; i < 3; i++) h_out3[i] = ctx->center_cert[i];
     return URH_OK;
diff --git a/urh_b200/csrc/common.cuh b/urh_b200/csrc/common.cuh
--- a/urh_b200/csrc/common.cuh
+++ b/urh_b200/csrc/common.cuh
@@ -20,6 +20,8 @@
     int sm_count;
     cudaStream_t stream;
     cudaStream_t copy_stream[2];
+    cudaStream_t side_stream;
+    cudaEvent_t ev_fork, ev_join;
     cudaEvent_t ev_start, ev_stop;
     cudaEvent_t ev_copy[2], ev_comp[2];
     cudaEvent_t ev_k0, ev_k1;
@@ -108,12 +110,13 @@
         return (code);                                            \
     } while (0)
 
-#define URH_LAUNCH(ctx, kernel, grid, block, smem, ...)                                   \
+#define URH_LAUNCH_ON(ctx, strm, kernel, grid, block, smem, ...)                          \
     do {                                                                                  \
-        kernel<<<(grid), (block), (smem), (ctx)->stream>>>(__VA_ARGS__);                  \
+        kernel<<<(grid), (block), (smem), (strm)>>>(__VA_ARGS__);                         \
         (ctx)->launches++;                                                                \
         URH_CUDA(ctx, cudaGetLastError());                                                \
     } while (0)
+#define URH_LAUNCH(ctx, kernel, grid, block, smem, ...) URH_LAUNCH_ON(ctx, (ctx)->stream, kernel, grid, block, smem, __VA_ARGS__)
 
 #define URH_TL_MARK(ctx, label) do { if ((ctx)->profiling >= 2 && (ctx)->tl_ready && (ctx)->tl_count < 32) { \
         (ctx)->tl_name[(ctx)->tl_count] = (label); cudaEventRecord((ctx)->tl_ev[(ctx)->tl_count++], (ctx)->stream); } } while (0)
@@ -156,6 +159,9 @@
 int urh_costas_stream_end(urh_ctx* ctx, const UrhCostasStream* S);
 int64_t urh_costas_arena_bytes(int64_t n, int loop_order);
 
+enum { URH_REC_ROWS, URH_REC_FIRED, URH_REC_CENTER, URH_REC_STATE, URH_REC_CERTIFIED, URH_REC_STRADDLE, URH_REC_REDONE, URH_REC_KEPT,
+       URH_REC_WORDS };
+
 int urh_read_i64(urh_ctx* ctx, const int64_t* d_src, int count, int64_t* h_out);
 
 __host__ __device__ static inline int64_t urh_div_up(int64_t a, int64_t b) { return (a + b - 1) / b; }
diff --git a/urh_b200/csrc/context.cu b/urh_b200/csrc/context.cu
--- a/urh_b200/csrc/context.cu
+++ b/urh_b200/csrc/context.cu
@@ -69,6 +69,11 @@
     bool ok = cudaStreamCreateWithFlags(&ctx->stream, cudaStreamNonBlocking) == cudaSuccess;
     ok = ok && cudaStreamCreateWithFlags(&ctx->copy_stream[0], cudaStreamNonBlocking) == cudaSuccess;
     ok = ok && cudaStreamCreateWithFlags(&ctx->copy_stream[1], cudaStreamNonBlocking) == cudaSuccess;
+    int prio_low = 0, prio_high = 0;
+    ok = ok && cudaDeviceGetStreamPriorityRange(&prio_low, &prio_high) == cudaSuccess;
+    ok = ok && cudaStreamCreateWithPriority(&ctx->side_stream, cudaStreamNonBlocking, prio_high) == cudaSuccess;
+    ok = ok && cudaEventCreateWithFlags(&ctx->ev_fork, cudaEventDisableTiming) == cudaSuccess;
+    ok = ok && cudaEventCreateWithFlags(&ctx->ev_join, cudaEventDisableTiming) == cudaSuccess;
     ok = ok && cudaEventCreate(&ctx->ev_start) == cudaSuccess && cudaEventCreate(&ctx->ev_stop) == cudaSuccess;
     for (int i = 0; i < 2 && ok; i++) {
         ok = ok && cudaEventCreateWithFlags(&ctx->ev_copy[i], cudaEventDisableTiming) == cudaSuccess;
@@ -110,6 +115,9 @@
         cudaEventDestroy(ctx->ev_comp[i]);
         cudaStreamDestroy(ctx->copy_stream[i]);
     }
+    cudaEventDestroy(ctx->ev_fork);
+    cudaEventDestroy(ctx->ev_join);
+    cudaStreamDestroy(ctx->side_stream);
     cudaStreamDestroy(ctx->stream);
     delete ctx;
 }
diff --git a/urh_b200/csrc/digitize.cu b/urh_b200/csrc/digitize.cu
--- a/urh_b200/csrc/digitize.cu
+++ b/urh_b200/csrc/digitize.cu
@@ -7,6 +7,7 @@
 #include "fsk_fast.cuh"
 #include "dense_f32.cuh"
 #include "stream_ring.cuh"
+#include "tilescan.cuh"
 
 #include <math.h>
 #include <stdlib.h>
@@ -164,30 +165,9 @@
 
 #define URH_GUESS_SAMPLES 16384
 #define URH_GUESS_BINS 128
-#define URH_GUESS_THREADS 1024
-__global__ void __launch_bounds__(URH_GUESS_THREADS) k_speculate_guess(const float2* __restrict__ iq, int64_t n, float noise_sqrd, int forced,
-                                                                      float forced_tg, float* __restrict__ d_tg, unsigned int* __restrict__ redone) {
-    constexpr int PER = URH_GUESS_SAMPLES / URH_GUESS_THREADS;
-    __shared__ unsigned int s_hist[URH_GUESS_BINS];
-    __shared__ float s_mn[32], s_mx[32];
-    if (forced) {
-        if (threadIdx.x == 0) { *d_tg = forced_tg; *redone = 0u; }
-        return;
-    }
-    for (int b = threadIdx.x; b < URH_GUESS_BINS; b += blockDim.x) s_hist[b] = 0u;
-    float v[PER];
-    float mn = INFINITY, mx = -INFINITY;
-#pragma unroll
-    for (int k = 0; k < PER; k++) {
-        const int64_t i = 1 + (int64_t)(k * URH_GUESS_THREADS + threadIdx.x) * (n - 1) / URH_GUESS_SAMPLES;
-        const float2 p = iq[i - 1], c = iq[i];
-        v[k] = NAN;
-        if (!(c.x * c.x + c.y * c.y <= noise_sqrd)) {
-            v[k] = atan2f(p.x * c.y - p.y * c.x, p.x * c.x + p.y * c.y);
-            mn = fminf(mn, v[k]);
-            mx = fmaxf(mx, v[k]);
-        }
-    }
+#define URH_GUESS_THREADS 256
+#define URH_GUESS_BLOCKS (URH_GUESS_SAMPLES / URH_GUESS_THREADS)
+__device__ __forceinline__ void guess_block_minmax(float& mn, float& mx, float* s_mn, float* s_mx) {
     for (int off = 16; off > 0; off >>= 1) {
         mn = fminf(mn, __shfl_xor_sync(URH_FULL_MASK, mn, off));
         mx = fmaxf(mx, __shfl_xor_sync(URH_FULL_MASK, mx, off));
@@ -196,31 +176,87 @@
     __syncthreads();
     mn = INFINITY; mx = -INFINITY;
     for (int w = 0; w < URH_GUESS_THREADS / 32; w++) { mn = fminf(mn, s_mn[w]); mx = fmaxf(mx, s_mx[w]); }
+}
+__global__ void __launch_bounds__(URH_GUESS_THREADS) k_speculate_guess(const float2* __restrict__ iq, int64_t n, float noise_sqrd, int forced,
+                                                                      float forced_tg, float* __restrict__ d_tg, unsigned int* __restrict__ redone,
+                                                                      int16_t* __restrict__ d_init, unsigned int* __restrict__ gh, int64_t gh_words,
+                                                                      float* __restrict__ vals, float2* __restrict__ mnmx,
+                                                                      unsigned long long* __restrict__ ticket, unsigned long long ticket_base) {
+    constexpr int PER = URH_GUESS_SAMPLES / URH_GUESS_THREADS;
+    __shared__ unsigned int s_hist[URH_GUESS_BINS];
+    __shared__ float s_mn[URH_GUESS_THREADS / 32], s_mx[URH_GUESS_THREADS / 32];
+    __shared__ unsigned long long s_top[2];
+    __shared__ bool s_last;
+    for (int64_t w = ((int64_t)blockIdx.x * URH_GUESS_THREADS + threadIdx.x) * 4; w < gh_words; w += (int64_t)gridDim.x * URH_GUESS_THREADS * 4)
+        *(uint4*)(gh + w) = make_uint4(0u, 0u, 0u, 0u);
+    float mn = INFINITY, mx = -INFINITY;
+    if (!forced) {
+        const int j = blockIdx.x * URH_GUESS_THREADS + threadIdx.x;
+        const int64_t i = 1 + (int64_t)j * (n - 1) / URH_GUESS_SAMPLES;
+        const float2 p = iq[i - 1], c = iq[i];
+        float v = NAN;
+        if (!(c.x * c.x + c.y * c.y <= noise_sqrd)) {
+            v = atan2f(p.x * c.y - p.y * c.x, p.x * c.x + p.y * c.y);
+            mn = fminf(mn, v);
+            mx = fmaxf(mx, v);
+        }
+        vals[j] = v;
+        guess_block_minmax(mn, mx, s_mn, s_mx);
+        if (threadIdx.x == 0) mnmx[blockIdx.x] = make_float2(mn, mx);
+    }
+    __threadfence();
+    __syncthreads();
+    if (threadIdx.x == 0) s_last = atomicAdd(ticket, 1ull) - ticket_base == gridDim.x - 1;
+    __syncthreads();
+    if (!s_last) return;
+    __threadfence();
+    if (forced) {
+        if (threadIdx.x == 0) { *d_tg = forced_tg; *redone = 0u; *d_init = 0; }
+        return;
+    }
+    for (int b = threadIdx.x; b < URH_GUESS_BINS; b += URH_GUESS_THREADS) s_hist[b] = 0u;
+    mn = INFINITY; mx = -INFINITY;
+    for (int b = threadIdx.x; b < (int)gridDim.x; b += URH_GUESS_THREADS) {
+        const float2 m = __ldcg(mnmx + b);
+        mn = fminf(mn, m.x);
+        mx = fmaxf(mx, m.y);
+    }
+    guess_block_minmax(mn, mx, s_mn, s_mx);
     const float width = (mx - mn) / URH_GUESS_BINS;
+    if (threadIdx.x < 2) s_top[threadIdx.x] = 0ull;
     if (width > 0.0f) {
-#pragma unroll
-        for (int k = 0; k < PER; k++)
-            if (!isnan(v[k])) atomicAdd(&s_hist[min((int)((v[k] - mn) / width), URH_GUESS_BINS - 1)], 1u);
+#pragma unroll 8
+        for (int k = 0; k < PER; k++) {
+            const float v = __ldcg(vals + k * URH_GUESS_THREADS + threadIdx.x);
+            const int bin = isnan(v) ? -1 : min((int)((v - mn) / width), URH_GUESS_BINS - 1);
+            const unsigned int same = __match_any_sync(URH_FULL_MASK, bin);
+            if (bin >= 0 && (threadIdx.x & 31) == __ffs(same) - 1) atomicAdd(&s_hist[bin], (unsigned int)__popc(same));
+        }
     }
     __syncthreads();
-    if (threadIdx.x != 0) return;
-    *redone = 0u;
-    if (!(mn <= mx)) { *d_tg = 0.0f; return; }
-    if (!(width > 0.0f)) { *d_tg = mn; return; }
     constexpr int WINDOW = (int)(0.05 * URH_GUESS_BINS) + 1;
-    int top[2] = {-1, -1};
-    for (int b = 0; b < URH_GUESS_BINS; b++) {
+    unsigned long long key = 0ull;
+    if (width > 0.0f && threadIdx.x < URH_GUESS_BINS) {
+        const int b = threadIdx.x;
         const unsigned int y = s_hist[b];
         bool peak = y > 0u;
         for (int d = 1; d < WINDOW && peak; d++)
             peak = y > (b + d < URH_GUESS_BINS ? s_hist[b + d] : 0u) && y > (b - d >= 0 ? s_hist[b - d] : 0u);
-        if (!peak) continue;
-        if (top[0] < 0 || y > s_hist[top[0]]) { top[1] = top[0]; top[0] = b; }
-        else if (top[1] < 0 || y > s_hist[top[1]]) top[1] = b;
-    }
-    if (top[0] < 0) *d_tg = 0.5f * (mn + mx);
-    else if (top[1] < 0) *d_tg = mn + ((float)top[0] + 0.5f) * width;
-    else *d_tg = mn + (0.5f * (float)(top[0] + top[1]) + 0.5f) * width;
+        if (peak) key = ((unsigned long long)y << 8) | (unsigned long long)(255 - b);
+    }
+    if (key) atomicMax(&s_top[0], key);
+    __syncthreads();
+    if (key && key != s_top[0]) atomicMax(&s_top[1], key);
+    __syncthreads();
+    if (threadIdx.x != 0) return;
+    *redone = 0u;
+    *d_init = 0;
+    if (!(mn <= mx)) { *d_tg = 0.0f; return; }
+    if (!(width > 0.0f)) { *d_tg = mn; return; }
+    const int top0 = s_top[0] ? 255 - (int)(s_top[0] & 255) : -1, top1 = s_top[1] ? 255 - (int)(s_top[1] & 255) : -1;
+    if (top0 < 0) *d_tg = 0.5f * (mn + mx);
+    else if (top1 < 0) *d_tg = mn + ((float)top0 + 0.5f) * width;
+    else *d_tg = mn + (0.5f * (float)(top0 + top1) + 0.5f) * width;
 }
 
 
@@ -278,14 +314,14 @@
     const int vec_in = iq_vec_aligned(d_iq, DT) ? 1 : 0;
     const int vec_out = (d_qad && ((uintptr_t)d_qad % 8) == 0) ? 1 : 0;
     const int threads = URH_WARPS_PER_BLOCK * 32;
-    auto generic = [&](int64_t begin, int64_t end) -> int {
+    auto generic = [&](int64_t begin, int64_t end, cudaStream_t s) -> int {
         begin = begin < tile_lo ? tile_lo : begin;
         end = end > tile_hi ? tile_hi : end;
         const int64_t count = end - begin;
         if (count <= 0) return URH_OK;
-        URH_LAUNCH(ctx, (k_dense_iq<DT, MOD, DIG>), (unsigned)urh_div_up(count, URH_WARPS_PER_BLOCK), threads, fine_smem, d_iq, n, dp,
-                   d_qad, vec_in, vec_out, cls, tol, tiles, staging, stage_cap, init_cls, cls_of_zero, begin, count, has_halo,
-                   tile_stats, fine);
+        URH_LAUNCH_ON(ctx, s, (k_dense_iq<DT, MOD, DIG>), (unsigned)urh_div_up(count, URH_WARPS_PER_BLOCK), threads, fine_smem, d_iq, n, dp,
+                      d_qad, vec_in, vec_out, cls, tol, tiles, staging, stage_cap, init_cls, cls_of_zero, begin, count, has_halo,
+                      tile_stats, fine);
         return URH_OK;
     };
     const int64_t nfull = n / URH_TILE;
@@ -293,6 +329,11 @@
     URH_PROF_BEGIN(ctx);
     if (fast) {
         const int64_t fb = tile_lo > 1 ? tile_lo : 1, fe = tile_hi < nfull ? tile_hi : nfull;
+        const bool tile0 = tile_lo < 1 && tile_hi > 0;
+        if (tile0) {
+            URH_CUDA(ctx, cudaEventRecord(ctx->ev_fork, ctx->stream));
+            URH_CUDA(ctx, cudaStreamWaitEvent(ctx->side_stream, ctx->ev_fork, 0));
+        }
         if (fe > fb) {
             const unsigned grid = (unsigned)urh_div_up(fe - fb, URH_WARPS_PER_BLOCK);
             static const bool fifo = getenv("URH_B200_FSK_NO_FIFO") == nullptr;
@@ -325,10 +366,14 @@
                                 tiles, staging, stage_cap, fb, fe - fb, nullptr, UrhFine{});
             }
         }
-        URH_CHECK(generic(0, 1));
-        URH_CHECK(generic(nfull, ntiles));
+        if (tile0) {
+            URH_CHECK(generic(0, 1, ctx->side_stream));
+            URH_CUDA(ctx, cudaEventRecord(ctx->ev_join, ctx->side_stream));
+            URH_CUDA(ctx, cudaStreamWaitEvent(ctx->stream, ctx->ev_join, 0));
+        }
+        URH_CHECK(generic(nfull, ntiles, ctx->stream));
     } else {
-        URH_CHECK(generic(0, ntiles));
+        URH_CHECK(generic(0, ntiles, ctx->stream));
     }
     URH_PROF_END(ctx);
     return URH_OK;
@@ -410,9 +455,11 @@
 }
 
 int urh_finish_local(urh_ctx* ctx, int64_t n, int tol, bool is_ask, uint32_t sps, const UrhTileSummary* tiles, const uint32_t* staging,
-                     int stage_cap, const int16_t* d_init, int64_t* k);
+                     int stage_cap, const int16_t* d_init, int64_t* k, int64_t* record = nullptr,
+                     int64_t* h_record = nullptr);
 int urh_finish_shard(urh_ctx* ctx, int64_t n, int tol, bool is_ask, uint32_t sps, const UrhTileSummary* tiles, const uint32_t* staging,
-                     int stage_cap, const int16_t* d_init, int64_t global_offset, int64_t n_total, int64_t* k);
+                     int stage_cap, const int16_t* d_init, int64_t global_offset, int64_t n_total, int64_t* k, int64_t* record = nullptr,
+                     int64_t* h_record = nullptr);
 
 static int digitize_finish(urh_ctx* ctx, int64_t n, int tol, bool is_ask, uint32_t sps, UrhTileSummary* tiles,
                            uint32_t* staging, int stage_cap, int16_t* d_init, int64_t* k) {
@@ -802,9 +849,8 @@
 
 struct CenterPlan;
 int urh_center_chain(urh_ctx* ctx, const float* d_qad, int64_t n, const UrhTileStats* ts, int64_t max_size, int rank, int world,
-                     const UrhFine* fine, CenterPlan** d_plan_out);
+                     const UrhFine* fine, int64_t* record, CenterPlan** d_plan_out);
 int urh_center_plan_result(urh_ctx* ctx, const CenterPlan* plan, const float** d_centerf, const double** d_center, const int** d_state);
-int urh_center_plan_certify_stats(urh_ctx* ctx, const CenterPlan* plan, int64_t* h_dst3);
 
 extern "C" int urh_shard_digitize(urh_ctx* ctx, const void* d_iq, int dtype, const float* d_qad_in, int64_t n, int has_halo,
                                   float noise_mag, int mod_type, float center, uint16_t tolerance, uint32_t samples_per_symbol,
@@ -882,13 +928,16 @@
     UrhTileStats* ts;
     URH_CHECK(urh_arena(ctx, (size_t)ntiles, &ts));
     const bool no_certify = getenv("URH_B200_CENTER_NO_CERTIFY") != nullptr;
+    const bool speculate = !sharded && !h_iq && !sc && mod_type == URH_MOD_FSK && dtype == URH_DT_F32 &&
+                           getenv("URH_B200_NO_SPECULATE") == nullptr;
     UrhFine fine = {};
+    int64_t fine_words = 0;
     if (!sharded && !no_certify) {
         fine.slab_tiles = urh_div_up(ntiles, URH_FINE_SLABS);
         if (fine.slab_tiles < URH_WARPS_PER_BLOCK) fine.slab_tiles = URH_WARPS_PER_BLOCK;
-        const int64_t nslabs = urh_div_up(ntiles, fine.slab_tiles);
-        URH_CHECK(urh_arena(ctx, (size_t)(nslabs * URH_FINE_NB), &fine.gh));
-        URH_CUDA(ctx, cudaMemsetAsync(fine.gh, 0, (size_t)(nslabs * URH_FINE_NB) * sizeof(unsigned int), ctx->stream));
+        fine_words = urh_div_up(ntiles, fine.slab_tiles) * URH_FINE_NB;
+        URH_CHECK(urh_arena(ctx, (size_t)fine_words, &fine.gh));
+        if (!speculate) URH_CUDA(ctx, cudaMemsetAsync(fine.gh, 0, (size_t)fine_words * sizeof(unsigned int), ctx->stream));
         fine.scale = (mod_type == URH_MOD_FSK) ? 512.0f : 4096.0f;
         fine.off = (mod_type == URH_MOD_FSK) ? 2048.0f : 0.0f;
     }
@@ -919,18 +968,24 @@
         URH_CHECK(urh_arena(ctx, (size_t)ntiles * cap, &staging));
         URH_CHECK(urh_arena(ctx, 8, &d_init));
     }
-    const bool speculate = !sharded && !h_iq && !sc && mod_type == URH_MOD_FSK && dtype == URH_DT_F32 &&
-                           getenv("URH_B200_NO_SPECULATE") == nullptr;
+    int64_t* record;
+    URH_CHECK(urh_arena(ctx, URH_REC_WORDS, &record));
+    int64_t h_record[URH_REC_WORDS] = {};
     UrhSpec spec = {};
     if (speculate) {
-        float* tg;
+        float *tg, *vals;
+        float2* mnmx;
         URH_CHECK(urh_arena(ctx, 1, &tg));
-        URH_CHECK(urh_arena(ctx, 1, &spec.redone));
+        spec.redone = (unsigned int*)(record + URH_REC_REDONE);
         URH_CHECK(urh_arena(ctx, (size_t)ntiles, &spec.margin));
+        URH_CHECK(urh_arena(ctx, URH_GUESS_SAMPLES, &vals));
+        URH_CHECK(urh_arena(ctx, URH_GUESS_BLOCKS, &mnmx));
+        urhts::Ws ws;
+        URH_CHECK(urhts::prepare(ctx, URH_GUESS_BLOCKS, &ws));
         spec.tg = tg;
         const char* forced = getenv("URH_B200_SPECULATE_GUESS");
-        URH_LAUNCH(ctx, k_speculate_guess, 1, URH_GUESS_THREADS, 0, (const float2*)d_iq, n, dp.noise_sqrd, forced ? 1 : 0,
-                   forced ? strtof(forced, nullptr) : 0.0f, tg, spec.redone);
+        URH_LAUNCH(ctx, k_speculate_guess, URH_GUESS_BLOCKS, URH_GUESS_THREADS, 0, (const float2*)d_iq, n, dp.noise_sqrd, forced ? 1 : 0,
+                   forced ? strtof(forced, nullptr) : 0.0f, tg, spec.redone, d_init, fine.gh, fine_words, vals, mnmx, ws.counter, ws.base);
     }
     int chunk_no = 0;
     for (int64_t t0 = 0; t0 < (sc ? 0 : ntiles); t0 += chunk_tiles, chunk_no++) {
@@ -951,22 +1006,13 @@
     }
     CenterPlan* plan = nullptr;
     URH_CHECK(urh_center_chain(ctx, d_qad_out, n, ts, max_size, sharded ? ctx->nccl_rank : 0, sharded ? ctx->nccl_world : 1,
-                               fine.gh ? &fine : nullptr, &plan));
+                               fine.gh ? &fine : nullptr, record, &plan));
     const float* d_centerf;
-    const double* d_center;
-    const int* d_state;
-    urh_center_plan_result(ctx, plan, &d_centerf, &d_center, &d_state);
+    urh_center_plan_result(ctx, plan, &d_centerf, nullptr, nullptr);
     int64_t rows = 0;
     if (sc) {
-        URH_CUDA(ctx, cudaMemcpyAsync(ctx->h_mail + 40, d_center, sizeof(double), cudaMemcpyDeviceToHost, ctx->stream));
-        URH_CUDA(ctx, cudaMemcpyAsync(ctx->h_mail + 41, d_state, sizeof(int), cudaMemcpyDeviceToHost, ctx->stream));
-        URH_CHECK(urh_center_plan_certify_stats(ctx, plan, ctx->h_mail + 42));
-        URH_CUDA(ctx, cudaMemcpyAsync(ctx->h_mail + 45, (const int64_t*)ctx->center_prefix + ntiles, sizeof(int64_t), cudaMemcpyDeviceToHost,
-                                      ctx->stream));
-        URH_CUDA(ctx, cudaStreamSynchronize(ctx->stream));
-        int st0 = 0;
-        memcpy(&st0, ctx->h_mail + 41, sizeof(int));
-        if (st0 == 1) {
+        URH_CHECK(urh_read_i64(ctx, record, URH_REC_WORDS, h_record));
+        if (h_record[URH_REC_STATE] == 1) {
             StreamDigitizer dz;
             URH_CHECK(dz.init(ctx, n, scs, tol, mod_type == URH_MOD_ASK, samples_per_symbol));
             for (int64_t s0 = 0; s0 < n; s0 += scs) {
@@ -976,9 +1022,9 @@
             }
             rows = dz.rows;
         }
-        *sc->kept = ctx->h_mail[45];
+        *sc->kept = h_record[URH_REC_KEPT];
     } else {
-        URH_CUDA(ctx, cudaMemsetAsync(d_init, 0, 16, ctx->stream));
+        if (!speculate) URH_CUDA(ctx, cudaMemsetAsync(d_init, 0, 16, ctx->stream));
         const int vec_in = (((uintptr_t)d_qad_out % 8) == 0) ? 1 : 0;
         int64_t grid = urh_div_up(ntiles, URH_WARPS_PER_BLOCK);
         if (speculate) {
@@ -989,24 +1035,21 @@
         }
         URH_LAUNCH(ctx, (k_dense_f32<SrcQad2, float>), (unsigned)grid, URH_WARPS_PER_BLOCK * 32, 0,
                    (const float*)d_qad_out, n, vec_in, cls, tol, tiles, staging, cap, d_init, 0, d_centerf, (const UrhTileStats*)ts, spec);
-        URH_CUDA(ctx, cudaMemcpyAsync(ctx->h_mail + 40, d_center, sizeof(double), cudaMemcpyDeviceToHost, ctx->stream));
-        URH_CUDA(ctx, cudaMemcpyAsync(ctx->h_mail + 41, d_state, sizeof(int), cudaMemcpyDeviceToHost, ctx->stream));
-        URH_CHECK(urh_center_plan_certify_stats(ctx, plan, ctx->h_mail + 42));
-        ctx->h_mail[46] = 0;
-        if (speculate) URH_CUDA(ctx, cudaMemcpyAsync(ctx->h_mail + 46, spec.redone, sizeof(unsigned int), cudaMemcpyDeviceToHost, ctx->stream));
         if (sharded)
-            URH_CHECK(urh_finish_shard(ctx, n, tol, mod_type == URH_MOD_ASK, samples_per_symbol, tiles, staging, cap, d_init, global_offset, n_total, &rows));
+            URH_CHECK(urh_finish_shard(ctx, n, tol, mod_type == URH_MOD_ASK, samples_per_symbol, tiles, staging, cap, d_init, global_offset, n_total, &rows,
+                                       record, h_record));
         else
-            URH_CHECK(urh_finish_local(ctx, n, tol, mod_type == URH_MOD_ASK, samples_per_symbol, tiles, staging, cap, d_init, &rows));
-    }
-    memcpy(center, ctx->h_mail + 40, sizeof(double));
-    int st = 0;
-    memcpy(&st, ctx->h_mail + 41, sizeof(int));
+            URH_CHECK(urh_finish_local(ctx, n, tol, mod_type == URH_MOD_ASK, samples_per_symbol, tiles, staging, cap, d_init, &rows, record, h_record));
+    }
+    memcpy(center, &h_record[URH_REC_CENTER], sizeof(double));
+    const int st = (int)h_record[URH_REC_STATE];
     *center_state = st;
-    ctx->center_cert[0] = ctx->h_mail[42];
+    ctx->center_cert[0] = h_record[URH_REC_CERTIFIED];
     ctx->center_cert[1] = fine.gh ? URH_FINE_NB : 0;
-    ctx->center_cert[2] = ctx->h_mail[44];
-    const int64_t redone = (spec.hi > spec.lo) ? ctx->h_mail[46] : 0;
+    ctx->center_cert[2] = h_record[URH_REC_STRADDLE];
+    unsigned int redone_u = 0;
+    memcpy(&redone_u, &h_record[URH_REC_REDONE], sizeof(redone_u));
+    const int64_t redone = (spec.hi > spec.lo) ? (int64_t)redone_u : 0;
     ctx->spec_stats[0] = spec.hi - spec.lo;
     ctx->spec_stats[1] = spec.hi - spec.lo - redone;
     ctx->spec_stats[2] = redone;
diff --git a/urh_b200/csrc/finish.cu b/urh_b200/csrc/finish.cu
--- a/urh_b200/csrc/finish.cu
+++ b/urh_b200/csrc/finish.cu
@@ -203,7 +203,7 @@
         if (l_prev == CLS_NONE) l_prev = *d_prev0;
         l_idx = row_off[tl];
         l_pp = prev_fired[tl];
-        if (l_pp < 0) l_pp = *d_xprev_fired;
+        if (l_pp < 0 && d_xprev_fired) l_pp = *d_xprev_fired;
     }
     for (int j0 = 0; j0 < FIN_TILES && t0 + j0 < ntiles; j0 += FIN_BATCH) {
         uint32_t w0[FIN_BATCH];
@@ -343,6 +343,8 @@
     int emit_tail;
     UrhChain* chain;
     int64_t row_base, rows_cap;
+    int64_t* record;
+    int64_t* h_record;
 };
 
 static int finish_tiles(urh_ctx* ctx, int64_t n, int tol, bool is_ask, uint32_t sps, const UrhTileSummary* tiles, const uint32_t* staging,
@@ -361,7 +363,7 @@
     TileFire* fire;
     URH_CHECK(urh_arena(ctx, (size_t)ntiles, &fire));
     URH_CHECK(urh_arena(ctx, (size_t)(32 + 8 * (sharded ? sh.world : 0)), &d_small));
-    URH_CUDA(ctx, cudaMemsetAsync(d_small, 0xff, 4 * sizeof(int64_t), ctx->stream));
+    int64_t* d_rows = sh.record ? sh.record : d_small;
     RunCarry* d_tot_run = (RunCarry*)(d_small + 4);
     CandAgg* d_tot_cand = (CandAgg*)(d_small + 6);
     FireAgg* d_tot_fire = (FireAgg*)(d_small + 8);
@@ -407,7 +409,7 @@
     FireAgg fi_ident;
     fi_ident.fired = 0; fi_ident.last_pos = -1;
     URH_CHECK((urhts::scan<FireAgg, FireOp, ScanFirings>(ctx, ntiles, fi_ident, FireOp(), fc, d_tot_fire)));
-    const int64_t* xprev = chain ? &chain->prev_fired : d_small + 2;
+    const int64_t* xprev = chain ? &chain->prev_fired : nullptr;
     if (sharded) {
         URH_TL_MARK(ctx, "x6 firings: enter");
         URH_CHECK(urh_coll_allgather(ctx, d_tot_fire, d_all3, sizeof(FireAgg)));
@@ -430,9 +432,15 @@
     for (int attempt = 0; attempt < 2; attempt++) {
         URH_LAUNCH(ctx, k_finish_rows, (unsigned)urh_div_up(ntiles, 8 * FIN_TILES), 256, 0, tiles, staging, stage_cap, (const int32_t*)head_rel,
                    (const int32_t*)prev_cls, prev0, (const int64_t*)row_off, (const int64_t*)prev_fired, xprev, ntiles, sh.global_offset,
-                   sh.n_total, tol, is_ask ? 1 : 0, (int64_t)sps, sh.emit_tail, row_base, raw, raw_cap, d_small);
+                   sh.n_total, tol, is_ask ? 1 : 0, (int64_t)sps, sh.emit_tail, row_base, raw, raw_cap, d_rows);
         if (sharded && attempt == 0) URH_TL_MARK(ctx, "rows written");
-        URH_CHECK(urh_read_i64(ctx, d_small, 2, got));
+        if (sh.record) {
+            URH_CHECK(urh_read_i64(ctx, sh.record, URH_REC_WORDS, sh.h_record));
+            got[0] = sh.h_record[URH_REC_ROWS];
+            got[1] = sh.h_record[URH_REC_FIRED];
+        } else {
+            URH_CHECK(urh_read_i64(ctx, d_small, 2, got));
+        }
         if (sharded) URH_CHECK(urh_p2p_check(ctx));
         if (got[0] <= raw_cap) break;
         if (attempt == 1 || chain) URH_FAIL(ctx, URH_ERR_CUDA, "finish_tiles: row buffer overflow after regrowth");
@@ -472,22 +480,26 @@
     sh.rank = 0; sh.world = 1; sh.global_offset = global_offset; sh.n_total = n_total;
     sh.emit_tail = (global_offset + n == n_total) ? 1 : 0;
     sh.chain = chain; sh.row_base = row_base; sh.rows_cap = rows_cap;
+    sh.record = nullptr; sh.h_record = nullptr;
     return finish_tiles(ctx, n, tol, is_ask, sps, tiles, staging, stage_cap, d_init, sh, k);
 }
 
 int urh_finish_local(urh_ctx* ctx, int64_t n, int tol, bool is_ask, uint32_t sps, const UrhTileSummary* tiles, const uint32_t* staging,
-                     int stage_cap, const int16_t* d_init, int64_t* k) {
+                     int stage_cap, const int16_t* d_init, int64_t* k, int64_t* record, int64_t* h_record) {
     FinishShard sh;
     sh.rank = 0; sh.world = 1; sh.global_offset = 0; sh.n_total = n; sh.emit_tail = 1;
     sh.chain = nullptr; sh.row_base = 0; sh.rows_cap = 0;
+    sh.record = record; sh.h_record = h_record;
     return finish_tiles(ctx, n, tol, is_ask, sps, tiles, staging, stage_cap, d_init, sh, k);
 }
 
 int urh_finish_shard(urh_ctx* ctx, int64_t n, int tol, bool is_ask, uint32_t sps, const UrhTileSummary* tiles, const uint32_t* staging,
-                     int stage_cap, const int16_t* d_init, int64_t global_offset, int64_t n_total, int64_t* k) {
+                     int stage_cap, const int16_t* d_init, int64_t global_offset, int64_t n_total, int64_t* k, int64_t* record,
+                     int64_t* h_record) {
     FinishShard sh;
     sh.rank = ctx->nccl_rank; sh.world = ctx->nccl_world; sh.global_offset = global_offset; sh.n_total = n_total;
     sh.emit_tail = (ctx->nccl_rank == ctx->nccl_world - 1) ? 1 : 0;
     sh.chain = nullptr; sh.row_base = 0; sh.rows_cap = 0;
+    sh.record = record; sh.h_record = h_record;
     return finish_tiles(ctx, n, tol, is_ask, sps, tiles, staging, stage_cap, d_init, sh, k);
 }
```

Result: no change. 216,300 (median of 6 runs) (+1.3%).
